# Sirui-Xu/InterDiff

Measured on AMD Instinct MI355X. Metric: denoising frame-steps/sec (denoising-steps/sec x B x T frames), higher is better.
Workload: dtype f32 (every contraction of the denoiser -- feed-forward block, QKV projection, self-attention, row-block contractions and the two token GEMMs: every fp32 operand as two f16 planes, 3 f16 MFMAs per product, fp32 accumulate; SMPL and everything else fp32 MFMA / VALU)

## Files before the change

include/interdiff_hip.h:

```cpp
#ifndef INTERDIFF_HIP_H
#define INTERDIFF_HIP_H

#include <stddef.h>
#include <stdint.h>

#ifdef __cplusplus
extern "C" {
#endif

#define IDF_OK            0
#define IDF_E_INVAL      -22
#define IDF_E_NOMEM      -12
#define IDF_E_LAUNCH     -5

int         interdiff_abi_version(void);
const char *interdiff_build_info(void);

int interdiff_rotation_6d_to_matrix   (const float *d6, float *m,  int64_t n, void *stream);
int interdiff_matrix_to_rotation_6d   (const float *m,  float *d6, int64_t n, void *stream);
int interdiff_matrix_to_axis_angle    (const float *m,  float *aa, int64_t n, void *stream);
int interdiff_axis_angle_to_matrix    (const float *aa, float *m,  int64_t n, void *stream);
int interdiff_axis_angle_to_quaternion(const float *aa, float *q,  int64_t n, void *stream);
int interdiff_rotation_6d_to_axis_angle(const float *d6, float *aa, int64_t n, void *stream);

typedef struct {
    int32_t V, J, n_betas, KB, S;
    const float   *blend;
    const float   *jt;
    const float   *js;
    const int32_t *parents;
    const int32_t *skin_idx;
    const float   *skin_w;
} idf_smpl_model;

size_t interdiff_smpl_workspace_bytes(const idf_smpl_model *m, int64_t N);
int interdiff_smpl_forward(const idf_smpl_model *m, const float *pose, const float *betas,
                           const float *trans, int64_t N, float *verts, float *jtr,
                           float *v_posed, void *ws, size_t ws_bytes, void *stream);

int interdiff_vertex_normals(const float *verts, int64_t N, int32_t V, const int32_t *faces,
                             const int32_t *adj_ptr, const int32_t *adj_face,
                             const int32_t *adj_corner, float *normals, void *stream);
int interdiff_nn_argmin(const float *q, int32_t Pq, const float *r, int32_t Pr, int64_t N,
                        int32_t *idx, void *stream);
int interdiff_point2point_signed(const float *x, int32_t P1, const float *y, int32_t P2, int64_t N,
                                 const float *x_normals, const float *y_normals,
                                 float *y2x_signed, float *x2y_signed, int32_t *yidx, int32_t *xidx,
                                 float *y2x, float *x2y, void *stream);

#define IDF_MDM_LAYERS 8
#define IDF_MDM_D      256
#define IDF_MDM_FF     1024
#define IDF_MDM_HEADS  4
#define IDF_MDM_NQ     10
#define IDF_MDM_MEM    10
#define IDF_MDM_MEM_MAX 16
#define IDF_FFN_SLICES 5

typedef struct {
    int64_t is_qan;
    int64_t sa_in_w, sa_in_b, sa_out_w, sa_out_b;
    int64_t qc, wk;
    int64_t ca_q_w, ca_q_b;
    int64_t ca_kv_w, ca_kv_b;
    int64_t ca_out_w, ca_out_b;
    int64_t ff1_w, ff1_b, ff2_w, ff2_b;
    int64_t ffn_pack;
    int64_t ffn_b1p;
    int64_t sa_in_pack;
    int64_t sa_out_frag;
    int64_t ln_w[3], ln_b[3];
    int64_t ffn_pack_h2;
    int64_t sa_in_pack_h2;
    int64_t qc_h2;
    int64_t rb_h2_ok;
    int64_t sa_out_frag_h2;
    int64_t qkv_bounds_ok;
} idf_mdm_layer;

typedef struct {
    int32_t C;
    int32_t n_steps;
    const float *arena;
    int64_t in_w, in_b;
    int64_t out_w, out_b;
    int64_t temb_table;
    int64_t pe;
    int32_t max_T, has_encoder;
    idf_mdm_layer layer[IDF_MDM_LAYERS];
    idf_mdm_layer enc_layer[IDF_MDM_LAYERS];
    int32_t tune[8];
    int64_t out_w_h2, in_w_h2;
    int64_t tail_h2_ok;
    int32_t mem_len;
    int32_t rb_tokens;
} idf_mdm_weights;

int interdiff_gemm_f32(const float *A, int32_t lda, const float *W, const float *bias, const float *resid, float *C,
                       int32_t ldc, int32_t M, int32_t N, int32_t K, int32_t epi, int32_t cfg, void *stream);

int interdiff_mdm_ffn(const idf_mdm_weights *w, int32_t layer, int32_t encoder, const float *x2, int32_t M, float *parts, void *stream);
size_t interdiff_mdm_memctx_floats_for(int32_t B, int32_t mem_len);

size_t interdiff_mdm_memctx_floats(int32_t B);
size_t interdiff_mdm_workspace_bytes(int32_t B, int32_t T);
int interdiff_mdm_prepare_memory(const idf_mdm_weights *w, const float *cond, int32_t B,
                                 float *memctx, void *ws, size_t ws_bytes, void *stream);
int interdiff_mdm_forward(const idf_mdm_weights *w, const float *memctx, const float *x,
                          const int64_t *ts, int32_t B, int32_t T, float *x0,
                          void *ws, size_t ws_bytes, void *stream);

typedef struct {
    int64_t w[3], b[3];
    int32_t c[4];
} idf_pn_mlp;

typedef struct {
    const float *arena;
    idf_pn_mlp sa1[2];
    idf_pn_mlp sa2[2];
    int64_t lin_w, lin_b;
} idf_pointnet2;

int interdiff_pointnet2_encode(const idf_pointnet2 *pn, const float *obj_points, int32_t B, int32_t P, float *out,
                               void *stream);
size_t interdiff_mdm_encode_workspace_bytes(int32_t B, int32_t Tp);
int interdiff_mdm_encode(const idf_mdm_weights *w, const float *pc, const float *x_past, int32_t B, int32_t Tp,
                         float *cond, void *ws, size_t ws_bytes, void *stream);

int interdiff_inpaint(float *x0, const float *gt, const uint8_t *mask, int64_t n, void *stream);
int interdiff_posterior_step(float *x, const float *x0, const float *noise, int64_t n,
                             float c1, float c2, float sigma, uint64_t seed, uint64_t step_index,
                             void *stream);
int interdiff_randn(float *out, int64_t n, uint64_t seed, uint64_t step_index, void *stream);
int interdiff_posterior_step_at(float *x, const float *x0, const float *noise, int64_t n,
                                float c1, float c2, float sigma, uint64_t seed, uint64_t step_index,
                                uint64_t elem0, void *stream);
int interdiff_randn_at(float *out, int64_t n, uint64_t seed, uint64_t step_index, uint64_t elem0, void *stream);
int interdiff_posterior_step_dev(float *x, const float *x0, const float *gt, const uint8_t *mask, int64_t n,
                                 const float *table, int64_t *state, int64_t *ts, int32_t B, void *stream);
int interdiff_sampler_advance(int64_t *state, int64_t *ts, int32_t B, void *stream);
int interdiff_posterior_step_dev_map(float *x, const float *x0, const float *gt, const uint8_t *mask, int64_t n,
                                     const float *table, const int64_t *tmap, int64_t *state, int64_t *ts, int32_t B, void *stream);
int interdiff_sampler_advance_map(int64_t *state, int64_t *ts, const int64_t *tmap, int32_t B, void *stream);
int interdiff_mdm_forward_step(const idf_mdm_weights *w, const float *memctx, float *x, int64_t *ts, int32_t B, int32_t T,
                               const float *gt, const uint8_t *mask, const float *table, int64_t *state,
                               void *ws, size_t ws_bytes, void *stream);
#define IDF_STEP_EMBED_READY 1
#define IDF_STEP_EMBED_NEXT 2
int interdiff_mdm_forward_step_ex(const idf_mdm_weights *w, const float *memctx, float *x, int64_t *ts, int32_t B, int32_t T,
                                  const float *gt, const uint8_t *mask, const float *table, int64_t *state, void *ws,
                                  size_t ws_bytes, int32_t flags, void *stream);
int interdiff_mdm_forward_step_map(const idf_mdm_weights *w, const float *memctx, float *x, int64_t *ts, int32_t B, int32_t T,
                                   const float *gt, const uint8_t *mask, const float *table, const int64_t *tmap, int64_t *state,
                                   void *ws, size_t ws_bytes, int32_t flags, void *stream);
int interdiff_mdm_step_chaining(const idf_mdm_weights *w);
int interdiff_exclusive_cu_report(char *buf, int32_t cap);
int interdiff_debug_deny_exclusive(const char *patterns);

typedef struct {
    int32_t T, past_len, P, n_pre;
    const float *arena;
    int64_t dct_pad;
    int64_t dct;
    int64_t idct;
    int64_t hand_bonus;
    int64_t layer[12];
    int32_t cin[12], cout[12];
} idf_objproj;

int interdiff_objprojector_sample(const idf_objproj *op, const float *obj_angles,
                                  const float *obj_trans, const float *markers,
                                  const int32_t *contact, int32_t B, float *out, void *stream);
size_t interdiff_objprojector_forward_workspace_bytes(int32_t B);
int interdiff_objprojector_forward(const idf_objproj *op, const float *obj_angles, const float *obj_trans, const float *markers,
                                   const int32_t *contact, int32_t B, int32_t initialize, float *out, void *ws, size_t ws_bytes, void *stream);

int interdiff_correction_finetune_param_table(const idf_objproj *op, int32_t *table, int32_t *n_param, int32_t *n_bn);
size_t interdiff_correction_finetune_workspace_bytes(const idf_objproj *op, int32_t B);
int interdiff_correction_finetune_grads(const idf_objproj *op, const float *params, const float *bn, const float *obj_angles,
                                        const float *obj_trans, const float *markers, const int32_t *contact, const float *d_obj_pred,
                                        int32_t B, int32_t T, int32_t initialize, const float *weights8, float *out9, float *grads, void *ws,
                                        size_t ws_bytes, void *stream);
int interdiff_correction_finetune_step(const idf_objproj *op, float *arena, float *params, const float *bn, const float *grads,
                                       float *exp_avg, float *exp_avg_sq, int32_t step, double lr, double beta1, double beta2, double eps,
                                       double weight_decay, void *stream);

size_t interdiff_correction_train_workspace_bytes(const idf_objproj *op, int32_t B);
int interdiff_correction_train_grads(const idf_objproj *op, const float *params, float *bn, const float *obj_angles, const float *obj_trans,
                                     const float *markers, const int32_t *contact, const int32_t *nodes, const float *d_obj_pred, int32_t B,
                                     int32_t T, int32_t initialize, const float *weights8, double p_drop, const uint8_t *masks, uint64_t seed,
                                     uint64_t step, double momentum, int32_t update_running, float *out9, float *grads, float *batch_stats,
                                     void *ws, size_t ws_bytes, void *stream);
int interdiff_correction_train_masks(const idf_objproj *op, int32_t B, double p_drop, uint64_t seed, uint64_t step, uint8_t *masks_out,
                                     void *stream);

int interdiff_correction_finetune_predict(const idf_objproj *op, const float *params, const float *bn, const float *obj_angles,
                                          const float *obj_trans, const float *markers, const int32_t *contact, int32_t B, int32_t T,
                                          int32_t initialize, float *obj_pred_out, void *ws, size_t ws_bytes, void *stream);
int interdiff_correction_train_predict(const idf_objproj *op, const float *params, const float *obj_angles, const float *obj_trans,
                                       const float *markers, const int32_t *contact, const int32_t *nodes, int32_t B, int32_t T,
                                       int32_t initialize, double p_drop, const uint8_t *masks, uint64_t seed, uint64_t step, float *obj_pred_out,
                                       void *ws, size_t ws_bytes, void *stream);

typedef struct {
    const idf_smpl_model *smpl;
    const idf_objproj    *objproj;
    const int32_t *faces;
    const int32_t *adj_ptr, *adj_face, *adj_corner;
    const int32_t *markers_idx;
    int32_t n_markers, n_points, past_len;
    int32_t tune;
    const int32_t *vorder, *faces_scan, *markers_scan, *adj_pair_scan;
    const int32_t *adj_pair;
    const int32_t *vrank;
} idf_correction_ctx;

size_t interdiff_correction_workspace_bytes(const idf_correction_ctx *c, int32_t B, int32_t T);
int interdiff_correction(const idf_correction_ctx *c, float *x0, const float *gt,
                         const float *hand_pose, const float *beta, const float *obj_points,
                         int32_t B, int32_t T, float blend_t ,
                         uint8_t *condition, int32_t *contact, float *distance, float *loss,
                         void *ws, size_t ws_bytes, void *stream);
int interdiff_correction_dev(const idf_correction_ctx *c, float *x0, const float *gt, const float *hand_pose,
                             const float *beta, const float *obj_points, int32_t B, int32_t T, const float *table,
                             const int64_t *state, void *ws, size_t ws_bytes, void *stream);

#define IDF_CONTACT_STATS 12
size_t interdiff_contact_nn_workspace_bytes(const idf_correction_ctx *c, int32_t B, int32_t T);
int interdiff_contact_nn(const idf_correction_ctx *c, const float *verts, const float *obj_points, const float *objR,
                         const float *objT, int32_t B, int32_t T, float *o2h, int32_t *idx, uint64_t *stats,
                         void *ws, size_t ws_bytes, void *stream);

size_t interdiff_metrics_workspace_bytes(const idf_correction_ctx *c, int32_t B, int32_t T);
int interdiff_metrics(const idf_correction_ctx *c, const float *obj_pred, const float *jtr,
                      const float *body_trans, const float *obj_gt, const float *jtr_gt,
                      const float *body_trans_gt, const float *verts, const float *obj_points,
                      int32_t B, int32_t T, int32_t J, float *out6 ,
                      void *ws, size_t ws_bytes, void *stream);

typedef struct {
    int32_t T, past_len, J, n_pre;
    const float *arena;
    int64_t dct_pad;
    int64_t dct;
    int64_t idct;
    int64_t layer[12];
    int32_t cin[12], cout[12];
} idf_skel_objproj;

int interdiff_skeleton_objprojector_sample(const idf_skel_objproj *op, const float *obj_angles,
                                           const float *obj_trans, const float *human_points, int32_t B,
                                           float *quat_out, float *trans_out, void *stream);
int interdiff_skeleton_correction(const idf_skel_objproj *op, const float *x, const float *gt,
                                  const float *zero_pose_obj, int32_t B, int32_t T, float blend_t,
                                  float *out, void *stream);
int interdiff_skeleton_metrics(const float *body_pred, const float *body_gt, const float *obj_pred,
                               const float *obj_gt, const float *pose_pred, const float *pose_gt,
                               int32_t T, int32_t B, int32_t from_frame, float *out4, void *stream);

int interdiff_skeleton_finetune_param_table(const idf_skel_objproj *op, int32_t *table, int32_t *n_param, int32_t *n_bn);
size_t interdiff_skeleton_finetune_workspace_bytes(const idf_skel_objproj *op, int32_t B);
int interdiff_skeleton_finetune_grads(const idf_skel_objproj *op, const float *params, const float *bn, const float *obj_angles,
                                      const float *obj_trans, const float *human_points, const float *pose_gt, int32_t B, int32_t T,
                                      const float *weights8, float *out9, float *grads, void *ws, size_t ws_bytes, void *stream);
int interdiff_skeleton_finetune_step(const idf_skel_objproj *op, float *arena, float *params, const float *bn, const float *grads,
                                     float *exp_avg, float *exp_avg_sq, int32_t step, double lr, double beta1, double beta2, double eps,
                                     double weight_decay, void *stream);

size_t interdiff_skeleton_train_workspace_bytes(const idf_skel_objproj *op, int32_t B);
int interdiff_skeleton_train_grads(const idf_skel_objproj *op, const float *params, float *bn, const float *obj_angles, const float *obj_trans,
                                   const float *human_points, const float *pose_gt, int32_t B, int32_t T, const float *weights8, double p_drop,
                                   const uint8_t *masks, uint64_t seed, uint64_t step, double momentum, int32_t update_running, float *out9,
                                   float *grads, float *batch_stats, void *ws, size_t ws_bytes, void *stream);
int interdiff_skeleton_train_masks(const idf_skel_objproj *op, int32_t B, double p_drop, uint64_t seed, uint64_t step, uint8_t *masks_out,
                                   void *stream);

typedef struct idf_skel_head {
    int32_t n_body, n_points;
    int32_t n_tiles, reserved;
    int64_t out_w, out_b;
    int64_t shape_w, shape_b;
} idf_skel_head;
int interdiff_skeleton_mdm_forward(const idf_mdm_weights *w, const idf_skel_head *head, const float *memctx, const float *x,
                                   const int64_t *ts, const float *zero_pose_obj, int32_t B, int32_t T, float *x0,
                                   void *ws, size_t ws_bytes, void *stream);
int interdiff_skeleton_mdm_forward_step(const idf_mdm_weights *w, const idf_skel_head *head, const float *memctx, float *x,
                                        int64_t *ts, const float *zero_pose_obj, int32_t B, int32_t T, const float *gt,
                                        const uint8_t *mask, const float *table, int64_t *state, void *ws, size_t ws_bytes,
                                        void *stream);
int interdiff_skeleton_mdm_forward_step_map(const idf_mdm_weights *w, const idf_skel_head *head, const float *memctx, float *x,
                                            int64_t *ts, const float *zero_pose_obj, int32_t B, int32_t T, const float *gt,
                                            const uint8_t *mask, const float *table, const int64_t *tmap, int64_t *state, void *ws,
                                            size_t ws_bytes, void *stream);
size_t interdiff_skeleton_mdm_encode_workspace_bytes(int32_t B, int32_t Tp);
int interdiff_skeleton_mdm_encode(const idf_mdm_weights *w, const idf_skel_head *head, const float *zero_pose_obj,
                                  const float *x_past, int32_t B, int32_t Tp, float *cond, void *ws, size_t ws_bytes,
                                  void *stream);

#define IDF_OPT_NP 483
#define IDF_OPT_NLOSS 6
typedef struct {
    const idf_correction_ctx *geo;
    const float   *blendT;
    const int32_t *jv_ptr;
    const int32_t *jv_vtx;
    const float   *jv_w;
    int32_t K3P, _pad;
} idf_opt_ctx;

typedef struct {
    int32_t B, T, P, max_iters;
    const float *betas;
    const float *obj_points;
    float *param, *init, *grad, *m, *v, *best;
    float *pose, *tr;
    float *verts, *vposed, *verts_gt, *gv;
    float *jtr;
    float *pts, *y2x;
    float *y2x_signed;
    int32_t *yidx;
    int32_t *near;
    float *dvposed;
    float *dA;
    float *dfeat;
    float *gtr;
    float *lossf;
    float *loss;
    float *loss_hist;
    float *best_loss;
    int32_t *flag;
    uint8_t *foot_static;
    int32_t *foot_cnt;
    int32_t *ctl;
    void *smpl_ws; size_t smpl_ws_bytes;
    int32_t *porder; float *psort, *pbox;
} idf_opt_state;

int interdiff_optimize_init(const idf_opt_ctx *c, const idf_opt_state *st, const float *pose, const float *trans,
                            const float *obj_angles, const float *obj_trans, int32_t first_iter, void *stream);
int interdiff_optimize_loss_grad(const idf_opt_ctx *c, const idf_opt_state *st, void *stream);
int interdiff_optimize_step(const idf_opt_ctx *c, const idf_opt_state *st, void *stream);
int interdiff_optimize_finish(const idf_opt_ctx *c, const idf_opt_state *st, float *pose, float *trans, float *obj_angles,
                              float *obj_trans, void *stream);
int interdiff_debug_joint_map_vjp(const float *R, const float *g_out, float *g_in, int32_t n);
int interdiff_debug_lds_sentinel(uint32_t *out, int32_t n_wg, int32_t spin, void *stream);
int interdiff_debug_f16_aggressor(const float *src, size_t n_floats, float *sink, int32_t iters, int32_t grid, int32_t with_loads, void *stream);

enum { IDF_LOSS_VAL = 0, IDF_LOSS_TEST = 1 };
int interdiff_q_sample(float *x_t, const float *x0, const float *noise, const int64_t *ts, const float *sqrt_ac, const float *sqrt_1mac,
                       int32_t n_steps, const float *gt, const uint8_t *mask, int32_t B, int64_t per_clip, uint64_t seed, uint64_t elem0,
                       void *stream);
int interdiff_denoising_losses(const float *pred, const float *target, int32_t B, int32_t T, int32_t past_len, float *out, void *stream);
size_t interdiff_sample_losses_workspace_bytes(int32_t K, int32_t B);
int interdiff_sample_losses(const float *samples, const float *gt, const float *hand_pose, int32_t K, int32_t B, int32_t T, int32_t past_len,
                            int32_t variant, float *out_terms, float *out_per_clip, void *ws, size_t ws_bytes, void *stream);

int interdiff_denoising_loss_grad(const float *pred, const float *target, int32_t B, int32_t T, int32_t past_len, const float *weights16,
                                  float *d_pred, void *stream);
int interdiff_mdm_train_param_table(int64_t *offsets, int64_t *sizes, int32_t *n_tensors, int64_t *n_param);
size_t interdiff_mdm_train_workspace_bytes(int32_t B, int32_t T, int32_t mem_len);
int interdiff_mdm_train_grads(const float *params, const float *pe, int32_t pe_rows, const float *x_t, const int64_t *ts, const float *cond,
                              const float *target, int32_t B, int32_t T, int32_t mem_len, int32_t past_len, const float *weights16,
                              const float *d_pred_in, float *grads, float *d_cond, float *pred, float *terms, void *ws, size_t ws_bytes,
                              void *stream);
int interdiff_mdm_train_step(float *params, const float *grads, float *exp_avg, float *exp_avg_sq, int64_t n, int32_t step, double lr,
                             double beta1, double beta2, double eps, double weight_decay, void *stream);

int interdiff_mdm_train_full_param_table(int64_t *offsets, int64_t *sizes, int32_t *n_tensors, int64_t *n_param);
size_t interdiff_mdm_train_full_workspace_bytes(int32_t B, int32_t T, int32_t past_len);
int interdiff_mdm_train_full_grads(const float *params, const float *pe, int32_t pe_rows, const float *x_t, const int64_t *ts, const float *pc,
                                   const float *target, int32_t B, int32_t T, int32_t past_len, const float *weights16, const float *d_pred_in,
                                   float *grads, float *cond, float *d_cond, float *d_pc, float *pred, float *terms, void *ws, size_t ws_bytes,
                                   void *stream);

size_t interdiff_pointnet2_saves_bytes(int32_t B);
int interdiff_pointnet2_encode_saved(const idf_pointnet2 *pn, const float *obj_points, int32_t B, int32_t P, float *out, void *saves, size_t saves_bytes,
                                     void *stream);
int interdiff_pointnet2_finetune_param_table(int64_t *offsets, int64_t *sizes, int32_t *n_tensors, int64_t *n_param);
size_t interdiff_pointnet2_finetune_workspace_bytes(int32_t B);
int interdiff_pointnet2_finetune_grads(const idf_pointnet2 *pn, const float *theta, const float *stats, const float *obj_points, int32_t B, int32_t P,
                                       const void *saves, const float *d_pc, float *grads, void *ws, size_t ws_bytes, void *stream);
int interdiff_pointnet2_refold(const idf_pointnet2 *pn, const float *theta, const float *stats, void *stream);

size_t interdiff_pointnet2_train_workspace_bytes(int32_t B);
int interdiff_pointnet2_train_forward(const float *theta, const float *obj_points, int32_t B, int32_t P, float *pc_out, void *ws, size_t ws_bytes, void *stream);
int interdiff_pointnet2_train_grads(const float *theta, const float *obj_points, int32_t B, int32_t P, const float *d_pc, float *grads, void *ws, size_t ws_bytes,
                                    void *stream);
int interdiff_pointnet2_train_stats(const void *ws, int32_t B, double momentum, float *stats, void *stream);

size_t interdiff_skeleton_sample_losses_workspace_bytes(int32_t K, int32_t B);
int interdiff_skeleton_sample_losses(const float *pred, const float *gt, int32_t K, int32_t B, int32_t C, int32_t T, int32_t past_len,
                                     int32_t n_body, int32_t n_points, float *out_terms, float *out_per_clip, void *ws, size_t ws_bytes,
                                     void *stream);
int interdiff_skeleton_denoising_losses(const float *pred, const float *target, int32_t B, int32_t T, int32_t past_len, int32_t n_body,
                                        int32_t n_points, float *out, void *stream);

int interdiff_skeleton_denoising_loss_grad(const float *pred, const float *target, int32_t B, int32_t T, int32_t past_len, const float *weights13,
                                           float *d_pred, void *stream);
int interdiff_skeleton_mdm_train_param_table(int64_t *offsets, int64_t *sizes, int32_t *n_tensors, int64_t *n_param);
size_t interdiff_skeleton_mdm_train_workspace_bytes(int32_t B, int32_t T, int32_t past_len);
int interdiff_skeleton_mdm_train_grads(const float *params, const float *pe, int32_t pe_rows, const float *x_t, const int64_t *ts, const float *target,
                                       const float *zero_pose_obj, int32_t B, int32_t T, int32_t past_len, const float *weights13,
                                       const float *d_pred_in, float *grads, float *cond, float *pred, float *terms, void *ws, size_t ws_bytes,
                                       void *stream);

size_t interdiff_correction_losses_workspace_bytes(int32_t T, int32_t B, int32_t V, int32_t P);
int interdiff_correction_losses(const float *obj_pred, const float *obj_gt, const float *obj_points, int32_t point_stride, const float *human_verts,
                                int32_t T, int32_t B, int32_t V, int32_t P, int32_t rot_width, int32_t past_len, float *out_terms, float *out_frames,
                                void *ws, size_t ws_bytes, void *stream);

size_t interdiff_correction_geometry_grads_workspace_bytes(int32_t T, int32_t B, int32_t V, int32_t P);
int interdiff_correction_geometry_grads(const float *obj_pred, const float *obj_points, int32_t point_stride, const float *human_verts, int32_t T,
                                        int32_t B, int32_t V, int32_t P, double w_penetration, double w_contact, float *d_obj_pred_out,
                                        float *terms2_out, float *frames_out, void *ws, size_t ws_bytes, void *stream);

size_t interdiff_contact_labels_workspace_bytes(int64_t N, int32_t V, int32_t F, int32_t P);
int interdiff_contact_labels(const float *verts, int64_t N, int32_t V, const int32_t *faces, int32_t F, const float *points, int32_t P,
                             int64_t point_frame_stride, const float *objR, const float *objT, float thres, uint8_t *obj_label ,
                             uint8_t *human_label , float *signed_dist , void *ws, size_t ws_bytes, void *stream);
int interdiff_debug_point_triangle(const float *tri, const float *p, float *out, int32_t n);

#define IDF_RENDER_SUBPIX 16
#define IDF_RENDER_GUARD 32768
#define IDF_RENDER_MAX_DIM 2048
#define IDF_RENDER_ZONE (1 << 28)
#define IDF_RENDER_REC_INTS 20
#define IDF_RENDER_TILE 16
#define IDF_RENDER_MAX_MESHES 8
enum { IDF_RMESH_SCENE_SPACE = 1, IDF_RMESH_VERTEX_RGB = 2 };
typedef struct {
    float off[3], cam_t[3];
    float cam_cos, cam_sin, znear, focal;
    float light[9];
    float light_gain, ambient;
    float bg[3];
    float reserved;
} idf_render_scene;
typedef struct {
    const float *verts, *normals;
    const int32_t *faces;
    const float *rgb, *R, *t;
    int32_t V, F, frames, flags;
} idf_render_mesh;
size_t interdiff_render_frames_workspace_bytes(int64_t n_images, int64_t n_triangles, int32_t H, int32_t W);
int interdiff_render_frames(const idf_render_scene *scene, const idf_render_mesh *meshes, int32_t n_meshes, int64_t N, int32_t views, int32_t H,
                            int32_t W, uint8_t *out_rgb, int32_t *out_id, int32_t *out_depth, int32_t *out_setup, int64_t *dropped, float *stage_ms,
                            void *ws, size_t ws_bytes, void *stream);
int interdiff_debug_render_setup_vertex(const idf_render_scene *scene, int32_t view, int32_t scene_space, int32_t H, int32_t W, const float *pos,
                                        const float *nrm, const float *rgb, float *out_f, int32_t *out_i, int32_t n);
int interdiff_debug_render_pixel(const int32_t *rec, const int32_t *ij, int32_t *out, int32_t n);

#define IDF_SKEL_REC_INTS 8
#define IDF_SKEL_MAX_REC 128
#define IDF_SKEL_MAX_WIRES 40
#define IDF_SKEL_WD_MAX 1024
#define IDF_SKEL_TILE 16
enum { IDF_SKEL_PLAIN = 0, IDF_SKEL_PREDGT = 1 };
typedef struct {
    float view[12];
    float aspect[3], margin[3];
    float dist, kx, cx, ky, cy;
    int32_t line_wd, disc_wd, style, pred_from;
    uint8_t colour[5][4];
} idf_skel_view;
size_t interdiff_skeleton_render_frames_workspace_bytes(int64_t n_frames);
int interdiff_skeleton_render_frames(const idf_skel_view *view, const float *body, const float *obj, const float *body_gt, const float *obj_gt,
                                     const int32_t *wires, int32_t n_wires, int64_t B, int32_t T, int32_t T_gt, int32_t H, int32_t W, uint8_t *out_rgb,
                                     int32_t *out_setup, int32_t *out_count, int64_t *dropped, float *stage_ms, void *ws, size_t ws_bytes, void *stream);
int interdiff_skeleton_raster_records(const int32_t *recs, int32_t count, int64_t n_frames, int32_t H, int32_t W, uint8_t *out_rgb, void *stream);
int interdiff_debug_skeleton_setup(const idf_skel_view *view, const float *body, const float *obj, const float *body_gt, const float *obj_gt,
                                   const int32_t *wires, int32_t n_wires, int32_t T, int32_t T_gt, int32_t t, int32_t *rec, int32_t *count,
                                   int32_t *dropped);
int interdiff_debug_skeleton_pixel(const int32_t *rec, int32_t n_rec, const int32_t *ij, int32_t *out, int32_t n);

typedef struct {
    int32_t n_seq, P, V, n_markers;
    const int64_t *seq_off;
    const float *pose, *betas;
    const double *fit64;
    const float *joints, *obj_points6;
    const int32_t *first_label, *body_ptr, *body_idx, *markers_idx;
} idf_clip_set;
typedef struct {
    float *body_pose, *hand_pose, *body_trans, *obj_angles, *obj_trans, *pelvis, *beta, *gt, *ground, *centroid, *rotation, *obj_points, *obj_points6;
    uint8_t *contact_label;
} idf_clip_batch;
int interdiff_clip_batch(const idf_clip_set *cs, const int32_t *clips, int32_t B, int32_t T, int32_t sample_rate, const idf_clip_batch *out, void *stream);
int interdiff_clip_body_records(const idf_clip_set *cs, const int32_t *clips, int32_t B, int32_t T, int32_t sample_rate, const float *verts,
                                const float *normals, const int32_t *frame_map, int64_t n_frames, float *human_verts, float *markers,
                                uint8_t *contact_label, void *stream);
int interdiff_debug_clip_canon(const double *fit, const float *pelvis, const float *pose, int32_t T, const float *rotation_override, float *root,
                               float *trans, float *obj_angle, float *obj_trans, float *pelvis_out, float *gt, float *centroid, float *rotation);

typedef struct {
    int32_t n_video, J, P, reserved;
    const int64_t *row_off;
    const float *table, *zero_pose_obj;
} idf_skel_clip_set;
typedef struct {
    float *body, *obj, *pose, *zero_pose_obj, *gt;
} idf_skel_window_batch;
int interdiff_skeleton_video_prepare(const double *skel, const double *obj, const double *pose, const double *contact, const int64_t *seq_off,
                                     const int64_t *row_off, int32_t n_video, int32_t J, int32_t P, int32_t stride, float *table, float *zero_pose_obj,
                                     double *report, double *row_contact, int8_t *signs, void *stream);
int interdiff_debug_skeleton_video_prepare(const double *skel, const double *obj, const double *pose, const double *contact, int64_t F, int32_t J, int32_t P,
                                           int32_t stride, float *table, float *zero_pose_obj, double *report, double *row_contact, int8_t *signs);
int interdiff_skeleton_window_batch(const idf_skel_clip_set *cs, const int32_t *clips, int32_t B, int32_t T, const idf_skel_window_batch *out, void *stream);

enum {
    IDF_K_EMBED = 0, IDF_K_GEMM_QKV, IDF_K_SELF_ATTN, IDF_K_GEMM_OUTPROJ, IDF_K_ROWBLOCK_QAN,
    IDF_K_ROWBLOCK_STD, IDF_K_FFN_FUSED, IDF_K_RESERVED7, IDF_K_GEMM_HEADS, IDF_K_MEM_PREP,
    IDF_K_INPAINT, IDF_K_POSTERIOR, IDF_K_CORR_PREPARE, IDF_K_SMPL_POSE, IDF_K_SMPL_BLEND_SKIN,
    IDF_K_CORR_CONTACT, IDF_K_CORR_REDUCE, IDF_K_OBJPROJ, IDF_K_CORR_BLEND, IDF_K_OTHER,
    IDF_K_COUNT
};
int interdiff_profile_begin(int32_t capacity);
int interdiff_profile_end(double *ms_per_kind, int64_t *count_per_kind);

enum {
    IDF_TUNE_FFN = 3, IDF_TUNE_FFN_MATH = 4, IDF_TUNE_COUNT = 8
};

#ifdef __cplusplus
}
#endif
#endif
```

interdiff_amd/_lib.py:

```python
import ctypes as C
import os
import torch

_HERE = os.path.dirname(os.path.abspath(__file__))
LIB_PATH = os.environ.get('INTERDIFF_HIP_LIB') or os.path.join(_HERE, 'csrc', 'libinterdiff_hip.so')
ABI_VERSION = 17

vp, i32, i64, f32, u64, sz = C.c_void_p, C.c_int32, C.c_int64, C.c_float, C.c_uint64, C.c_size_t

MDM_LAYERS = 8
FFN_SLICES = 5
STEP_EMBED_READY, STEP_EMBED_NEXT = 1, 2
LOSS_VAL, LOSS_TEST = 0, 1
TUNE = dict(ffn=3, ffn_math=4)


class SmplModel(C.Structure):
    _fields_ = [('V', i32), ('J', i32), ('n_betas', i32), ('KB', i32), ('S', i32),
                ('blend', vp), ('jt', vp), ('js', vp), ('parents', vp), ('skin_idx', vp), ('skin_w', vp)]


class MdmLayer(C.Structure):
    _fields_ = [('is_qan', i64),
                ('sa_in_w', i64), ('sa_in_b', i64), ('sa_out_w', i64), ('sa_out_b', i64),
                ('qc', i64), ('wk', i64),
                ('ca_q_w', i64), ('ca_q_b', i64), ('ca_kv_w', i64), ('ca_kv_b', i64),
                ('ca_out_w', i64), ('ca_out_b', i64),
                ('ff1_w', i64), ('ff1_b', i64), ('ff2_w', i64), ('ff2_b', i64), ('ffn_pack', i64), ('ffn_b1p', i64), ('sa_in_pack', i64), ('sa_out_frag', i64),
                ('ln_w', i64 * 3), ('ln_b', i64 * 3), ('ffn_pack_h2', i64), ('sa_in_pack_h2', i64), ('qc_h2', i64), ('rb_h2_ok', i64), ('sa_out_frag_h2', i64), ('qkv_bounds_ok', i64)]


class MdmWeights(C.Structure):
    _fields_ = [('C', i32), ('n_steps', i32), ('arena', vp),
                ('in_w', i64), ('in_b', i64), ('out_w', i64), ('out_b', i64),
                ('temb_table', i64), ('pe', i64), ('max_T', i32), ('has_encoder', i32),
                ('layer', MdmLayer * MDM_LAYERS), ('enc_layer', MdmLayer * MDM_LAYERS), ('tune', i32 * 8), ('out_w_h2', i64), ('in_w_h2', i64), ('tail_h2_ok', i64), ('mem_len', i32), ('rb_tokens', i32)]


class PnMlp(C.Structure):
    _fields_ = [('w', i64 * 3), ('b', i64 * 3), ('c', i32 * 4)]


class PointNet2(C.Structure):
    _fields_ = [('arena', vp), ('sa1', PnMlp * 2), ('sa2', PnMlp * 2), ('lin_w', i64), ('lin_b', i64)]


class ObjProj(C.Structure):
    _fields_ = [('T', i32), ('past_len', i32), ('P', i32), ('n_pre', i32), ('arena', vp),
                ('dct_pad', i64), ('dct', i64), ('idct', i64), ('hand_bonus', i64),
                ('layer', i64 * 12), ('cin', i32 * 12), ('cout', i32 * 12)]


class SkelObjProj(C.Structure):
    _fields_ = [('T', i32), ('past_len', i32), ('J', i32), ('n_pre', i32), ('arena', vp),
                ('dct_pad', i64), ('dct', i64), ('idct', i64),
                ('layer', i64 * 12), ('cin', i32 * 12), ('cout', i32 * 12)]


class SkelHead(C.Structure):
    _fields_ = [('n_body', i32), ('n_points', i32), ('n_tiles', i32), ('reserved', i32),
                ('out_w', i64), ('out_b', i64), ('shape_w', i64), ('shape_b', i64)]


class CorrectionCtx(C.Structure):
    _fields_ = [('smpl', C.POINTER(SmplModel)), ('objproj', C.POINTER(ObjProj)),
                ('faces', vp), ('adj_ptr', vp), ('adj_face', vp), ('adj_corner', vp), ('markers_idx', vp),
                ('n_markers', i32), ('n_points', i32), ('past_len', i32), ('tune', i32),
                ('vorder', vp), ('faces_scan', vp), ('markers_scan', vp), ('adj_pair_scan', vp), ('adj_pair', vp), ('vrank', vp)]


class OptCtx(C.Structure):
    _fields_ = [('geo', C.POINTER(CorrectionCtx)), ('blendT', vp), ('jv_ptr', vp), ('jv_vtx', vp), ('jv_w', vp), ('K3P', i32), ('_pad', i32)]


OPT_NP, OPT_NLOSS = 483, 6
_OPT_PTRS = ('betas', 'obj_points', 'param', 'init', 'grad', 'm', 'v', 'best', 'pose', 'tr', 'verts', 'vposed', 'verts_gt', 'gv',
             'jtr', 'pts', 'y2x', 'y2x_signed', 'yidx', 'near', 'dvposed', 'dA', 'dfeat', 'gtr', 'lossf', 'loss', 'loss_hist',
             'best_loss', 'flag', 'foot_static', 'foot_cnt', 'ctl', 'smpl_ws')


class OptState(C.Structure):
    _fields_ = [('B', i32), ('T', i32), ('P', i32), ('max_iters', i32)] + [(k, vp) for k in _OPT_PTRS] + [('smpl_ws_bytes', sz), ('porder', vp), ('psort', vp), ('pbox', vp)]


class RenderScene(C.Structure):
    _fields_ = [('off', f32 * 3), ('cam_t', f32 * 3), ('cam_cos', f32), ('cam_sin', f32), ('znear', f32), ('focal', f32),
                ('light', f32 * 9), ('light_gain', f32), ('ambient', f32), ('bg', f32 * 3), ('reserved', f32)]


class RenderMesh(C.Structure):
    _fields_ = [('verts', vp), ('normals', vp), ('faces', vp), ('rgb', vp), ('R', vp), ('t', vp),
                ('V', i32), ('F', i32), ('frames', i32), ('flags', i32)]


class SkelView(C.Structure):
    _fields_ = [('view', f32 * 12), ('aspect', f32 * 3), ('margin', f32 * 3), ('dist', f32), ('kx', f32), ('cx', f32), ('ky', f32), ('cy', f32),
                ('line_wd', i32), ('disc_wd', i32), ('style', i32), ('pred_from', i32), ('colour', (C.c_uint8 * 4) * 5)]


class ClipSet(C.Structure):
    _fields_ = [('n_seq', i32), ('P', i32), ('V', i32), ('n_markers', i32), ('seq_off', vp), ('pose', vp), ('betas', vp), ('fit64', vp), ('joints', vp),
                ('obj_points6', vp), ('first_label', vp), ('body_ptr', vp), ('body_idx', vp), ('markers_idx', vp)]


CLIP_BATCH_FIELDS = ('body_pose', 'hand_pose', 'body_trans', 'obj_angles', 'obj_trans', 'pelvis', 'beta', 'gt', 'ground', 'centroid', 'rotation', 'obj_points',
                     'obj_points6', 'contact_label')


class ClipBatch(C.Structure):
    _fields_ = [(k, vp) for k in CLIP_BATCH_FIELDS]


class SkelClipSet(C.Structure):
    _fields_ = [('n_video', i32), ('J', i32), ('P', i32), ('reserved', i32), ('row_off', vp), ('table', vp), ('zero_pose_obj', vp)]


SKEL_WINDOW_FIELDS = ('body', 'obj', 'pose', 'zero_pose_obj', 'gt')


class SkelWindowBatch(C.Structure):
    _fields_ = [(k, vp) for k in SKEL_WINDOW_FIELDS]


CLIP_MAX_T = 128
SKEL_SET_MAX_P, SKEL_WINDOW_LDS = 64, 64 * 1024
SKEL_PLAIN, SKEL_PREDGT = 0, 1
SKEL_REC_INTS, SKEL_MAX_REC, SKEL_MAX_WIRES, SKEL_WD_MAX, SKEL_TILE = 8, 128, 40, 1024, 16
RMESH_SCENE_SPACE, RMESH_VERTEX_RGB = 1, 2
RENDER_SUBPIX, RENDER_GUARD, RENDER_MAX_DIM, RENDER_ZONE, RENDER_REC_INTS, RENDER_TILE = 16, 32768, 2048, 1 << 28, 20, 16

_SIGS = {
    'interdiff_abi_version': (C.c_int, []),
    'interdiff_build_info': (C.c_char_p, []),
    'interdiff_rotation_6d_to_matrix': (C.c_int, [vp, vp, i64, vp]),
    'interdiff_matrix_to_rotation_6d': (C.c_int, [vp, vp, i64, vp]),
    'interdiff_matrix_to_axis_angle': (C.c_int, [vp, vp, i64, vp]),
    'interdiff_axis_angle_to_matrix': (C.c_int, [vp, vp, i64, vp]),
    'interdiff_axis_angle_to_quaternion': (C.c_int, [vp, vp, i64, vp]),
    'interdiff_rotation_6d_to_axis_angle': (C.c_int, [vp, vp, i64, vp]),
    'interdiff_smpl_workspace_bytes': (sz, [C.POINTER(SmplModel), i64]),
    'interdiff_smpl_forward': (C.c_int, [C.POINTER(SmplModel), vp, vp, vp, i64, vp, vp, vp, vp, sz, vp]),
    'interdiff_vertex_normals': (C.c_int, [vp, i64, i32, vp, vp, vp, vp, vp, vp]),
    'interdiff_nn_argmin': (C.c_int, [vp, i32, vp, i32, i64, vp, vp]),
    'interdiff_point2point_signed': (C.c_int, [vp, i32, vp, i32, i64, vp, vp, vp, vp, vp, vp, vp, vp, vp]),
    'interdiff_gemm_f32': (C.c_int, [vp, i32, vp, vp, vp, vp, i32, i32, i32, i32, i32, i32, vp]),
    'interdiff_pointnet2_encode': (C.c_int, [C.POINTER(PointNet2), vp, i32, i32, vp, vp]),
    'interdiff_mdm_encode_workspace_bytes': (sz, [i32, i32]),
    'interdiff_mdm_encode': (C.c_int, [C.POINTER(MdmWeights), vp, vp, i32, i32, vp, vp, sz, vp]),
    'interdiff_mdm_ffn': (C.c_int, [C.POINTER(MdmWeights), i32, i32, vp, i32, vp, vp]),
    'interdiff_mdm_memctx_floats': (sz, [i32]),
    'interdiff_mdm_memctx_floats_for': (sz, [i32, i32]),
    'interdiff_mdm_workspace_bytes': (sz, [i32, i32]),
    'interdiff_mdm_prepare_memory': (C.c_int, [C.POINTER(MdmWeights), vp, i32, vp, vp, sz, vp]),
    'interdiff_mdm_forward': (C.c_int, [C.POINTER(MdmWeights), vp, vp, vp, i32, i32, vp, vp, sz, vp]),
    'interdiff_mdm_forward_step': (C.c_int, [C.POINTER(MdmWeights), vp, vp, vp, i32, i32, vp, vp, vp, vp, vp, sz, vp]),
    'interdiff_mdm_forward_step_ex': (C.c_int, [C.POINTER(MdmWeights), vp, vp, vp, i32, i32, vp, vp, vp, vp, vp, sz, i32, vp]),
    'interdiff_mdm_forward_step_map': (C.c_int, [C.POINTER(MdmWeights), vp, vp, vp, i32, i32, vp, vp, vp, vp, vp, vp, sz, i32, vp]),
    'interdiff_mdm_step_chaining': (C.c_int, [C.POINTER(MdmWeights)]),
    'interdiff_inpaint': (C.c_int, [vp, vp, vp, i64, vp]),
    'interdiff_posterior_step': (C.c_int, [vp, vp, vp, i64, f32, f32, f32, u64, u64, vp]),
    'interdiff_randn': (C.c_int, [vp, i64, u64, u64, vp]),
    'interdiff_posterior_step_at': (C.c_int, [vp, vp, vp, i64, f32, f32, f32, u64, u64, u64, vp]),
    'interdiff_randn_at': (C.c_int, [vp, i64, u64, u64, u64, vp]),
    'interdiff_posterior_step_dev': (C.c_int, [vp, vp, vp, vp, i64, vp, vp, vp, i32, vp]),
    'interdiff_sampler_advance': (C.c_int, [vp, vp, i32, vp]),
    'interdiff_posterior_step_dev_map': (C.c_int, [vp, vp, vp, vp, i64, vp, vp, vp, vp, i32, vp]),
    'interdiff_sampler_advance_map': (C.c_int, [vp, vp, vp, i32, vp]),
    'interdiff_objprojector_sample': (C.c_int, [C.POINTER(ObjProj), vp, vp, vp, vp, i32, vp, vp]),
    'interdiff_objprojector_forward_workspace_bytes': (sz, [i32]),
    'interdiff_objprojector_forward': (C.c_int, [C.POINTER(ObjProj), vp, vp, vp, vp, i32, i32, vp, vp, sz, vp]),
    'interdiff_correction_finetune_param_table': (C.c_int, [C.POINTER(ObjProj), vp, C.POINTER(i32), C.POINTER(i32)]),
    'interdiff_correction_finetune_workspace_bytes': (sz, [C.POINTER(ObjProj), i32]),
    'interdiff_correction_finetune_grads': (C.c_int, [C.POINTER(ObjProj), vp, vp, vp, vp, vp, vp, vp, i32, i32, i32, C.POINTER(f32), vp, vp, vp, sz, vp]),
    'interdiff_correction_finetune_step': (C.c_int, [C.POINTER(ObjProj), vp, vp, vp, vp, vp, vp, i32, C.c_double, C.c_double, C.c_double, C.c_double,
                                                     C.c_double, vp]),
    'interdiff_correction_finetune_predict': (C.c_int, [C.POINTER(ObjProj), vp, vp, vp, vp, vp, vp, i32, i32, i32, vp, vp, sz, vp]),
    'interdiff_correction_train_predict': (C.c_int, [C.POINTER(ObjProj), vp, vp, vp, vp, vp, vp, i32, i32, i32, C.c_double, vp, u64, u64, vp, vp, sz, vp]),
    'interdiff_correction_geometry_grads_workspace_bytes': (sz, [i32, i32, i32, i32]),
    'interdiff_correction_geometry_grads': (C.c_int, [vp, vp, i32, vp, i32, i32, i32, i32, C.c_double, C.c_double, vp, vp, vp, vp, sz, vp]),
    'interdiff_correction_train_workspace_bytes': (sz, [C.POINTER(ObjProj), i32]),
    'interdiff_correction_train_grads': (C.c_int, [C.POINTER(ObjProj), vp, vp, vp, vp, vp, vp, vp, vp, i32, i32, i32, C.POINTER(f32), C.c_double, vp, u64, u64,
                                                   C.c_double, i32, vp, vp, vp, vp, sz, vp]),
    'interdiff_correction_train_masks': (C.c_int, [C.POINTER(ObjProj), i32, C.c_double, u64, u64, vp, vp]),
    'interdiff_correction_workspace_bytes': (sz, [C.POINTER(CorrectionCtx), i32, i32]),
    'interdiff_correction': (C.c_int, [C.POINTER(CorrectionCtx), vp, vp, vp, vp, vp, i32, i32, f32,
                                       vp, vp, vp, vp, vp, sz, vp]),
    'interdiff_correction_dev': (C.c_int, [C.POINTER(CorrectionCtx), vp, vp, vp, vp, vp, i32, i32, vp, vp, vp, sz, vp]),
    'interdiff_metrics_workspace_bytes': (sz, [C.POINTER(CorrectionCtx), i32, i32]),
    'interdiff_metrics': (C.c_int, [C.POINTER(CorrectionCtx), vp, vp, vp, vp, vp, vp, vp, vp, i32, i32, i32,
                                    vp, vp, sz, vp]),
    'interdiff_contact_nn_workspace_bytes': (sz, [C.POINTER(CorrectionCtx), i32, i32]),
    'interdiff_contact_nn': (C.c_int, [C.POINTER(CorrectionCtx), vp, vp, vp, vp, i32, i32, vp, vp, vp, vp, sz, vp]),
    'interdiff_skeleton_objprojector_sample': (C.c_int, [C.POINTER(SkelObjProj), vp, vp, vp, i32, vp, vp, vp]),
    'interdiff_skeleton_correction': (C.c_int, [C.POINTER(SkelObjProj), vp, vp, vp, i32, i32, f32, vp, vp]),
    'interdiff_skeleton_metrics': (C.c_int, [vp, vp, vp, vp, vp, vp, i32, i32, i32, vp, vp]),
    'interdiff_skeleton_finetune_param_table': (C.c_int, [C.POINTER(SkelObjProj), vp, C.POINTER(i32), C.POINTER(i32)]),
    'interdiff_skeleton_finetune_workspace_bytes': (sz, [C.POINTER(SkelObjProj), i32]),
    'interdiff_skeleton_finetune_grads': (C.c_int, [C.POINTER(SkelObjProj), vp, vp, vp, vp, vp, vp, i32, i32, C.POINTER(f32), vp, vp, vp, sz, vp]),
    'interdiff_skeleton_finetune_step': (C.c_int, [C.POINTER(SkelObjProj), vp, vp, vp, vp, vp, vp, i32, C.c_double, C.c_double, C.c_double, C.c_double,
                                                   C.c_double, vp]),
    'interdiff_skeleton_train_workspace_bytes': (sz, [C.POINTER(SkelObjProj), i32]),
    'interdiff_skeleton_train_grads': (C.c_int, [C.POINTER(SkelObjProj), vp, vp, vp, vp, vp, vp, i32, i32, C.POINTER(f32), C.c_double, vp, u64, u64,
                                                 C.c_double, i32, vp, vp, vp, vp, sz, vp]),
    'interdiff_skeleton_train_masks': (C.c_int, [C.POINTER(SkelObjProj), i32, C.c_double, u64, u64, vp, vp]),
    'interdiff_skeleton_mdm_forward': (C.c_int, [C.POINTER(MdmWeights), C.POINTER(SkelHead), vp, vp, vp, vp, i32, i32, vp, vp, sz, vp]),
    'interdiff_skeleton_mdm_forward_step': (C.c_int, [C.POINTER(MdmWeights), C.POINTER(SkelHead), vp, vp, vp, vp, i32, i32, vp, vp, vp, vp, vp, sz, vp]),
    'interdiff_skeleton_mdm_forward_step_map': (C.c_int, [C.POINTER(MdmWeights), C.POINTER(SkelHead), vp, vp, vp, vp, i32, i32, vp, vp, vp, vp, vp, vp, sz, vp]),
    'interdiff_skeleton_mdm_encode_workspace_bytes': (sz, [i32, i32]),
    'interdiff_skeleton_mdm_encode': (C.c_int, [C.POINTER(MdmWeights), C.POINTER(SkelHead), vp, vp, i32, i32, vp, vp, sz, vp]),
    'interdiff_q_sample': (C.c_int, [vp, vp, vp, vp, vp, vp, i32, vp, vp, i32, i64, u64, u64, vp]),
    'interdiff_denoising_losses': (C.c_int, [vp, vp, i32, i32, i32, vp, vp]),
    'interdiff_sample_losses_workspace_bytes': (sz, [i32, i32]),
    'interdiff_sample_losses': (C.c_int, [vp, vp, vp, i32, i32, i32, i32, i32, vp, vp, vp, sz, vp]),
    'interdiff_denoising_loss_grad': (C.c_int, [vp, vp, i32, i32, i32, C.POINTER(f32), vp, vp]),
    'interdiff_mdm_train_param_table': (C.c_int, [C.POINTER(i64), C.POINTER(i64), C.POINTER(i32), C.POINTER(i64)]),
    'interdiff_mdm_train_workspace_bytes': (sz, [i32, i32, i32]),
    'interdiff_mdm_train_grads': (C.c_int, [vp, vp, i32, vp, vp, vp, vp, i32, i32, i32, i32, C.POINTER(f32), vp, vp, vp, vp, vp, vp, sz, vp]),
    'interdiff_mdm_train_step': (C.c_int, [vp, vp, vp, vp, i64, i32, C.c_double, C.c_double, C.c_double, C.c_double, C.c_double, vp]),
    'interdiff_mdm_train_full_param_table': (C.c_int, [C.POINTER(i64), C.POINTER(i64), C.POINTER(i32), C.POINTER(i64)]),
    'interdiff_mdm_train_full_workspace_bytes': (sz, [i32, i32, i32]),
    'interdiff_mdm_train_full_grads': (C.c_int, [vp, vp, i32, vp, vp, vp, vp, i32, i32, i32, C.POINTER(f32), vp, vp, vp, vp, vp, vp, vp, vp, sz, vp]),
    'interdiff_pointnet2_saves_bytes': (sz, [i32]),
    'interdiff_pointnet2_encode_saved': (C.c_int, [C.POINTER(PointNet2), vp, i32, i32, vp, vp, sz, vp]),
    'interdiff_pointnet2_finetune_param_table': (C.c_int, [C.POINTER(i64), C.POINTER(i64), C.POINTER(i32), C.POINTER(i64)]),
    'interdiff_pointnet2_finetune_workspace_bytes': (sz, [i32]),
    'interdiff_pointnet2_finetune_grads': (C.c_int, [C.POINTER(PointNet2), vp, vp, vp, i32, i32, vp, vp, vp, vp, sz, vp]),
    'interdiff_pointnet2_refold': (C.c_int, [C.POINTER(PointNet2), vp, vp, vp]),
    'interdiff_pointnet2_train_workspace_bytes': (sz, [i32]),
    'interdiff_pointnet2_train_forward': (C.c_int, [vp, vp, i32, i32, vp, vp, sz, vp]),
    'interdiff_pointnet2_train_grads': (C.c_int, [vp, vp, i32, i32, vp, vp, vp, sz, vp]),
    'interdiff_pointnet2_train_stats': (C.c_int, [vp, i32, C.c_double, vp, vp]),
    'interdiff_skeleton_sample_losses_workspace_bytes': (sz, [i32, i32]),
    'interdiff_skeleton_sample_losses': (C.c_int, [vp, vp, i32, i32, i32, i32, i32, i32, i32, vp, vp, vp, sz, vp]),
    'interdiff_skeleton_denoising_losses': (C.c_int, [vp, vp, i32, i32, i32, i32, i32, vp, vp]),
    'interdiff_skeleton_denoising_loss_grad': (C.c_int, [vp, vp, i32, i32, i32, C.POINTER(f32), vp, vp]),
    'interdiff_skeleton_mdm_train_param_table': (C.c_int, [C.POINTER(i64), C.POINTER(i64), C.POINTER(i32), C.POINTER(i64)]),
    'interdiff_skeleton_mdm_train_workspace_bytes': (sz, [i32, i32, i32]),
    'interdiff_skeleton_mdm_train_grads': (C.c_int, [vp, vp, i32, vp, vp, vp, vp, i32, i32, i32, C.POINTER(f32), vp, vp, vp, vp, vp, vp, sz, vp]),
    'interdiff_correction_losses_workspace_bytes': (sz, [i32, i32, i32, i32]),
    'interdiff_correction_losses': (C.c_int, [vp, vp, vp, i32, vp, i32, i32, i32, i32, i32, i32, vp, vp, vp, sz, vp]),
    'interdiff_contact_labels_workspace_bytes': (sz, [i64, i32, i32, i32]),
    'interdiff_contact_labels': (C.c_int, [vp, i64, i32, vp, i32, vp, i32, i64, vp, vp, f32, vp, vp, vp, vp, sz, vp]),
    'interdiff_debug_point_triangle': (C.c_int, [vp, vp, vp, i32]),
    'interdiff_render_frames_workspace_bytes': (sz, [i64, i64, i32, i32]),
    'interdiff_render_frames': (C.c_int, [C.POINTER(RenderScene), C.POINTER(RenderMesh), i32, i64, i32, i32, i32, vp, vp, vp, vp, C.POINTER(i64), C.POINTER(f32),
                                          vp, sz, vp]),
    'interdiff_debug_render_setup_vertex': (C.c_int, [C.POINTER(RenderScene), i32, i32, i32, i32, vp, vp, vp, vp, vp, i32]),
    'interdiff_debug_render_pixel': (C.c_int, [vp, vp, vp, i32]),
    'interdiff_skeleton_render_frames_workspace_bytes': (sz, [i64]),
    'interdiff_skeleton_render_frames': (C.c_int, [C.POINTER(SkelView), vp, vp, vp, vp, vp, i32, i64, i32, i32, i32, i32, vp, vp, vp, C.POINTER(i64),
                                                   C.POINTER(f32), vp, sz, vp]),
    'interdiff_skeleton_raster_records': (C.c_int, [vp, i32, i64, i32, i32, vp, vp]),
    'interdiff_debug_skeleton_setup': (C.c_int, [C.POINTER(SkelView), vp, vp, vp, vp, vp, i32, i32, i32, i32, vp, C.POINTER(i32), C.POINTER(i32)]),
    'interdiff_debug_skeleton_pixel': (C.c_int, [vp, i32, vp, vp, i32]),
    'interdiff_optimize_init': (C.c_int, [C.POINTER(OptCtx), C.POINTER(OptState), vp, vp, vp, vp, i32, vp]),
    'interdiff_optimize_loss_grad': (C.c_int, [C.POINTER(OptCtx), C.POINTER(OptState), vp]),
    'interdiff_optimize_step': (C.c_int, [C.POINTER(OptCtx), C.POINTER(OptState), vp]),
    'interdiff_optimize_finish': (C.c_int, [C.POINTER(OptCtx), C.POINTER(OptState), vp, vp, vp, vp, vp]),
    'interdiff_debug_joint_map_vjp': (C.c_int, [vp, vp, vp, i32]),
    'interdiff_clip_batch': (C.c_int, [C.POINTER(ClipSet), vp, i32, i32, i32, C.POINTER(ClipBatch), vp]),
    'interdiff_clip_body_records': (C.c_int, [C.POINTER(ClipSet), vp, i32, i32, i32, vp, vp, vp, i64, vp, vp, vp, vp]),
    'interdiff_debug_clip_canon': (C.c_int, [vp, vp, vp, i32, vp, vp, vp, vp, vp, vp, vp, vp, vp]),
    'interdiff_skeleton_video_prepare': (C.c_int, [vp, vp, vp, vp, vp, vp, i32, i32, i32, i32, vp, vp, vp, vp, vp, vp]),
    'interdiff_debug_skeleton_video_prepare': (C.c_int, [vp, vp, vp, vp, i64, i32, i32, i32, vp, vp, vp, vp, vp]),
    'interdiff_skeleton_window_batch': (C.c_int, [C.POINTER(SkelClipSet), vp, i32, i32, C.POINTER(SkelWindowBatch), vp]),
    'interdiff_debug_lds_sentinel':(C.c_int, [vp, i32, i32, vp]),
    'interdiff_exclusive_cu_report': (C.c_int, [C.c_char_p, i32]),
    'interdiff_debug_deny_exclusive': (C.c_int, [C.c_char_p]),
    'interdiff_debug_f16_aggressor': (C.c_int, [vp, sz, vp, i32, i32, i32, vp]),
    'interdiff_profile_begin': (C.c_int, [i32]),
    'interdiff_profile_end': (C.c_int, [C.POINTER(C.c_double), C.POINTER(C.c_int64)]),
}

KERNEL_KINDS = ('embed', 'gemm_qkv', 'self_attn', 'gemm_outproj', 'rowblock_qan', 'rowblock_std', 'ffn_fused', 'reserved7',
                'gemm_heads', 'mem_prep', 'inpaint', 'posterior', 'corr_prepare', 'smpl_pose', 'smpl_blend_skin',
                'corr_contact', 'corr_reduce', 'objproj', 'corr_blend', 'other')

_lib = None


class HipLibraryMissing(RuntimeError):
    pass


def load():
    global _lib
    if _lib is not None:
        return _lib
    if not os.path.exists(LIB_PATH):
        raise HipLibraryMissing('%s not found: build it with `python -m interdiff_amd.csrc.build` '
                                '(there is no CPU/torch fallback for the hot path)' % LIB_PATH)
    lib = C.CDLL(LIB_PATH)
    for name, (res, args) in _SIGS.items():
        fn = getattr(lib, name)
        fn.restype, fn.argtypes = res, args
    if lib.interdiff_abi_version() != ABI_VERSION:
        raise HipLibraryMissing('stale %s: abi %d != %d, rebuild' % (LIB_PATH, lib.interdiff_abi_version(), ABI_VERSION))
    _lib = lib
    return lib


def exclusive_cu_report():
    buf = C.create_string_buffer(8192)
    bad = load().interdiff_exclusive_cu_report(buf, len(buf))
    if bad < 0:
        check(bad, 'exclusive_cu_report')
    return buf.value.decode(), bad


def debug_deny_exclusive(patterns=''):
    check(load().interdiff_debug_deny_exclusive(patterns.encode() if patterns else None), 'debug_deny_exclusive')


def exported_symbols():
    return sorted(_SIGS)


_ERR = {-22: 'IDF_E_INVAL (bad shape / pointer / unsupported size)', -12: 'IDF_E_NOMEM (workspace too small)',
        -5: 'IDF_E_LAUNCH (kernel launch failed)'}


def check(rc, what=''):
    if rc != 0:
        raise RuntimeError('interdiff_hip %s failed: %s' % (what, _ERR.get(rc, rc)))


def dptr(t, dtype=None, allow_none=False):
    if t is None:
        if allow_none:
            return vp(None)
        raise ValueError('null tensor')
    if not t.is_cuda:
        raise ValueError('interdiff_amd ops need device tensors (got %s); the HIP path has no CPU fallback' % t.device)
    if not t.is_contiguous():
        raise ValueError('tensor must be contiguous')
    if dtype is not None and t.dtype != dtype:
        raise ValueError('expected %s, got %s' % (dtype, t.dtype))
    return vp(t.data_ptr())


def stream():
    return vp(torch.cuda.current_stream().cuda_stream)
```

interdiff_amd/correction.py:

```python
import ctypes as C
import os
import itertools
import numpy as np
import torch
from . import _lib
from .geometry import MeshTopology

MARKERS67 = [3470, 3171, 3327, 857, 1812, 628, 182, 3116, 3040, 239,
             1666, 1725, 0, 2174, 1568, 1368, 3387, 2112, 1053, 1058,
             3336, 3346, 1323, 2108, 3122, 3314, 1252, 1082, 1861, 1454,
             850, 2224, 3233, 1769, 6728, 4343, 5273, 4116, 3694, 6399,
             6540, 6488, 3749, 5135, 5194, 3512, 5635, 5210, 4360, 4841,
             6786, 5573, 4538, 4544, 6736, 6747, 4804, 5568, 6544, 6682,
             5322, 4927, 5686, 4598, 6633, 3506, 3508]


_UID = itertools.count(1)


def correction_gate(t0):
    return not (t0 > 500 or t0 % 50 != 0)


class HipCorrection:
    def __init__(self, smpl_layer, objprojector, n_points=2048, past_len=10, markers=MARKERS67, device='cuda', scan_order=True):
        self.lib = _lib.load()
        self.device = torch.device(device)
        self.smpl, self.objproj, self.past_len = smpl_layer, objprojector, past_len
        self.topo = MeshTopology(smpl_layer.th_faces, smpl_layer.cmodel.V, self.device, rest_vertices=getattr(smpl_layer, 'v_template', None) if scan_order else None)
        self.markers_idx = torch.tensor(list(markers), dtype=torch.int32, device=self.device)
        ctx = _lib.CorrectionCtx()
        ctx.smpl = C.pointer(smpl_layer.cmodel)
        ctx.objproj = C.pointer(objprojector.cop)
        self.topo.fill_ctx(ctx)
        ctx.markers_idx = self.markers_idx.data_ptr()
        ctx.n_markers, ctx.n_points, ctx.past_len = len(markers), n_points, past_len
        if self.topo.vorder is not None:
            self.markers_scan = self.topo.scan_positions(markers, self.device)
            ctx.markers_scan = self.markers_scan.data_ptr()
        ctx.tune = 0
        self.ctx = ctx
        self._ws = {}
        self.debug = None
        self._uid = next(_UID)

    graph_capturable = True

    def workspace_for(self, B, T):
        return torch.empty(self.lib.interdiff_correction_workspace_bytes(C.byref(self.ctx), B, T), dtype=torch.uint8, device=self.device)

    def apply_dev(self, x, table, state, y, ws):
        B, _, Cc, T = x.shape
        if y['obj_points'].shape[1] != self.ctx.n_points:
            raise ValueError('obj_points must have %d points' % self.ctx.n_points)
        _lib.check(self.lib.interdiff_correction_dev(C.byref(self.ctx), _lib.dptr(x, torch.float32), _lib.dptr(y['inpainted_motion'], torch.float32),
                                                     _lib.dptr(y['hand_pose'], torch.float32), _lib.dptr(y['beta'], torch.float32),
                                                     _lib.dptr(y['obj_points'], torch.float32), B, T, _lib.dptr(table), _lib.dptr(state),
                                                     _lib.dptr(ws), ws.numel(), _lib.stream()), 'correction_dev')
        return x

    def _workspace(self, B, T):
        need = self.lib.interdiff_correction_workspace_bytes(C.byref(self.ctx), B, T)
        key = torch.cuda.current_stream(self.device).cuda_stream
        ws = self._ws.pop(key, None)
        if ws is None or ws.numel() < need:
            ws = torch.empty(need, dtype=torch.uint8, device=self.device)
        self._ws[key] = ws
        if len(self._ws) > self.MAX_STREAM_WORKSPACES:
            torch.cuda.synchronize(self.device)
            self._ws.pop(next(iter(self._ws)))
        return ws

    MAX_STREAM_WORKSPACES = 4

    def apply(self, x, t0, y):
        B, _, Cc, T = x.shape
        if not x.is_contiguous():
            raise ValueError('x must be contiguous (it is updated in place)')
        if y['obj_points'].shape[1] != self.ctx.n_points:
            raise ValueError('obj_points must have %d points' % self.ctx.n_points)
        gt = y['inpainted_motion'].contiguous()
        hp, beta, pts = y['hand_pose'].contiguous().float(), y['beta'].contiguous().float(), y['obj_points'].contiguous().float()
        ws = self._workspace(B, T)
        dbg = [None] * 4
        if self.debug is not None:
            dbg = [torch.empty(B, dtype=torch.uint8, device=self.device), torch.empty(B, len(MARKERS67), dtype=torch.int32, device=self.device),
                   torch.empty(B, device=self.device), torch.empty(B, device=self.device)]
        blend_t = float(np.float32(t0) / np.float32(1000))
        _lib.check(self.lib.interdiff_correction(C.byref(self.ctx), _lib.dptr(x, torch.float32), _lib.dptr(gt, torch.float32),
                                                 _lib.dptr(hp), _lib.dptr(beta), _lib.dptr(pts), B, T, blend_t,
                                                 *[_lib.dptr(d, allow_none=True) for d in dbg], _lib.dptr(ws), ws.numel(),
                                                 _lib.stream()), 'correction')
        if self.debug is not None:
            self.debug.update(condition=dbg[0], contact=dbg[1], distance=dbg[2], loss=dbg[3])
        return x

    def contact_nn(self, verts, obj_points, objR, objT, want_stats=False):
        T, B = verts.shape[:2]
        P = self.ctx.n_points
        o2h = torch.empty(T, B, P, device=self.device)
        idx = torch.empty(T, B, P, dtype=torch.int32, device=self.device)
        stats = torch.zeros(12, dtype=torch.int64, device=self.device) if want_stats else None
        need = self.lib.interdiff_contact_nn_workspace_bytes(C.byref(self.ctx), B, T)
        ws = getattr(self, '_nn_ws', None)
        if ws is None or ws.numel() < need:
            ws = self._nn_ws = torch.empty(need, dtype=torch.uint8, device=self.device)
        v, pts, R_, t_ = (a.contiguous().float() for a in (verts, obj_points, objR, objT))
        _lib.check(self.lib.interdiff_contact_nn(C.byref(self.ctx), _lib.dptr(v), _lib.dptr(pts), _lib.dptr(R_), _lib.dptr(t_), B, T, _lib.dptr(o2h),
                                                 _lib.dptr(idx), _lib.dptr(stats, allow_none=True), _lib.dptr(ws), ws.numel(), _lib.stream()), 'contact_nn')
        return (o2h, idx, tuple(int(x) for x in stats.cpu())) if want_stats else (o2h, idx)

    def is_active(self, t0):
        return correction_gate(int(t0))

    def __call__(self, x, t, model_kwargs):
        t0 = getattr(t, 'host_value', None)
        if t0 is None:
            t0 = int(t[0])
        if not correction_gate(t0):
            return x
        return self.apply(x, t0, model_kwargs['y'])
```

interdiff_amd/csrc/contact_scan.h:

```cpp
#pragma once
#include <float.h>
#include "common.h"
#include "objproj.h"
#include "vec3.h"

namespace {

constexpr int MAXP = 2048;
__global__ __launch_bounds__(1024) void corr_point_order_kernel(const float *__restrict__ obj_points, int P, int32_t *__restrict__ porder) {
    __shared__ unsigned long long keys[MAXP];
    __shared__ float red[6][1024];
    const int b = blockIdx.x, tid = threadIdx.x;
    const float *op = obj_points + (size_t)b * P * 3;
    float p[2][3];
    float lo[3] = {FLT_MAX, FLT_MAX, FLT_MAX}, hi[3] = {-FLT_MAX, -FLT_MAX, -FLT_MAX};
#pragma unroll
    for (int k = 0; k < 2; ++k) {
        const int i = tid + 1024 * k;
#pragma unroll
        for (int a = 0; a < 3; ++a) {
            p[k][a] = i < P ? op[3 * i + a] : 0.f;
            if (i < P) { lo[a] = fminf(lo[a], p[k][a]); hi[a] = fmaxf(hi[a], p[k][a]); }
        }
    }
#pragma unroll
    for (int a = 0; a < 3; ++a) { red[a][tid] = lo[a]; red[3 + a][tid] = hi[a]; }
    __syncthreads();
    for (int s = 512; s > 0; s >>= 1) {
        if (tid < s) {
#pragma unroll
            for (int a = 0; a < 3; ++a) {
                red[a][tid] = fminf(red[a][tid], red[a][tid + s]);
                red[3 + a][tid] = fmaxf(red[3 + a][tid], red[3 + a][tid + s]);
            }
        }
        __syncthreads();
    }
#pragma unroll
    for (int k = 0; k < 2; ++k) {
        const int i = tid + 1024 * k;
        unsigned long long key = ~0ull;
        if (i < P) {
            unsigned code = 0;
            unsigned q[3];
#pragma unroll
            for (int a = 0; a < 3; ++a) {
                const float ext = red[3 + a][0] - red[a][0];
                const float u = ext > 0.f ? (p[k][a] - red[a][0]) / ext : 0.f;
                q[a] = (unsigned)fminf(fmaxf(u * 1023.0f, 0.f), 1023.0f);
            }
#pragma unroll
            for (int bit = 0; bit < 10; ++bit)
#pragma unroll
                for (int a = 0; a < 3; ++a) code |= ((q[a] >> bit) & 1u) << (3 * bit + a);
            key = ((unsigned long long)code << 11) | (unsigned)i;
        }
        keys[i] = key;
    }
    __syncthreads();
    for (int k = 2; k <= MAXP; k <<= 1) {
        for (int j = k >> 1; j > 0; j >>= 1) {
            const int l = 2 * j * (tid / j) + (tid % j), r = l + j;
            const unsigned long long x = keys[l], y = keys[r];
            const bool up = (l & k) == 0;
            if ((x > y) == up) { keys[l] = y; keys[r] = x; }
            __syncthreads();
        }
    }
#pragma unroll
    for (int k = 0; k < 2; ++k) {
        const int i = tid + 1024 * k;
        if (i < P) porder[(size_t)b * P + i] = (int32_t)(keys[i] & 2047u);
    }
}

constexpr int MAXM = 128;
constexpr float MARK_D2 = 0.00039999996079131961f;
constexpr int CB = 16;
constexpr int SB = 8;
constexpr int SEED_STRIDE = 4;
constexpr int CT = 1024;
constexpr int TASK = 64;
typedef float v2f __attribute__((ext_vector_type(2)));

struct ContactLds {
    int V4, nCB, nSB, nSeed;
    int rec, mark, box, sbox, seed, flags, red, pl, total;
    __host__ __device__ explicit ContactLds(int V) {
        V4 = (V + CB - 1) / CB * CB; nCB = V4 / CB; nSB = (nCB + SB - 1) / SB; nSeed = (nCB + SEED_STRIDE - 1) / SEED_STRIDE;
        rec = 0;
        mark = rec + V4;
        box = mark + MAXM;
        sbox = box + 3 * (nSB * SB / 2);
        seed = sbox + 3 * ((nSB + 2) / 2);
        flags = seed + 2 * ((nSeed + 1) / 2);
        red = flags + MAXM / 4;
        pl = red + CT / 4;
        total = pl + MAXP / 4;
    }
};

__device__ __forceinline__ float3 lds_rec(const float4 *vs, int pos) {
    const float *f = reinterpret_cast<const float *>(vs + 2 * (pos >> 1));
    const int h = pos & 1;
    return make_float3(f[h], f[2 + h], f[4 + h]);
}
__device__ __forceinline__ void lds_rec_store(float4 *vs, int pos, float x, float y, float z) {
    float *f = reinterpret_cast<float *>(vs + 2 * (pos >> 1));
    const int h = pos & 1;
    f[h] = x; f[2 + h] = y; f[4 + h] = z;
}
__device__ __forceinline__ void lds_box_store(float4 *bx, int k, float3 lo, float3 hi) {
    float *f = reinterpret_cast<float *>(bx + 3 * (k >> 1));
    const int h = k & 1;
    f[h] = lo.x; f[2 + h] = lo.y; f[4 + h] = lo.z; f[6 + h] = hi.x; f[8 + h] = hi.y; f[10 + h] = hi.z;
}
__device__ __forceinline__ void lds_box_load(const float4 *bx, int k, float3 &lo, float3 &hi) {
    const float *f = reinterpret_cast<const float *>(bx + 3 * (k >> 1));
    const int h = k & 1;
    lo = make_float3(f[h], f[2 + h], f[4 + h]);
    hi = make_float3(f[6 + h], f[8 + h], f[10 + h]);
}

struct PredArgs {
    idf_objproj op;
    const float *obj_angles, *obj_trans;
    const int32_t *markers_idx;
    float *markers, *keep;
    int nclips;
};
template <bool OPT, bool WITH_PRED = false>
__global__ __launch_bounds__(CT) void corr_contact_kernel(const float *__restrict__ verts, int V,
                                                          const float *__restrict__ obj_points, int P,
                                                          const int32_t *__restrict__ porder ,
                                                          const float *__restrict__ objR, const float *__restrict__ objT,
                                                          const int32_t *__restrict__ faces ,
                                                          const int32_t *__restrict__ adj_ptr,
                                                          const int32_t *__restrict__ adj_face,
                                                          const int32_t *__restrict__ adj_corner,
                                                          const int32_t *__restrict__ adj_pair ,
                                                          const int32_t *__restrict__ vorder ,
                                                          const int32_t *__restrict__ vrank ,
                                                          const int32_t *__restrict__ markers_pos , int M, int B,
                                                          float *__restrict__ markers_out, float *__restrict__ loss_sum,
                                                          float *__restrict__ min_dist, int32_t *__restrict__ label,
                                                          float *__restrict__ o2h_out ,
                                                          int32_t *__restrict__ idx_out ,
                                                          unsigned long long *__restrict__ stats ,
                                                          int64_t nn_from ,
                                                          const float *__restrict__ pts_frame , int frames_per_clip ,
                                                          const PredArgs pred) {
    extern __shared__ __attribute__((aligned(16))) float4 vs[];
    if constexpr (WITH_PRED) {
        if ((int)blockIdx.x < pred.nclips) {
            const int b = blockIdx.x, Tn = pred.op.T;
            for (int i = threadIdx.x; i < Tn * M; i += CT) {
                const int t = i / M, m = i - t * M;
                const size_t nfr = (size_t)t * B + b;
                const float *v = verts + (nfr * V + pred.markers_idx[m]) * 3;
                float *o = pred.markers + (nfr * M + m) * 3;
                o[0] = v[0]; o[1] = v[1]; o[2] = v[2];
            }
            __threadfence();
            __syncthreads();
            idf_objproj_dev::objproj_body<1>(reinterpret_cast<float *>(vs), pred.op, pred.obj_angles, pred.obj_trans, pred.markers, nullptr, B, b, pred.keep, nullptr);
            return;
        }
    }
    const ContactLds L(V);
    const int nCB = L.nCB, nSB = L.nSB;
    float4 *ms = vs + L.mark, *bb = vs + L.box, *sbb = vs + L.sbox, *sd = vs + L.seed;
    int *flags = reinterpret_cast<int *>(vs + L.flags);
    float *red = reinterpret_cast<float *>(vs + L.red);
    float *pl = reinterpret_cast<float *>(vs + L.pl);
    __shared__ int next_task;
    const int64_t n = WITH_PRED ? (int64_t)blockIdx.x - pred.nclips : (int64_t)blockIdx.x;
    const int b = OPT ? (int)(n / frames_per_clip) : (int)(n % B), tid = threadIdx.x;
    const float *vf = verts + (size_t)n * V * 3;
    const bool do_nn = n >= nn_from;
    long long t_prev = 0;
    int n_phase = 0;
    auto phase_done = [&]() {
        if (stats && tid == 0 && do_nn) {
            const long long now = (long long)__builtin_readcyclecounter();
            if (n_phase > 0) atomicAdd(stats + 3 + n_phase, (unsigned long long)(now - t_prev));
            t_prev = now;
        }
        ++n_phase;
    };
    phase_done();
    float R[9] = {1.f, 0.f, 0.f, 0.f, 1.f, 0.f, 0.f, 0.f, 1.f}, tr[3] = {0.f, 0.f, 0.f};
    if constexpr (!OPT) {
#pragma unroll
        for (int k = 0; k < 9; ++k) R[k] = objR[n * 9 + k];
#pragma unroll
        for (int k = 0; k < 3; ++k) tr[k] = objT[n * 3 + k];
    }
    const int my_marker_pos = (!OPT && tid < M) ? markers_pos[tid] : 0;
    if (vorder && vrank) {
        for (int i0 = tid; i0 < V; i0 += 4 * CT) {
            typedef float f3v __attribute__((ext_vector_type(3), aligned(4)));
            int pos[4];
            f3v pv[4];
#pragma unroll
            for (int k = 0; k < 4; ++k) {
                const int i = min(i0 + k * CT, V - 1);
                pos[k] = vrank[i];
                pv[k] = *reinterpret_cast<const f3v *>(vf + 3 * i);
            }
#pragma unroll
            for (int k = 0; k < 4; ++k) {
                if (i0 + k * CT < V) {
                    lds_rec_store(vs, pos[k], pv[k].x, pv[k].y, pv[k].z);
                    reinterpret_cast<int *>(vs + 2 * (pos[k] >> 1) + 1)[2 + (pos[k] & 1)] = i0 + k * CT;
                }
            }
        }
        for (int v = V + tid; v < L.V4; v += CT) {
            lds_rec_store(vs, v, 3e18f, 3e18f, 3e18f);
            reinterpret_cast<int *>(vs + 2 * (v >> 1) + 1)[2 + (v & 1)] = 0x7fffffff;
        }
    } else
    for (int v0 = tid; v0 < L.V4; v0 += 4 * CT) {
        int o[4];
        float x[4], y[4], z[4];
#pragma unroll
        for (int k = 0; k < 4; ++k) {
            const int v = v0 + k * CT;
            o[k] = v < V ? (vorder ? vorder[v] : v) : -1;
        }
#pragma unroll
        for (int k = 0; k < 4; ++k) {
            x[k] = y[k] = z[k] = 3e18f;
            if (o[k] >= 0) {
                typedef float f3v __attribute__((ext_vector_type(3), aligned(4)));
                const f3v pv = *reinterpret_cast<const f3v *>(vf + 3 * o[k]);
                x[k] = pv.x; y[k] = pv.y; z[k] = pv.z;
            }
        }
#pragma unroll
        for (int k = 0; k < 4; ++k) {
            const int v = v0 + k * CT;
            if (v < L.V4) {
                lds_rec_store(vs, v, x[k], y[k], z[k]);
                reinterpret_cast<int *>(vs + 2 * (v >> 1) + 1)[2 + (v & 1)] = o[k] >= 0 ? o[k] : 0x7fffffff;
            }
        }
    }
    if (tid < MAXM) flags[tid] = 0;
    const int ntask_all = (P + TASK - 1) / TASK;
    const int task0 = (int)((long long)blockIdx.y * ntask_all / gridDim.y), task1 = (int)((long long)(blockIdx.y + 1) * ntask_all / gridDim.y);
    if (tid == 0) next_task = task0;
    for (int i = tid; i < MAXP; i += CT) pl[i] = 0.f;
    __syncthreads();
    phase_done();
    if (!OPT && tid < ((M + 1) & ~1)) {
        float3 mk = make_float3(3e18f, 3e18f, 3e18f);
        if (tid < M) {
            mk = lds_rec(vs, my_marker_pos);
            if (markers_out) {
                float *mo = markers_out + ((size_t)n * M + tid) * 3;
                mo[0] = mk.x; mo[1] = mk.y; mo[2] = mk.z;
            }
        }
        lds_rec_store(ms, tid, mk.x, mk.y, mk.z);
    }
    if (do_nn) {
#define IDF_DPP8(v, op, ctrl) v = op(v, __builtin_bit_cast(float, __builtin_amdgcn_update_dpp(__builtin_bit_cast(int, v), __builtin_bit_cast(int, v), ctrl, 0xf, 0xf, false)))
        const int lane_ = tid & 63, wave_ = tid >> 6, nsw = 2 * ((nSB + 2) / 2);
        for (int sb = wave_; sb < nsw; sb += CT / 64) {
            const int pr = sb * 64 + lane_;
            float lx = FLT_MAX, ly = FLT_MAX, lz = FLT_MAX, hx = -FLT_MAX, hy = -FLT_MAX, hz = -FLT_MAX;
            if (2 * pr < V) {
                const float4 xy = vs[2 * pr], zz = vs[2 * pr + 1];
                const bool two = 2 * pr + 1 < V;
                lx = two ? fminf(xy.x, xy.y) : xy.x; hx = two ? fmaxf(xy.x, xy.y) : xy.x;
                ly = two ? fminf(xy.z, xy.w) : xy.z; hy = two ? fmaxf(xy.z, xy.w) : xy.z;
                lz = two ? fminf(zz.x, zz.y) : zz.x; hz = two ? fmaxf(zz.x, zz.y) : zz.x;
            }
            IDF_DPP8(lx, fminf, 0xB1); IDF_DPP8(lx, fminf, 0x4E); IDF_DPP8(lx, fminf, 0x141);
            IDF_DPP8(ly, fminf, 0xB1); IDF_DPP8(ly, fminf, 0x4E); IDF_DPP8(ly, fminf, 0x141);
            IDF_DPP8(lz, fminf, 0xB1); IDF_DPP8(lz, fminf, 0x4E); IDF_DPP8(lz, fminf, 0x141);
            IDF_DPP8(hx, fmaxf, 0xB1); IDF_DPP8(hx, fmaxf, 0x4E); IDF_DPP8(hx, fmaxf, 0x141);
            IDF_DPP8(hy, fmaxf, 0xB1); IDF_DPP8(hy, fmaxf, 0x4E); IDF_DPP8(hy, fmaxf, 0x141);
            IDF_DPP8(hz, fmaxf, 0xB1); IDF_DPP8(hz, fmaxf, 0x4E); IDF_DPP8(hz, fmaxf, 0x141);
            const int cb = sb * SB + (lane_ >> 3);
            if ((lane_ & 7) == 0 && cb < nSB * SB) lds_box_store(bb, cb, make_float3(lx, ly, lz), make_float3(hx, hy, hz));
            const float slx = -wave_max(-lx), sly = -wave_max(-ly), slz = -wave_max(-lz), shx = wave_max(hx), shy = wave_max(hy), shz = wave_max(hz);
            if (lane_ == 0) lds_box_store(sbb, sb, make_float3(slx, sly, slz), make_float3(shx, shy, shz));
        }
#undef IDF_DPP8
        for (int k = tid; k < 2 * ((L.nSeed + 1) / 2); k += CT) {
            const float3 p = lds_rec(vs, min(k * SEED_STRIDE, nCB - 1) * CB);
            lds_rec_store(sd, k, p.x, p.y, p.z);
        }
    }
    const float *op = OPT ? pts_frame + (size_t)n * P * 3 : obj_points + (size_t)b * P * 3;
    const int ln = tid & 63, ntask = task1;
    __syncthreads();
    phase_done();
    float mind2 = FLT_MAX;
    unsigned n_exec = 0, n_test = 0, n_tasks = 0;
    for (;;) {
        int task = 0;
        if (ln == 0) task = atomicAdd(&next_task, 1);
        task = __builtin_amdgcn_readfirstlane(task);
        if (task >= ntask) break;
        ++n_tasks;
        const int sp = task * TASK + ln;
        const int i = sp < P ? (porder ? porder[(size_t)b * P + sp] : sp) : -1;
        const bool valid = i >= 0;
        float px = 0.f, py = 0.f, pz = 0.f;
        if (valid) { px = op[3 * i]; py = op[3 * i + 1]; pz = op[3 * i + 2]; }
        const float qx = OPT ? px : (px * R[0] + py * R[1] + pz * R[2]) + tr[0];
        const float qy = OPT ? py : (px * R[3] + py * R[4] + pz * R[5]) + tr[1];
        const float qz = OPT ? pz : (px * R[6] + py * R[7] + pz * R[8]) + tr[2];
        if (do_nn) {
#pragma clang fp contract(off)
            const v2f QX = v2f{qx, qx}, QY = v2f{qy, qy}, QZ = v2f{qz, qz};
            auto pair_d2 = [&](const float4 xy, const float4 zz) {
#pragma clang fp contract(off)
                const v2f dx = QX - v2f{xy.x, xy.y}, dy = QY - v2f{xy.z, xy.w}, dz = QZ - v2f{zz.x, zz.y};
                return (dx * dx + dy * dy) + dz * dz;
            };
            auto pair_a2 = [&](const float4 xy, const float2 zz) {
                const v2f dx = QX - v2f{xy.x, xy.y}, dy = QY - v2f{xy.z, xy.w}, dz = QZ - v2f{zz.x, zz.y};
                return __builtin_elementwise_fma(dz, dz, __builtin_elementwise_fma(dy, dy, dx * dx));
            };
            constexpr float SCAN_M = 1.000003814697265625f, SCAN_ABS = 1e-37f;
            float seed = FLT_MAX;
            for (int k = 0; k < (L.nSeed + 1) / 2; k += 4) {
                float4 xy[4]; float2 zz[4];
#pragma unroll
                for (int u = 0; u < 4; ++u) { xy[u] = sd[2 * min(k + u, (L.nSeed + 1) / 2 - 1)]; zz[u] = *reinterpret_cast<const float2 *>(&sd[2 * min(k + u, (L.nSeed + 1) / 2 - 1) + 1]); }
#pragma unroll
                for (int u = 0; u < 4; ++u) {
                    const v2f a2 = pair_a2(xy[u], zz[u]);
                    seed = fminf(fminf(seed, a2.x), a2.y);
                }
            }
            float thr = __builtin_fmaf(seed, SCAN_M, SCAN_ABS);
            float best = FLT_MAX, bthr = FLT_MAX;
            int tie = 0;
            int bblk = 0, bblk2 = 0;
            auto pair_lb = [&](const float4 a, const float4 bq, const float4 c) {
#pragma clang fp contract(off)
                const v2f ax = v2f{a.x, a.y} - QX, bx = QX - v2f{bq.z, bq.w};
                const v2f ay = v2f{a.z, a.w} - QY, by = QY - v2f{c.x, c.y};
                const v2f az = v2f{bq.x, bq.y} - QZ, bz = QZ - v2f{c.z, c.w};
                const v2f ex = v2f{fmaxf(fmaxf(ax.x, bx.x), 0.f), fmaxf(fmaxf(ax.y, bx.y), 0.f)};
                const v2f ey = v2f{fmaxf(fmaxf(ay.x, by.x), 0.f), fmaxf(fmaxf(ay.y, by.y), 0.f)};
                const v2f ez = v2f{fmaxf(fmaxf(az.x, bz.x), 0.f), fmaxf(fmaxf(az.y, bz.y), 0.f)};
                return __builtin_elementwise_fma(ez, ez, __builtin_elementwise_fma(ey, ey, ex * ex));
            };
            auto score_block = [&](int cb) {
                ++n_exec;
                const int v0 = cb * CB;
                float4 xy[CB / 2]; float2 zz[CB / 2];
#pragma unroll
                for (int u = 0; u < CB / 2; ++u) { xy[u] = vs[v0 + 2 * u]; zz[u] = *reinterpret_cast<const float2 *>(&vs[v0 + 2 * u + 1]); }
                float bm = FLT_MAX;
#pragma unroll
                for (int u = 0; u < CB / 2; ++u) {
                    const v2f a2 = pair_a2(xy[u], zz[u]);
                    bm = fminf(fminf(bm, a2.x), a2.y);
                }
                if (bm < best) {
                    const float w = __builtin_fmaf(bm, SCAN_M, SCAN_ABS);
                    if (best <= w) { tie = tie ? 2 : 1; bblk2 = bblk; } else tie = 0;
                    best = bm; bblk = v0; bthr = w; thr = fminf(thr, w);
                } else if (bm <= bthr) { tie = tie ? 2 : 1; bblk2 = v0; }
            };
            auto scan_super = [&](int sb) {
                const int cb0 = sb * SB;
#pragma unroll
                for (int j = 0; j < SB / 2; ++j) {
                    const int cb = cb0 + 2 * j;
                    const float4 *bx = bb + 3 * (cb >> 1);
                    const v2f lb = pair_lb(bx[0], bx[1], bx[2]);
                    n_test += 2;
                    if (__builtin_amdgcn_ballot_w64(valid && lb.x <= thr) != 0ull) score_block(cb);
                    if (__builtin_amdgcn_ballot_w64(valid && lb.y <= thr) != 0ull) score_block(cb + 1);
                }
            };
            if (!vorder) {
                for (int cb = 0; cb < nCB; ++cb) score_block(cb);
            } else
            for (int sb = 0; sb < nSB; sb += 2) {
                const float4 *bx = sbb + 3 * (sb >> 1);
                const v2f lb = pair_lb(bx[0], bx[1], bx[2]);
                n_test += 2;
                if (__builtin_amdgcn_ballot_w64(valid && lb.x <= thr) != 0ull) scan_super(sb);
                if (__builtin_amdgcn_ballot_w64(valid && lb.y <= thr) != 0ull) scan_super(sb + 1);
            }
            int pos = bblk, org = 0x7fffffff;
            float ebest = FLT_MAX;
            auto resolve_pair = [&](int pr) {
                const float4 xy = vs[2 * pr], zz = vs[2 * pr + 1];
                const v2f d2 = pair_d2(xy, zz);
                const int o0 = __builtin_bit_cast(int, zz.z), o1 = __builtin_bit_cast(int, zz.w);
                if (d2.x < ebest || (d2.x == ebest && o0 < org)) { ebest = d2.x; org = o0; pos = 2 * pr; }
                if (d2.y < ebest || (d2.y == ebest && o1 < org)) { ebest = d2.y; org = o1; pos = 2 * pr + 1; }
            };
            if (tie < 2) {
#pragma unroll
                for (int u = 0; u < CB / 2; ++u) resolve_pair((bblk >> 1) + u);
                if (tie) {
#pragma unroll
                    for (int u = 0; u < CB / 2; ++u) resolve_pair((bblk2 >> 1) + u);
                }
            } else {
                for (int pr = 0; pr < (V + 1) / 2; ++pr) resolve_pair(pr);
            }
            pos = min(pos, V - 1);
            if (org == 0x7fffffff) org = vorder ? vorder[pos] : pos;
            if constexpr (OPT) {
                if (valid) idx_out[(size_t)n * P + i] = org;
            } else if (valid) {
                const float3 v3 = lds_rec(vs, pos);
                float3 acc = make_float3(0.f, 0.f, 0.f);
                const int e0 = adj_ptr[org], e1 = adj_ptr[org + 1];
                if (adj_pair) {
                    for (int e = e0; e < e1; e += 4) {
                        int2 ab[4];
#pragma unroll
                        for (int u = 0; u < 4; ++u) ab[u] = *reinterpret_cast<const int2 *>(adj_pair + 2 * (size_t)min(e + u, e1 - 1));
#pragma unroll
                        for (int u = 0; u < 4; ++u) {
                            if (e + u < e1) {
                                const float3 nn = cross3(sub3(lds_rec(vs, ab[u].x), v3), sub3(lds_rec(vs, ab[u].y), v3));
                                acc.x += nn.x; acc.y += nn.y; acc.z += nn.z;
                            }
                        }
                    }
                } else {
                    for (int e = e0; e < e1; ++e) {
                        const int f = adj_face[e], c = adj_corner[e];
                        const float3 p0 = lds_rec(vs, faces[3 * f]), p1 = lds_rec(vs, faces[3 * f + 1]), p2 = lds_rec(vs, faces[3 * f + 2]);
                        float3 nn;
                        if (c == 1) nn = cross3(sub3(p2, p1), sub3(p0, p1));
                        else if (c == 2) nn = cross3(sub3(p0, p2), sub3(p1, p2));
                        else nn = cross3(sub3(p1, p0), sub3(p2, p0));
                        acc.x += nn.x; acc.y += nn.y; acc.z += nn.z;
                    }
                }
                const float nl = fmaxf(sqrtf(acc.x * acc.x + acc.y * acc.y + acc.z * acc.z), 1e-6f);
                const float vx = qx - v3.x, vy = qy - v3.y, vz = qz - v3.z;
                const float dt = (acc.x / nl) * vx + (acc.y / nl) * vy + (acc.z / nl) * vz;
                const float d = sqrtf(vx * vx + vy * vy + vz * vz);
                const float o2h = d * (dt > 0.f ? 1.f : (dt < 0.f ? -1.f : 0.f));
                if (o2h_out) o2h_out[(size_t)n * P + i] = o2h;
                if (idx_out) idx_out[(size_t)n * P + i] = org;
                pl[sp] = o2h < 0.f ? fabsf(o2h) * 20.0f : 0.f;
            }
        }
        if (!OPT && valid) {
#pragma clang fp contract(off)
            const v2f QX = v2f{qx, qx}, QY = v2f{qy, qy}, QZ = v2f{qz, qz};
            for (int p2 = 0; p2 < (M + 1) / 2; ++p2) {
                const float4 xy = ms[2 * p2], zz = ms[2 * p2 + 1];
                const v2f dx = v2f{xy.x, xy.y} - QX, dy = v2f{xy.z, xy.w} - QY, dz = v2f{zz.x, zz.y} - QZ;
                const v2f d2 = __builtin_elementwise_fma(dy, dy, dx * dx) + dz * dz;
                mind2 = fminf(fminf(mind2, d2.x), d2.y);
                if (__builtin_amdgcn_ballot_w64(fminf(d2.x, d2.y) < MARK_D2) != 0ull) {
                    if (d2.x < MARK_D2) flags[2 * p2] = 1;
                    if (d2.y < MARK_D2) flags[2 * p2 + 1] = 1;
                }
            }
        }
    }
    if (stats && ln == 0 && do_nn) {
        atomicAdd(stats, (unsigned long long)n_exec);
        atomicAdd(stats + 1, (unsigned long long)nCB * n_tasks);
        atomicAdd(stats + 2, (unsigned long long)n_test);
    }
    phase_done();
    if constexpr (OPT) return;
    __syncthreads();
    phase_done();
    float loss = 0.f;
#pragma unroll
    for (int k = 0; k < MAXP / CT; ++k) loss += pl[tid + CT * k];
    red[tid] = loss;
    __syncthreads();
    for (int s = CT / 2; s > 0; s >>= 1) {
        if (tid < s) red[tid] += red[tid + s];
        __syncthreads();
    }
    const float loss_total = red[0];
    __syncthreads();
    red[tid] = mind2;
    __syncthreads();
    for (int s = CT / 2; s > 0; s >>= 1) {
        if (tid < s) red[tid] = fminf(red[tid], red[tid + s]);
        __syncthreads();
    }
    if (tid == 0) { loss_sum[n] = loss_total; min_dist[n] = red[0] == FLT_MAX ? FLT_MAX : sqrtf(red[0]); }
    if (tid < M) label[(size_t)n * M + tid] = flags[tid];
    phase_done();
    if (stats && tid == 0 && do_nn) atomicAdd(stats + 3, 1ull);
}

size_t contact_lds_bytes(int V) { return (size_t)ContactLds(V).total * sizeof(float4); }

struct ContactArgs {
    const float *verts; int V;
    const float *obj_points; int P;
    int32_t *porder;
    const float *objR, *objT;
    const idf_correction_ctx *ctx;
    int B;
    float *markers, *loss_sum, *min_dist;
    int32_t *label;
    float *o2h;
    int32_t *idx;
    unsigned long long *stats;
    int64_t nn_from;
    const float *pts_frame; int frames_per_clip;
    PredArgs pred;
};

template <bool OPT, bool WITH_PRED>
int launch_contact(hipStream_t s, int64_t N, const ContactArgs &a) {
    static_assert(!(OPT && WITH_PRED), "the predictor rides with the hook's scan only");
    constexpr int SCAN_LDS_MAX = 160 * 1024 - 16384, LDS_LIMIT = WITH_PRED ? 160 * 1024 - 2048 : SCAN_LDS_MAX;
    const idf_correction_ctx *c = a.ctx;
    const size_t lds = contact_lds_bytes(a.V);
    if (lds > (size_t)SCAN_LDS_MAX || a.P > MAXP) return IDF_E_INVAL;
    const bool ordered = c->vorder != nullptr;
    if (OPT ? !ordered : (ordered != (c->faces_scan != nullptr) || ordered != (c->markers_scan != nullptr) || ordered != (c->adj_pair_scan != nullptr))) return IDF_E_INVAL;
    const int32_t *faces = OPT ? nullptr : ordered ? c->faces_scan : c->faces, *mpos = OPT ? nullptr : ordered ? c->markers_scan : c->markers_idx;
    const int32_t *adj_ptr = OPT ? nullptr : c->adj_ptr, *adj_face = OPT ? nullptr : c->adj_face, *adj_corner = OPT ? nullptr : c->adj_corner;
    const int32_t *adj_pair = OPT ? nullptr : c->adj_pair_scan;
    const int M = OPT ? 0 : c->n_markers;
    if (!OPT && a.porder) hipLaunchKernelGGL(corr_point_order_kernel, dim3((unsigned)a.B), dim3(1024), 0, s, a.obj_points, a.P, a.porder);
    const int nclips = WITH_PRED ? a.pred.nclips : 0;
    const size_t lds_launch = (nclips > 0 && lds < idf_objproj_dev::OBJPROJ_LDS) ? idf_objproj_dev::OBJPROJ_LDS : lds;
    if (lds_launch > (size_t)LDS_LIMIT) return IDF_E_INVAL;
    static std::atomic<uint64_t> lds_ok{0};
    if (idf_opt_in_lds(reinterpret_cast<const void *>(corr_contact_kernel<OPT, WITH_PRED>), LDS_LIMIT, lds_ok) != IDF_OK) return IDF_E_LAUNCH;
    hipLaunchKernelGGL((corr_contact_kernel<OPT, WITH_PRED>), OPT ? dim3((unsigned)N, 2) : dim3((unsigned)(N + nclips)), dim3(CT), lds_launch, s, a.verts, a.V,
                       a.obj_points, a.P, a.porder, a.objR, a.objT, faces, adj_ptr, adj_face, adj_corner, adj_pair, c->vorder, c->vrank, mpos, M, a.B,
                       a.markers, a.loss_sum, a.min_dist, a.label, a.o2h, a.idx, a.stats, a.nn_from, a.pts_frame, a.frames_per_clip, a.pred);
    return IDF_OK;
}

}
```

interdiff_amd/csrc/correction.hip:

```cpp
#include "common.h"
#include "objproj.h"
#include "rot_math.h"
#include <float.h>

namespace {

constexpr int NBODY = 22;
constexpr int CTOK = 144;

__global__ __launch_bounds__(256) void corr_prepare_kernel(const float *__restrict__ x0, const float *__restrict__ gt,
                                                           const float *__restrict__ hand_pose, int B, int T,
                                                           float *__restrict__ pose, float *__restrict__ trans,
                                                           float *__restrict__ objR, float *__restrict__ objT,
                                                           float *__restrict__ gt_angles, float *__restrict__ gt_trans) {
    const int64_t i = (int64_t)blockIdx.x * 256 + threadIdx.x;
    const int64_t N = (int64_t)B * T;
    if (i >= N * 24) return;
    const int64_t n = i / 24;
    const int slot = (int)(i - n * 24), t = (int)(n / B), b = (int)(n - (int64_t)t * B);
    const float *xb = x0 + (size_t)b * CTOK * T + t;
    if (slot < NBODY) {
        float d[6], m[9], a[3];
#pragma unroll
        for (int k = 0; k < 6; ++k) d[k] = xb[(size_t)(slot * 6 + k) * T];
        rot::rot6d_to_matrix(d, m);
        rot::matrix_to_axis_angle(m, a);
        float *p = pose + n * 156 + slot * 3;
        p[0] = a[0]; p[1] = a[1]; p[2] = a[2];
    } else if (slot == 22) {
        for (int k = 0; k < 90; ++k) pose[n * 156 + 66 + k] = hand_pose[n * 90 + k];
#pragma unroll
        for (int k = 0; k < 3; ++k) trans[n * 3 + k] = xb[(size_t)(132 + k) * T];
    } else {
        float d[6], m[9];
#pragma unroll
        for (int k = 0; k < 6; ++k) d[k] = xb[(size_t)(135 + k) * T];
        rot::rot6d_to_matrix(d, m);
#pragma unroll
        for (int k = 0; k < 9; ++k) objR[n * 9 + k] = m[k];
        const float *gb = gt + (size_t)b * CTOK * T + t;
#pragma unroll
        for (int k = 0; k < 3; ++k) {
            objT[n * 3 + k] = xb[(size_t)(141 + k) * T];
            gt_trans[n * 3 + k] = gb[(size_t)(141 + k) * T];
        }
#pragma unroll
        for (int k = 0; k < 6; ++k) gt_angles[n * 6 + k] = gb[(size_t)(135 + k) * T];
    }
}

}

#include "contact_scan.h"

namespace {

__global__ __launch_bounds__(128) void corr_reduce_kernel(const float *__restrict__ loss_sum, const float *__restrict__ min_dist,
                                                          const int32_t *__restrict__ label, int B, int T, int past, int P, int M,
                                                          uint8_t *__restrict__ condition, int32_t *__restrict__ contact,
                                                          float *__restrict__ distance_out, float *__restrict__ loss_out) {
    extern __shared__ float fr[];
    const int b = blockIdx.x, tid = threadIdx.x;
    for (int t = tid; t < T; t += 128) {
        fr[t] = loss_sum[(size_t)t * B + b];
        fr[T + t] = min_dist[(size_t)t * B + b];
    }
    if (tid < M) {
        int c = 0;
#pragma unroll 16
        for (int t = past; t < T; ++t) c += label[((size_t)t * B + b) * M + tid];
        contact[(size_t)b * M + tid] = c;
    }
    __syncthreads();
    if (tid == 0) {
        float ls = 0.f, ds = 0.f;
        for (int t = past; t < T; ++t) ls += fr[t] / (float)P;
        for (int t = 0; t < T; ++t) ds += fr[T + t];
        const float loss = ls / (float)(T - past), dist = ds / (float)T;
        condition[b] = !((loss < 0.002f) && (dist < 0.02f));
        if (distance_out) distance_out[b] = dist;
        if (loss_out) loss_out[b] = loss;
    }
}

__global__ __launch_bounds__(256) void corr_blend_kernel(float *__restrict__ x0, const float *__restrict__ proj,
                                                         const uint8_t *__restrict__ condition, int B, int T, float a,
                                                         const float *__restrict__ a_table, const int64_t *__restrict__ a_state) {
    if (a_table) a = a_table[a_state[0] * 4 + 3];
    const int64_t i = (int64_t)blockIdx.x * 256 + threadIdx.x;
    if (i >= (int64_t)B * CTOK * T) return;
    const int b = (int)(i / (CTOK * T)), r = (int)(i - (int64_t)b * CTOK * T), c = r / T, t = r - c * T;
    if (!condition[b]) return;
    const float x = x0[i];
    const float other = c < 135 ? x : proj[((size_t)t * B + b) * 9 + (c - 135)];
    x0[i] = a * x + (1.0f - a) * other;
}

struct CorrWs {
    float *pose, *trans, *objR, *objT, *gt_angles, *gt_trans, *verts, *jtr, *markers, *loss_sum, *min_dist, *proj, *proj_keep;
    int32_t *label, *contact, *porder;
    uint8_t *condition;
    void *smpl_ws;
    size_t smpl_ws_bytes, total;
};

CorrWs carve(const idf_correction_ctx *c, int B, int T, void *ws) {
    const int64_t N = (int64_t)B * T;
    const int V = c->smpl->V, J = c->smpl->J, M = c->n_markers;
    char *p = reinterpret_cast<char *>(ws);
    size_t off = 0;
    auto take = [&](size_t bytes) { char *r = p ? p + off : nullptr; off += idf_align(bytes); return r; };
    CorrWs w;
    w.pose = (float *)take(N * 156 * 4);
    w.trans = (float *)take(N * 3 * 4);
    w.objR = (float *)take(N * 9 * 4);
    w.objT = (float *)take(N * 3 * 4);
    w.gt_angles = (float *)take(N * 6 * 4);
    w.gt_trans = (float *)take(N * 3 * 4);
    w.verts = (float *)take((size_t)N * V * 3 * 4);
    w.jtr = (float *)take((size_t)N * J * 3 * 4);
    w.markers = (float *)take((size_t)N * M * 3 * 4);
    w.loss_sum = (float *)take(N * 4);
    w.min_dist = (float *)take(N * 4);
    w.proj = (float *)take(N * 9 * 4);
    w.label = (int32_t *)take((size_t)N * M * 4);
    w.contact = (int32_t *)take((size_t)B * M * 4);
    w.condition = (uint8_t *)take(B);
    w.porder = (int32_t *)take((size_t)B * c->n_points * 4);
    w.proj_keep = (float *)take((size_t)B * idf_objproj_keep_floats() * 4);
    w.smpl_ws_bytes = interdiff_smpl_workspace_bytes(c->smpl, N);
    w.smpl_ws = take(w.smpl_ws_bytes);
    w.total = off;
    return w;
}

}

#include "near_mask.h"

extern "C" size_t interdiff_correction_workspace_bytes(const idf_correction_ctx *c, int32_t B, int32_t T) {
    if (!c || !c->smpl || B <= 0 || T <= 0) return 0;
    return carve(c, B, T, nullptr).total;
}

static int correction_impl(const idf_correction_ctx *c, float *x0, const float *gt, const float *hand_pose,
                           const float *beta, const float *obj_points, int32_t B, int32_t T, float blend_t, const float *blend_table,
                           const int64_t *blend_state, uint8_t *condition, int32_t *contact, float *distance, float *loss, void *ws,
                           size_t ws_bytes, void *stream) {
    if (!c || !c->smpl || !c->objproj || !x0 || !gt || !hand_pose || !beta || !obj_points || !ws || B <= 0 || T <= 0) return IDF_E_INVAL;
    const int V = c->smpl->V, M = c->n_markers, P = c->n_points;
    if (c->smpl->J != 52 || c->smpl->n_betas != 10 || M > MAXM || M != c->objproj->P || P > MAXP || T != c->objproj->T ||
        c->past_len != c->objproj->past_len || c->past_len >= T)
        return IDF_E_INVAL;
    CorrWs w = carve(c, B, T, ws);
    if (ws_bytes < w.total) return IDF_E_NOMEM;
    hipStream_t s = idf_stream(stream);
    const int64_t N = (int64_t)B * T;
    const bool fused = (c->tune & 2) == 0 && idf_objproj_check(c->objproj) == IDF_OK;
    idf_prof_mark(IDF_K_CORR_PREPARE, s);
    hipLaunchKernelGGL(corr_prepare_kernel, dim3((unsigned)idf_cdiv(N * 24, 256)), dim3(256), 0, s, x0, gt, hand_pose, B, T, w.pose,
                       w.trans, w.objR, w.objT, w.gt_angles, w.gt_trans);
    int rc = interdiff_smpl_forward(c->smpl, w.pose, beta, w.trans, N, w.verts, w.jtr, nullptr, w.smpl_ws, w.smpl_ws_bytes, stream);
    if (rc) return rc;
    idf_prof_mark(IDF_K_CORR_CONTACT, s);
    ContactArgs a{};
    a.verts = w.verts; a.V = V;
    a.obj_points = obj_points; a.P = P;
    a.porder = w.porder;
    a.objR = w.objR; a.objT = w.objT;
    a.ctx = c;
    a.B = B;
    a.markers = fused ? nullptr : w.markers;
    a.loss_sum = w.loss_sum; a.min_dist = w.min_dist; a.label = w.label;
    a.nn_from = (int64_t)c->past_len * B;
    if (fused) {
        PredArgs &pred = a.pred;
        pred.op = *c->objproj;
        pred.obj_angles = w.gt_angles; pred.obj_trans = w.gt_trans;
        pred.markers_idx = c->markers_idx; pred.markers = w.markers; pred.keep = w.proj_keep;
        pred.nclips = B;
    }
    rc = launch_contact<false, true>(s, N, a);
    if (rc) return rc;
    uint8_t *cond = condition ? condition : w.condition;
    int32_t *cont = contact ? contact : w.contact;
    idf_prof_mark(IDF_K_CORR_REDUCE, s);
    hipLaunchKernelGGL(corr_reduce_kernel, dim3(B), dim3(128), 2 * (size_t)T * sizeof(float), s, w.loss_sum, w.min_dist, w.label, B, T, c->past_len, P, M, cond,
                       cont, distance, loss);
    if (fused) {
        idf_prof_mark(IDF_K_OBJPROJ, s);
        rc = idf_objproj_pick(c->objproj, w.proj_keep, cont, B, w.proj, s);
    } else {
        rc = interdiff_objprojector_sample(c->objproj, w.gt_angles, w.gt_trans, w.markers, cont, B, w.proj, stream);
    }
    if (rc) return rc;
    idf_prof_mark(IDF_K_CORR_BLEND, s);
    hipLaunchKernelGGL(corr_blend_kernel, dim3((unsigned)idf_cdiv((int64_t)B * CTOK * T, 256)), dim3(256), 0, s, x0, w.proj, cond, B, T,
                       blend_t, blend_table, blend_state);
    idf_prof_mark(-1, s);
    IDF_CHECK_LAUNCH();
    return IDF_OK;
}

extern "C" int interdiff_correction(const idf_correction_ctx *c, float *x0, const float *gt, const float *hand_pose,
                                    const float *beta, const float *obj_points, int32_t B, int32_t T, float blend_t,
                                    uint8_t *condition, int32_t *contact, float *distance, float *loss, void *ws,
                                    size_t ws_bytes, void *stream) {
    return correction_impl(c, x0, gt, hand_pose, beta, obj_points, B, T, blend_t, nullptr, nullptr, condition, contact, distance, loss, ws, ws_bytes, stream);
}

extern "C" int interdiff_correction_dev(const idf_correction_ctx *c, float *x0, const float *gt, const float *hand_pose,
                                        const float *beta, const float *obj_points, int32_t B, int32_t T, const float *table,
                                        const int64_t *state, void *ws, size_t ws_bytes, void *stream) {
    if (!table || !state) return IDF_E_INVAL;
    return correction_impl(c, x0, gt, hand_pose, beta, obj_points, B, T, 0.f, table, state, nullptr, nullptr, nullptr, nullptr, ws, ws_bytes, stream);
}

#include "corr_metrics.h"

static ContactArgs metrics_scan_args(const idf_correction_ctx *c, const MetWs &w, const float *verts, const float *obj_points, const float *objR, const float *objT, int B) {
    ContactArgs a{};
    a.verts = verts; a.V = c->smpl->V;
    a.obj_points = obj_points; a.P = c->n_points;
    a.porder = w.porder;
    a.objR = objR; a.objT = objT;
    a.ctx = c;
    a.B = B;
    a.markers = w.markers; a.loss_sum = w.loss_sum; a.min_dist = w.min_dist; a.label = w.label;
    return a;
}

extern "C" size_t interdiff_contact_nn_workspace_bytes(const idf_correction_ctx *c, int32_t B, int32_t T) {
    if (!c || B <= 0 || T <= 0) return 0;
    return carve_metrics(c, B, T, nullptr).total;
}

extern "C" int interdiff_contact_nn(const idf_correction_ctx *c, const float *verts, const float *obj_points, const float *objR,
                                    const float *objT, int32_t B, int32_t T, float *o2h, int32_t *idx, uint64_t *stats, void *ws,
                                    size_t ws_bytes, void *stream) {
    if (!c || !c->smpl || !verts || !obj_points || !objR || !objT || !ws || B <= 0 || T <= 0 || (!o2h && !idx)) return IDF_E_INVAL;
    if (c->n_markers > MAXM || c->n_points > MAXP) return IDF_E_INVAL;
    MetWs w = carve_metrics(c, B, T, ws);
    if (ws_bytes < w.total) return IDF_E_NOMEM;
    hipStream_t s = idf_stream(stream);
    if (stats && hipMemsetAsync(stats, 0, IDF_CONTACT_STATS * sizeof(uint64_t), s) != hipSuccess) return IDF_E_LAUNCH;
    ContactArgs a = metrics_scan_args(c, w, verts, obj_points, objR, objT, B);
    a.o2h = o2h ? o2h : w.o2h; a.idx = idx;
    a.stats = reinterpret_cast<unsigned long long *>(stats);
    const int rc = launch_contact<false, false>(s, (int64_t)B * T, a);
    if (rc) return rc;
    IDF_CHECK_LAUNCH();
    return IDF_OK;
}

extern "C" size_t interdiff_metrics_workspace_bytes(const idf_correction_ctx *c, int32_t B, int32_t T) {
    if (!c || B <= 0 || T <= 0) return 0;
    return carve_metrics(c, B, T, nullptr).total;
}

extern "C" int interdiff_metrics(const idf_correction_ctx *c, const float *obj_pred, const float *jtr, const float *body_trans,
                                 const float *obj_gt, const float *jtr_gt, const float *body_trans_gt, const float *verts,
                                 const float *obj_points, int32_t B, int32_t T, int32_t J, float *out6, void *ws, size_t ws_bytes,
                                 void *stream) {
    if (!c || !c->smpl || !obj_pred || !jtr || !body_trans || !obj_gt || !jtr_gt || !body_trans_gt || !verts || !obj_points || !out6 ||
        !ws || B <= 0 || T <= 0 || J <= 0)
        return IDF_E_INVAL;
    const int M = c->n_markers, P = c->n_points;
    if (M > MAXM || P > MAXP) return IDF_E_INVAL;
    MetWs w = carve_metrics(c, B, T, ws);
    if (ws_bytes < w.total) return IDF_E_NOMEM;
    hipStream_t s = idf_stream(stream);
    const int64_t N = (int64_t)B * T;
    idf_prof_mark(IDF_K_OTHER, s);
    hipLaunchKernelGGL(metrics_prepare_kernel, dim3((unsigned)idf_cdiv(N, 256)), dim3(256), 0, s, obj_pred, N, w.objR, w.objT);
    ContactArgs a = metrics_scan_args(c, w, verts, obj_points, w.objR, w.objT, B);
    a.o2h = w.o2h;
    const int rc = launch_contact<false, false>(s, N, a);
    if (rc) return rc;
    hipLaunchKernelGGL(metrics_reduce_kernel, dim3(B), dim3(256), 0, s, obj_pred, jtr, body_trans, obj_gt, jtr_gt, body_trans_gt, w.o2h, B,
                       T, J, P, out6);
    idf_prof_mark(-1, s);
    IDF_CHECK_LAUNCH();
    return IDF_OK;
}

int idf_point_order(hipStream_t s, const float *obj_points, int B, int P, int32_t *porder) {
    if (P > MAXP) return IDF_E_INVAL;
    hipLaunchKernelGGL(corr_point_order_kernel, dim3((unsigned)B), dim3(1024), 0, s, obj_points, P, porder);
    return IDF_OK;
}

int idf_nn_scan_opt(hipStream_t s, int64_t N, int frames_per_clip, const float *verts, int V, const float *pts_frame, const float *obj_points, int P,
                    const int32_t *porder, const idf_correction_ctx *c, int32_t *yidx) {
    ContactArgs a{};
    a.verts = verts; a.V = V;
    a.obj_points = obj_points; a.P = P;
    a.porder = const_cast<int32_t *>(porder);
    a.ctx = c;
    a.B = (int)(N / frames_per_clip);
    a.idx = yidx;
    a.pts_frame = pts_frame; a.frames_per_clip = frames_per_clip;
    return launch_contact<true, false>(s, N, a);
}

int idf_near_mask_opt(hipStream_t s, int64_t N, int frames_per_clip, const float *verts, int V, const float *pts_frame, int P, const int32_t *porder,
                      const int32_t *vorder, float *psort, float *pbox, int32_t *near) {
    return launch_near_mask(s, N, frames_per_clip, verts, V, pts_frame, P, porder, vorder, psort, pbox, near);
}
```

interdiff_amd/csrc/smpl.hip:

```cpp
#include "common.h"
#include "rot_math.h"
#include <algorithm>

#ifndef IDF_SMPL_STAMP
#define IDF_SMPL_STAMP(i) do { } while (0)
#endif

namespace {

constexpr int MAXJ = 64;

__global__ __launch_bounds__(64) void smpl_pose_kernel(const idf_smpl_model m, const float *__restrict__ pose,
                                                       const float *__restrict__ betas, const float *__restrict__ trans,
                                                       float *__restrict__ feat, float *__restrict__ A,
                                                       float *__restrict__ jtr) {
    __shared__ float Rs[MAXJ * 9], Js[MAXJ * 3], Gs[MAXJ * 12];
    const int64_t n = blockIdx.x;
    const int j = threadIdx.x, J = m.J, nb = m.n_betas, KB = m.KB;
    const float *beta = betas + n * nb;
    if (j < J) {
        rot::rodrigues_smpl(pose + n * 3 * J + 3 * j, Rs + j * 9);
#pragma unroll
        for (int c = 0; c < 3; ++c) {
            float s = m.jt[j * 3 + c];
            const float *jsr = m.js + (size_t)(j * 3 + c) * nb;
            for (int k = 0; k < nb; ++k) s += jsr[k] * beta[k];
            Js[j * 3 + c] = s;
        }
    }
    float *f = feat + n * KB;
    if (j >= 1 && j < J) {
#pragma unroll
        for (int e = 0; e < 9; ++e) f[(j - 1) * 9 + e] = Rs[j * 9 + e] - ((e == 0 || e == 4 || e == 8) ? 1.0f : 0.0f);
    }
    const int base = 9 * (J - 1);
    for (int k = j; k < KB - base; k += 64) f[base + k] = k < nb ? beta[k] : (k == nb ? 1.0f : 0.0f);
    __syncthreads();
    if (j < 12) {
        const int r = j >> 2, c = j & 3;
        Gs[j] = c < 3 ? Rs[r * 3 + c] : Js[r];
    }
    __syncthreads();
    for (int i = 1; i < J; ++i) {
        const int p = m.parents[i];
        if (j < 12) {
            const int r = j >> 2, c = j & 3;
            const float *gp = Gs + p * 12 + r * 4;
            float v;
            if (c < 3)
                v = gp[0] * Rs[i * 9 + c] + gp[1] * Rs[i * 9 + 3 + c] + gp[2] * Rs[i * 9 + 6 + c];
            else
                v = gp[0] * (Js[i * 3] - Js[p * 3]) + gp[1] * (Js[i * 3 + 1] - Js[p * 3 + 1]) +
                    gp[2] * (Js[i * 3 + 2] - Js[p * 3 + 2]) + gp[3];
            Gs[i * 12 + j] = v;
        }
        __syncthreads();
    }
    if (j < J) {
        const float *g = Gs + j * 12;
        const float jx = Js[j * 3], jy = Js[j * 3 + 1], jz = Js[j * 3 + 2];
        float *a = A + ((size_t)n * J + j) * 12;
#pragma unroll
        for (int r = 0; r < 3; ++r) {
            a[r * 4 + 0] = g[r * 4 + 0];
            a[r * 4 + 1] = g[r * 4 + 1];
            a[r * 4 + 2] = g[r * 4 + 2];
            a[r * 4 + 3] = g[r * 4 + 3] - (g[r * 4] * jx + g[r * 4 + 1] * jy + g[r * 4 + 2] * jz);
            jtr[((size_t)n * J + j) * 3 + r] = g[r * 4 + 3] + trans[n * 3 + r];
        }
    }
}

constexpr int FT = 32, VT = 64, NTC = 3 * VT;
constexpr int BT = 256;
constexpr int FM = FT / 16;
constexpr int STS = NTC + 1;
constexpr int SF = 16;
constexpr int TBF = 10, TBV = 4;

template <int NG>
__global__ __launch_bounds__(BT) void smpl_blend_skin_kernel(const idf_smpl_model m, const float *__restrict__ feat,
                                                              const float *__restrict__ A, const float *__restrict__ trans,
                                                              int64_t N, float *__restrict__ verts,
                                                              float *__restrict__ v_posed) {
    extern __shared__ __attribute__((aligned(16))) float sm[];
    idf_args_now(m.V, m.J, m.S, m.blend, m.skin_idx, m.skin_w, feat, A, trans, N, verts, v_posed, gridDim.x);
    constexpr int KB = 16 * NG, nq = KB / 4;
    const int V = m.V, J = m.J, S = m.S;
    float *As = sm, *stage = sm;
    const int tid = threadIdx.x, lane = tid & 63, wave = (tid >> 6) & 3, fh = tid >> 8, li = lane & 15, kq = lane >> 4;
    const int nft = (int)((N + FT - 1) / FT), nvt = (V + VT - 1) / VT;
    const int nwg = gridDim.x, id = blockIdx.x;
    const int xq = nwg >> 3, xr = nwg & 7, xcd = id & 7;
    const int lid = (xcd < xr ? xcd * (xq + 1) : xr * (xq + 1) + (xcd - xr) * xq) + (id >> 3);
    const int blk = lid / (TBF * TBV), wi = lid - blk * (TBF * TBV);
    const int nvb = (nvt + TBV - 1) / TBV;
    const int ftile = blk / nvb * TBF + wi % TBF, vtile = blk % nvb * TBV + wi / TBF;
    if (ftile >= nft || vtile >= nvt) return;
    const int64_t f0 = (int64_t)ftile * FT;
    const int v0 = vtile * VT;
    IDF_SMPL_STAMP(0);

    {
        const uint32_t as_lds = idf_lds_addr(As);
        const int ncell = FT * nq;
        for (int i = wave; i * 64 < ncell; i += BT / 64) {
            const int p = min(i * 64 + lane, ncell - 1), row = p / nq, pos = p - row * nq;
            idf_dma16_v(feat + (size_t)min(f0 + row, N - 1) * KB + ((pos ^ ((row >> 1) & 7)) << 2), as_lds + (uint32_t)(i * 1024));
        }
    }
    const int vl = tid & 63, vme = v0 + vl;
    float sw[4];
    int so[4];
#pragma unroll
    for (int k = 0; k < 4; ++k) {
        const size_t e = (size_t)min(vme, V - 1) * S + min(k, S - 1);
        sw[k] = m.skin_w[e];
        so[k] = m.skin_idx[e] * 12;
    }
#pragma unroll
    for (int k = 0; k < 4; ++k) {
        const bool ok = k < S && vme < V;
        sw[k] = ok ? sw[k] : 0.f;
        so[k] = ok ? so[k] : 0;
    }
    asm volatile("s_waitcnt vmcnt(0)" ::: "memory");
    __syncthreads();
    IDF_SMPL_STAMP(1);

    const float *brow[3];
#pragma unroll
    for (int t = 0; t < 3; ++t) brow[t] = m.blend + ((size_t)((vtile * 4 + wave) * 3 + t) * NG * 64 + lane) * 4;
    f32x4 acc[FM][3];
#pragma unroll
    for (int i = 0; i < FM; ++i)
#pragma unroll
        for (int t = 0; t < 3; ++t) acc[i][t] = f32x4{0.f, 0.f, 0.f, 0.f};
    constexpr int PD = 3;
    float4 bq[PD + 1][3];
    auto ldg = [&](float4 (&dst)[3], int gi) {
#pragma unroll
        for (int t = 0; t < 3; ++t) dst[t] = *reinterpret_cast<const float4 *>(brow[t] + gi * 256);
    };
    auto mac = [&](const float4 (&bc)[3], int gi) {
#pragma unroll
        for (int i = 0; i < FM; ++i) {
            const int row = (fh * FM + i) * 16 + li;
            const float4 a = *reinterpret_cast<const float4 *>(As + row * KB + (((gi * 4 + kq) ^ ((row >> 1) & 7)) << 2));
#pragma unroll
            for (int t = 0; t < 3; ++t) acc[i][t] = __builtin_amdgcn_mfma_f32_16x16x4f32(a.x, bc[t].x, acc[i][t], 0, 0, 0);
#pragma unroll
            for (int t = 0; t < 3; ++t) acc[i][t] = __builtin_amdgcn_mfma_f32_16x16x4f32(a.y, bc[t].y, acc[i][t], 0, 0, 0);
#pragma unroll
            for (int t = 0; t < 3; ++t) acc[i][t] = __builtin_amdgcn_mfma_f32_16x16x4f32(a.z, bc[t].z, acc[i][t], 0, 0, 0);
#pragma unroll
            for (int t = 0; t < 3; ++t) acc[i][t] = __builtin_amdgcn_mfma_f32_16x16x4f32(a.w, bc[t].w, acc[i][t], 0, 0, 0);
        }
    };
#pragma unroll
    for (int g = 0; g < PD && g < NG; ++g) ldg(bq[g], g);
#pragma unroll
    for (int g = 0; g < NG; ++g) {
        if (g + PD < NG) ldg(bq[(g + PD) % (PD + 1)], g + PD);
        __builtin_amdgcn_sched_barrier(0);
        mac(bq[g % (PD + 1)], g);
        __builtin_amdgcn_sched_barrier(0);
    }
    __syncthreads();
    IDF_SMPL_STAMP(2);
#pragma unroll
    for (int i = 0; i < FM; ++i)
#pragma unroll
        for (int t = 0; t < 3; ++t)
#pragma unroll
            for (int r = 0; r < 4; ++r) stage[((fh * FM + i) * 16 + kq * 4 + r) * STS + (wave * 3 + t) * 16 + li] = acc[i][t][r];

    float *Asub = sm + ((FT * STS + 255) & ~255);
    float *ost = Asub + ((SF * J * 12 + 255) & ~255);
    float *trs = ost + SF * NTC;
    const int arow = J * 12;
    if (tid < FT * 3) trs[tid] = trans[min(f0 + tid / 3, N - 1) * 3 + tid % 3];
    for (int sub = 0; sub < FT / SF; ++sub) {
        const int64_t fs = f0 + sub * SF;
        if (fs >= N) break;
        __syncthreads();
        {
            const uint32_t asub_lds = idf_lds_addr(Asub);
            const float *src = idf_uniform_ptr(A + (size_t)fs * arow);
            for (int i = wave; i * 256 < SF * arow; i += BT / 64) idf_dma16_s(src + (size_t)i * 256, (uint32_t)(lane << 4), asub_lds + (uint32_t)(i * 1024));
            asm volatile("s_waitcnt vmcnt(0)" ::: "memory");
        }
        __syncthreads();
        IDF_SMPL_STAMP(3 + 3 * sub);
#pragma unroll
        for (int k = 0; k < SF * VT / BT; ++k) {
            const int f = (tid >> 6) + (BT / 64) * k, fr = sub * SF + f;
            const float px = stage[fr * STS + 3 * vl], py = stage[fr * STS + 3 * vl + 1], pz = stage[fr * STS + 3 * vl + 2];
            float4 t0 = make_float4(0.f, 0.f, 0.f, 0.f), t1 = t0, t2 = t0;
            const float *Af = Asub + f * arow;
#pragma unroll
            for (int b = 0; b < 4; ++b) {
                if (b < S) {
                    const float w = sw[b];
                    const float4 *a = reinterpret_cast<const float4 *>(Af + so[b]);
                    const float4 a0 = a[0], a1 = a[1], a2 = a[2];
                    t0.x = fmaf(w, a0.x, t0.x); t0.y = fmaf(w, a0.y, t0.y); t0.z = fmaf(w, a0.z, t0.z); t0.w = fmaf(w, a0.w, t0.w);
                    t1.x = fmaf(w, a1.x, t1.x); t1.y = fmaf(w, a1.y, t1.y); t1.z = fmaf(w, a1.z, t1.z); t1.w = fmaf(w, a1.w, t1.w);
                    t2.x = fmaf(w, a2.x, t2.x); t2.y = fmaf(w, a2.y, t2.y); t2.z = fmaf(w, a2.z, t2.z); t2.w = fmaf(w, a2.w, t2.w);
                }
            }
            float *o = ost + f * NTC + 3 * vl;
            o[0] = fmaf(t0.x, px, fmaf(t0.y, py, fmaf(t0.z, pz, t0.w))) + trs[fr * 3 + 0];
            o[1] = fmaf(t1.x, px, fmaf(t1.y, py, fmaf(t1.z, pz, t1.w))) + trs[fr * 3 + 1];
            o[2] = fmaf(t2.x, px, fmaf(t2.y, py, fmaf(t2.z, pz, t2.w))) + trs[fr * 3 + 2];
        }
        __syncthreads();
        IDF_SMPL_STAMP(4 + 3 * sub);
        const int nvalid = min(VT, V - v0) * 3;
        for (int idx = tid; idx < SF * (NTC / 2); idx += BT) {
            const int f = idx / (NTC / 2), c2 = (idx - f * (NTC / 2)) * 2;
            if (fs + f >= N || c2 >= nvalid) continue;
            const size_t go = ((size_t)(fs + f) * V + v0) * 3 + c2;
            *reinterpret_cast<float2 *>(verts + go) = *reinterpret_cast<const float2 *>(ost + f * NTC + c2);
            if (v_posed) *reinterpret_cast<float2 *>(v_posed + go) = make_float2(stage[(sub * SF + f) * STS + c2], stage[(sub * SF + f) * STS + c2 + 1]);
        }
        IDF_SMPL_STAMP(5 + 3 * sub);
    }
}

}

extern "C" size_t interdiff_smpl_workspace_bytes(const idf_smpl_model *m, int64_t N) {
    if (!m || N < 0) return 0;
    return idf_align((size_t)N * m->KB * sizeof(float)) + idf_align(((size_t)N + SF) * m->J * 12 * sizeof(float));
}

extern "C" int interdiff_smpl_forward(const idf_smpl_model *m, const float *pose, const float *betas, const float *trans,
                                      int64_t N, float *verts, float *jtr, float *v_posed, void *ws, size_t ws_bytes,
                                      void *stream) {
    if (!m || !pose || !betas || !trans || !verts || !jtr || !ws || N < 0) return IDF_E_INVAL;
    if (m->J < 1 || m->J > MAXJ || m->KB % 16 != 0 || m->KB < 9 * (m->J - 1) + m->n_betas + 1 || m->S < 1) return IDF_E_INVAL;
    if (ws_bytes < interdiff_smpl_workspace_bytes(m, N)) return IDF_E_NOMEM;
    if (N == 0) return IDF_OK;
    hipStream_t s = idf_stream(stream);
    float *feat = reinterpret_cast<float *>(ws);
    float *A = reinterpret_cast<float *>(reinterpret_cast<char *>(ws) + idf_align((size_t)N * m->KB * sizeof(float)));
    idf_prof_mark(IDF_K_SMPL_POSE, s);
    hipLaunchKernelGGL(smpl_pose_kernel, dim3((unsigned)N), dim3(64), 0, s, *m, pose, betas, trans, feat, A, jtr);
    const size_t lds = std::max((size_t)FT * m->KB, (size_t)((FT * STS + 255) & ~255) + ((SF * m->J * 12 + 255) & ~255) + (size_t)SF * NTC + FT * 3) * sizeof(float);
    if (lds > 150 * 1024 || m->KB % 32 != 0 || (m->V * 3) % 2 != 0 || m->S > 4) return IDF_E_INVAL;
    if (m->KB != 480) return IDF_E_INVAL;
    static std::atomic<uint64_t> lds_ok{0};
    if (lds > 64 * 1024 && idf_opt_in_lds(reinterpret_cast<const void *>(smpl_blend_skin_kernel<30>), 150 * 1024, lds_ok) != IDF_OK) return IDF_E_LAUNCH;
    idf_prof_mark(IDF_K_SMPL_BLEND_SKIN, s);
    const unsigned nwg_launch = (unsigned)(idf_cdiv(idf_cdiv(N, FT), TBF) * idf_cdiv(idf_cdiv(m->V, VT), TBV) * TBF * TBV);
    hipLaunchKernelGGL(smpl_blend_skin_kernel<30>, dim3(nwg_launch), dim3(BT), lds, s, *m,
                       feat, A, trans, N, verts, v_posed);
    idf_prof_mark(-1, s);
    IDF_CHECK_LAUNCH();
    return IDF_OK;
}
```

interdiff_amd/diffusion.py:

```python
import itertools
import math
import os
import numpy as np
import torch
from . import _lib
from . import graph_sampler


def get_named_beta_schedule(schedule_name, num_diffusion_timesteps, scale_betas=1.):
    n = num_diffusion_timesteps
    if schedule_name == 'linear':
        scale = scale_betas * 1000 / n
        return np.linspace(scale * 0.0001, scale * 0.02, n, dtype=np.float64)
    if schedule_name == 'cosine':
        abar = lambda t: math.cos((t + 0.008) / 1.008 * math.pi / 2) ** 2
        return np.array([min(1 - abar((i + 1) / n) / abar(i / n), 0.999) for i in range(n)], dtype=np.float64)
    raise NotImplementedError('unknown beta schedule: %s' % schedule_name)


GRAPH_BLOCKS = (49, 7, 1)
SPLIT_MAX_BATCH = int(os.environ.get('INTERDIFF_SPLIT_MAX_BATCH', 128))
N_CHAINS = int(os.environ.get('INTERDIFF_CHAINS', 2))
MAX_GRAPH_SHAPES = 8
_UID = itertools.count(1)


def fresh_seed():
    return int(torch.randint(0, 2 ** 62, (1,), dtype=torch.int64).item())


def mask_operands(mask, gt, like):
    if mask is None or gt is None:
        return None, None
    assert like.shape == mask.shape == gt.shape
    return (mask if mask.dtype == torch.uint8 else mask.view(torch.uint8)).contiguous(), gt.contiguous()


def inpaint(x, gt, mask_u8):
    _lib.check(_lib.load().interdiff_inpaint(_lib.dptr(x, torch.float32), _lib.dptr(gt, torch.float32), _lib.dptr(mask_u8), x.numel(), _lib.stream()), 'inpaint')


def seeded_state(t_start, seed, elem0):
    return torch.tensor([t_start, 0, int(seed) & 0x7FFFFFFFFFFFFFFF, 0, 0, 0, elem0, 0], dtype=torch.int64)


def space_timesteps(num_timesteps, section_counts):
    if isinstance(section_counts, str):
        if section_counts.startswith('ddim'):
            want = int(section_counts[len('ddim'):])
            for stride in range(1, num_timesteps):
                if len(range(0, num_timesteps, stride)) == want:
                    return set(range(0, num_timesteps, stride))
            raise ValueError('cannot create exactly %d steps with an integer stride' % num_timesteps)
        section_counts = [int(c) for c in section_counts.split(',')]
    size_per, extra = divmod(num_timesteps, len(section_counts))
    start, kept = 0, []
    for k, count in enumerate(section_counts):
        size = size_per + (1 if k < extra else 0)
        if size < count:
            raise ValueError('cannot divide section of %d steps into %d' % (size, count))
        stride = 1 if count <= 1 else (size - 1) / (count - 1)
        kept += [start + round(cur) for cur in _strided(stride, count)]
        start += size
    return set(kept)


def _strided(stride, count):
    cur = 0.0
    for _ in range(count):
        yield cur
        cur += stride


def ddim_coefficients(alphas_cumprod, alphas_cumprod_prev, eta):
    ab, abp = np.asarray(alphas_cumprod, np.float64), np.asarray(alphas_cumprod_prev, np.float64)
    sigma = float(eta) * np.sqrt((1.0 - abp) / (1.0 - ab)) * np.sqrt(1.0 - ab / abp)
    k = np.sqrt(np.maximum(1.0 - abp - sigma ** 2, 0.0)) / np.sqrt(1.0 / ab - 1.0)
    return np.sqrt(abp) - k, k * np.sqrt(1.0 / ab), sigma


class GaussianDiffusion:

    def __init__(self, betas):
        betas = np.array(betas, dtype=np.float64)
        assert betas.ndim == 1 and (betas > 0).all() and (betas <= 1).all()
        self.betas = betas
        self.num_timesteps = int(betas.shape[0])
        alphas = 1.0 - betas
        self.alphas_cumprod = np.cumprod(alphas, axis=0)
        self.alphas_cumprod_prev = np.append(1.0, self.alphas_cumprod[:-1])
        self.posterior_variance = betas * (1.0 - self.alphas_cumprod_prev) / (1.0 - self.alphas_cumprod)
        self.posterior_log_variance_clipped = np.log(np.append(self.posterior_variance[1], self.posterior_variance[1:]))
        self.posterior_mean_coef1 = betas * np.sqrt(self.alphas_cumprod_prev) / (1.0 - self.alphas_cumprod)
        self.posterior_mean_coef2 = (1.0 - self.alphas_cumprod_prev) * np.sqrt(alphas) / (1.0 - self.alphas_cumprod)
        self._c1 = self.posterior_mean_coef1.astype(np.float32)
        self._c2 = self.posterior_mean_coef2.astype(np.float32)
        self._sigma = np.exp(np.float32(0.5) * self.posterior_log_variance_clipped.astype(np.float32)).astype(np.float32)
        self.sqrt_alphas_cumprod = np.sqrt(self.alphas_cumprod)
        self.sqrt_one_minus_alphas_cumprod = np.sqrt(1.0 - self.alphas_cumprod)
        self.timestep_map = list(range(self.num_timesteps))
        self.original_num_steps = self.num_timesteps
        self.identity_tmap_is_null = True
        self._t_cache = {}
        self._tables = {}
        self._rows_cache = {}
        self._tmaps = {}
        self._q_tables = {}
        self.fuse_plain_step = True
        self.chain_plain_steps = os.environ.get('INTERDIFF_CHAIN_STEPS', '1') != '0'
        self.split_chains = True
        self.split_min_rows = None
        self._uid = next(_UID)

    @property
    def is_respaced(self):
        return self.timestep_map != list(range(self.num_timesteps))

    def _timesteps(self, B, device, loop_side=False):
        key = (B, str(device), bool(loop_side) and self.is_respaced)
        if key not in self._t_cache:
            vals = torch.tensor(self.timestep_map, dtype=torch.int64) if not key[2] and self.is_respaced else torch.arange(self.num_timesteps, dtype=torch.int64)
            self._t_cache[key] = vals.to(device)[:, None].repeat(1, B).contiguous()
        return self._t_cache[key]

    def _tmap(self, device):
        if not self.is_respaced and self.identity_tmap_is_null:
            return None
        key = str(device)
        if key not in self._tmaps:
            self._tmaps[key] = torch.tensor(self.timestep_map, dtype=torch.int64).to(device)
        return self._tmaps[key]

    def _rows(self, sampler=('ddpm',)):
        if sampler not in self._rows_cache:
            if sampler[0] == 'ddpm':
                c1, c2, sig = self._c1, self._c2, self._sigma.copy()
            else:
                c1, c2, sig = (v.astype(np.float32) for v in ddim_coefficients(self.alphas_cumprod, self.alphas_cumprod_prev, sampler[1]))
            sig[0] = 0.0
            blend = (np.arange(self.num_timesteps, dtype=np.float32) / np.float32(1000)).astype(np.float32)
            self._rows_cache[sampler] = np.ascontiguousarray(np.stack([c1, c2, sig, blend], axis=1).astype(np.float32))
        return self._rows_cache[sampler]

    def _table(self, device, sampler=('ddpm',)):
        key = (str(device), sampler)
        if key not in self._tables:
            self._tables[key] = torch.from_numpy(self._rows(sampler)).to(device)
        return self._tables[key]

    def _step(self, model, img, x0_buf, i, it, t, model_kwargs, denoised_fn, noise_i, seed, elem0=0, rows_kw={}, t_hook=None, rows=None):
        lib = _lib.load()
        y = model_kwargs.get('y', {})
        x0 = model(img, t, **model_kwargs, **rows_kw)
        mu8, gc = mask_operands(y.get('inpainting_mask'), y.get('inpainted_motion'), x0)
        if mu8 is not None:
            inpaint(x0, gc, mu8)
        if denoised_fn is not None:
            x0 = denoised_fn(x0, t if t_hook is None else t_hook, model_kwargs)
        c1, c2, sigma = (float(v) for v in (self._rows() if rows is None else rows)[i, :3])
        _lib.check(lib.interdiff_posterior_step_at(_lib.dptr(img, torch.float32), _lib.dptr(x0, torch.float32),
                                                   _lib.dptr(noise_i, torch.float32, allow_none=True), img.numel(),
                                                   c1, c2, sigma, seed, it, elem0, _lib.stream()),
                   'posterior_step')
        return x0

    def p_sample_loop(self, model, shape, noise=None, clip_denoised=True, denoised_fn=None, cond_fn=None, model_kwargs=None,
                      device=None, progress=False, skip_timesteps=0, init_image=None, randomize_class=False,
                      cond_fn_with_grad=False, dump_steps=None, const_noise=False, step_noise=None, seed=None, n_steps=None,
                      use_graph=True, first_t=None, shard=None):
        return self._sample_loop(('ddpm',), model, shape, noise, clip_denoised, denoised_fn, cond_fn, model_kwargs, device, skip_timesteps,
                                 init_image, randomize_class, cond_fn_with_grad, dump_steps, const_noise, step_noise, seed, n_steps, use_graph,
                                 first_t, shard)

    def ddim_sample_loop(self, model, shape, noise=None, clip_denoised=True, denoised_fn=None, cond_fn=None, model_kwargs=None,
                         device=None, progress=False, eta=0.0, skip_timesteps=0, init_image=None, randomize_class=False,
                         cond_fn_with_grad=False, dump_steps=None, const_noise=False, step_noise=None, seed=None, n_steps=None,
                         use_graph=True, first_t=None, shard=None):
        return self._sample_loop(('ddim', float(eta)), model, shape, noise, clip_denoised, denoised_fn, cond_fn, model_kwargs, device,
                                 skip_timesteps, init_image, randomize_class, cond_fn_with_grad, dump_steps, const_noise, step_noise, seed,
                                 n_steps, use_graph, first_t, shard)

    def _sample_loop(self, sampler, model, shape, noise, clip_denoised, denoised_fn, cond_fn, model_kwargs, device, skip_timesteps, init_image,
                     randomize_class, cond_fn_with_grad, dump_steps, const_noise, step_noise, seed, n_steps, use_graph, first_t, shard):
        if clip_denoised:
            raise NotImplementedError('clip_denoised=True is not used on the eval path (eval_smpl_short.py:153)')
        if cond_fn is not None or skip_timesteps or init_image is not None or randomize_class or cond_fn_with_grad or const_noise:
            raise NotImplementedError('only noise=, denoised_fn=, model_kwargs=, dump_steps= are live (SURVEY.md §8(b))')
        if model_kwargs is None:
            model_kwargs = {}
        if seed is None:
            seed = fresh_seed()
        if device is None:
            device = next(model.parameters()).device
        assert isinstance(shape, (tuple, list))
        if shard is not None:
            shard = (int(shard[0]), int(shard[1]))
            if not 0 <= shard[0] <= shard[0] + shape[0] <= shard[1]:
                raise ValueError('shard=(first_clip, total_clips) must contain this batch of %d clips' % shape[0])
        first, total = (0, shape[0]) if shard is None else shard
        per_clip = int(np.prod(shape[1:]))
        elem0 = first * per_clip
        if shard is not None and elem0 % 4:
            raise ValueError('a shard must start at a multiple of 4 elements (C * T = %d per clip)' % per_clip)
        if noise is not None:
            img = noise.clone().contiguous().float()
        else:
            img = torch.empty(*shape, dtype=torch.float32, device=device)
            _lib.check(_lib.load().interdiff_randn_at(_lib.dptr(img), img.numel(), seed, 0xFFFFFFFF, elem0, _lib.stream()), 'randn')
            y = model_kwargs.get('y', {})
            mu8, gc = mask_operands(y.get('inpainting_mask'), y.get('inpainted_motion'), img) if sampler[0] == 'ddpm' else (None, None)
            if mu8 is not None:
                inpaint(img, gc, mu8)
        t_first = self.num_timesteps - 1 if first_t is None else int(first_t)
        if not 0 <= t_first < self.num_timesteps:
            raise ValueError('first_t outside the schedule')
        todo = t_first + 1 if n_steps is None else min(int(n_steps), t_first + 1)
        if (step_noise is None and use_graph and getattr(model, 'graph_safe', False) and img.is_cuda
                and 'cond' in model_kwargs.get('y', {}) and os.environ.get('INTERDIFF_NO_GRAPH') != '1'):
            return graph_sampler.sample(self, model, img, model_kwargs, denoised_fn, seed, todo, dump_steps, t_first, shard, sampler)
        rows_kw = {'batch_rows': total * shape[-1]} if shard is not None and getattr(model, 'accepts_batch_rows', False) else {}
        ts, ts_hook, rows = self._timesteps(shape[0], device), self._timesteps(shape[0], device, loop_side=True), self._rows(sampler)
        dump = []
        cond = model_kwargs.get('y', {}).get('cond') if isinstance(model_kwargs.get('y', None), dict) else None
        if cond is not None and hasattr(model, 'prepare_memory'):
            model.prepare_memory(cond)
        for it, i in enumerate(range(t_first, t_first - todo, -1)):
            t, th = ts[i], ts_hook[i]
            t.host_value = th.host_value = i
            if step_noise is None:
                nz = None
            elif callable(step_noise):
                nz = step_noise(it, img).contiguous()
            else:
                nz = step_noise[it]
            self._step(model, img, None, i, it, t, model_kwargs, denoised_fn, nz, seed, elem0, rows_kw, th, rows)
            if dump_steps is not None and it in dump_steps:
                dump.append(img.clone())
        return dump if dump_steps is not None else img

    def sample_timesteps(self, B, device, generator=None):
        gdev = generator.device if generator is not None else device
        t = torch.randint(0, self.num_timesteps, (B,), dtype=torch.int64, device=gdev, generator=generator).to(device)
        return t, torch.ones(B, dtype=torch.float32, device=device)

    def q_sample(self, x_start, t, noise=None, seed=None, inpainted_motion=None, inpainting_mask=None, elem0=0):
        lib = _lib.load()
        x0 = x_start.contiguous()
        if x0.dtype != torch.float32:
            raise ValueError('x_start must be float32')
        B = x0.shape[0]
        if tuple(t.shape) != (B,):
            raise ValueError('t must be [B]')
        if not t.is_cuda:
            if int(t.min()) < 0 or int(t.max()) >= self.num_timesteps:
                raise ValueError('t outside the schedule')
            t = t.to(x0.device)
        key = str(x0.device)
        if key not in self._q_tables:
            self._q_tables[key] = tuple(torch.from_numpy(v.astype(np.float32)).to(x0.device) for v in (self.sqrt_alphas_cumprod, self.sqrt_one_minus_alphas_cumprod))
        sa, s1 = self._q_tables[key]
        if (inpainted_motion is None) != (inpainting_mask is None):
            raise ValueError('inpainted_motion and inpainting_mask go together')
        mu8, gc = mask_operands(inpainting_mask, inpainted_motion, x0)
        if noise is not None:
            assert noise.shape == x0.shape
            noise = noise.contiguous()
        elif seed is None:
            seed = fresh_seed()
        x_t = torch.empty_like(x0)
        _lib.check(lib.interdiff_q_sample(_lib.dptr(x_t), _lib.dptr(x0), _lib.dptr(noise, torch.float32, allow_none=True),
                                          _lib.dptr(t.contiguous(), torch.int64), _lib.dptr(sa), _lib.dptr(s1), self.num_timesteps,
                                          _lib.dptr(gc, torch.float32, allow_none=True), _lib.dptr(mu8, allow_none=True), B, x0.numel() // B,
                                          int(seed or 0) & 0xFFFFFFFFFFFFFFFF, int(elem0), _lib.stream()), 'q_sample')
        return x_t

    def training_losses(self, model, x_start, t, model_kwargs=None, noise=None, seed=None):
        if model_kwargs is None:
            model_kwargs = {}
        y = model_kwargs.get('y', {})
        both = 'inpainting_mask' in y and 'inpainted_motion' in y
        x_t = self.q_sample(x_start, t, noise=noise, seed=seed, inpainted_motion=y['inpainted_motion'] if both else None,
                            inpainting_mask=y['inpainting_mask'] if both else None)
        t = t.to(x_t.device)
        if self.is_respaced:
            t = torch.tensor(self.timestep_map, dtype=torch.int64, device=x_t.device)[t]
        model_output = model(x_t, t, **model_kwargs)
        assert model_output.shape == x_start.shape
        return model_output, x_start


def sample_loop(diffusion, model, shape, sampler='ddpm', eta=0.0, **kw):
    if sampler == 'ddpm':
        return diffusion.p_sample_loop(model, shape, **kw)
    if sampler == 'ddim':
        return diffusion.ddim_sample_loop(model, shape, eta=eta, **kw)
    raise ValueError("sampler must be 'ddpm' or 'ddim'")


class SpacedDiffusion(GaussianDiffusion):

    def __init__(self, use_timesteps, betas, rescale_timesteps=False):
        if rescale_timesteps:
            raise NotImplementedError('rescale_timesteps=True is not built (the reference configuration is False: model/diffusion_smpl.py:258)')
        base = GaussianDiffusion(betas)
        self.use_timesteps = set(use_timesteps)
        last, new_betas, tmap = 1.0, [], []
        for i, ac in enumerate(base.alphas_cumprod):
            if i in self.use_timesteps:
                new_betas.append(1 - ac / last)
                last = ac
                tmap.append(i)
        super().__init__(np.array(new_betas))
        self.timestep_map, self.original_num_steps, self.rescale_timesteps = tmap, len(base.betas), False


def create_gaussian_diffusion(noise_schedule='cosine', diffusion_steps=1000, timestep_respacing=''):
    betas = get_named_beta_schedule(noise_schedule, diffusion_steps, 1.)
    if not timestep_respacing:
        timestep_respacing = [diffusion_steps]
    return SpacedDiffusion(space_timesteps(diffusion_steps, timestep_respacing), betas)
```

interdiff_amd/graph_sampler.py:

```python
import os
import torch
from . import _lib, diffusion

HOOK_KEYS = ('hand_pose', 'beta', 'obj_points')


def plan_steps(t_start, todo, active, dump_steps, fuse_hook):
    blocks = diffusion.GRAPH_BLOCKS
    dumps = () if dump_steps is None else dump_steps
    ops, i, it, end = [], t_start, 0, t_start - todo
    while i > end:
        if active(i):
            ops.append(('hook', 0) if fuse_hook else ('eager_hook',))
            k = 1
        else:
            run = 1
            while i - run > end and not active(i - run) and (it + run - 1) not in dumps:
                run += 1
            k = next(b for b in blocks if b <= run)
            if fuse_hook and k == run and i - run > end and active(i - run) and (it + k - 1) not in dumps:
                ops.append(('hook', k))
                k += 1
            else:
                ops.append(('plain', k))
        i -= k
        it += k
        if (it - 1) in dumps:
            ops.append(('dump', it - 1))
    return ops


def capture(enqueue, *args):
    g = torch.cuda.CUDAGraph()
    with torch.cuda.graph(g):
        enqueue(*args)
    return g


def posterior_update(x, x0, gt, mask, table, state, ts, tmap=None):
    _lib.check(_lib.load().interdiff_posterior_step_dev_map(_lib.dptr(x), _lib.dptr(x0), _lib.dptr(gt, allow_none=True), _lib.dptr(mask, allow_none=True),
                                                            x.numel(), _lib.dptr(table), _lib.dptr(tmap, torch.int64, allow_none=True), _lib.dptr(state),
                                                            _lib.dptr(ts), ts.numel(), _lib.stream()),
               'posterior_step_dev')


class Chain:

    def __init__(self, model, entry, sl, own_state):
        dev, h, mem_len = entry.x.device, sl.stop - sl.start, entry.cond.shape[0]
        self.sl = sl
        self.x, self.ts = entry.x[sl], entry.ts[sl]
        self.gt = None if entry.gt is None else entry.gt[sl]
        self.mask = None if entry.mask is None else entry.mask[sl]
        self.kwargs = {} if entry.zpo is None else {'zero_pose_obj': entry.zpo[sl]}
        self.state = torch.zeros(8, dtype=torch.int64, device=dev) if own_state else entry.state
        self.cond = torch.empty(mem_len, h, entry.cond.shape[2], device=dev)
        self.memctx = torch.empty(model.memctx_floats(h, mem_len), dtype=torch.float32, device=dev)
        self.ws = torch.empty(model.workspace_bytes(h, entry.x.shape[-1]), dtype=torch.uint8, device=dev)
        self.stream = torch.cuda.Stream(dev)


class HookBuffers:

    def __init__(self, hook, entry, y, shapes):
        B, T = entry.x.shape[0], entry.x.shape[-1]
        self.shapes = shapes
        self.ws = hook.workspace_for(B, T)
        self.y = {k: torch.empty(y[k].shape, dtype=torch.float32, device=entry.x.device) for k in HOOK_KEYS}
        self.y['inpainted_motion'] = entry.gt if entry.gt is not None else torch.empty_like(entry.x)
        self.fresh = True


class Entry:

    def __init__(self, img, cond, has_mask, zpo):
        dev = img.device
        self.x, self.x0 = torch.zeros_like(img), torch.empty_like(img)
        self.ts = torch.zeros(img.shape[0], dtype=torch.int64, device=dev)
        self.state = torch.zeros(8, dtype=torch.int64, device=dev)
        self.cond = torch.empty_like(cond, memory_format=torch.contiguous_format)
        self.gt = torch.empty_like(img) if has_mask else None
        self.mask = torch.empty(img.shape, dtype=torch.uint8, device=dev) if has_mask else None
        self.zpo = None if zpo is None else torch.empty(zpo.shape, dtype=torch.float32, device=dev)
        self.kwargs = {'y': {'cond': self.cond}}
        if zpo is not None:
            self.kwargs['zero_pose_obj'] = self.zpo
        self.graphs = {}
        self.chains = []
        self.hooks = {}
        self.chain_steps = None
        self.pool_keys = ()

    @staticmethod
    def of(model, key, img, cond, has_mask, zpo):
        cache = model.__dict__.setdefault('_graph_cache', {})
        entry = cache.get(key)
        if entry is not None:
            return entry, False
        entry = Entry(img, cond, has_mask, zpo)
        if len(cache) >= diffusion.MAX_GRAPH_SHAPES:
            evicted = list(cache.values())
            cache.clear()
            for old in evicted:
                model.forget_shape_buffers(old.pool_keys)
        cache[key] = entry
        return entry, True

    def load(self, cond, zpo, gt, mask):
        self.cond.copy_(cond)
        if zpo is not None:
            self.zpo.copy_(zpo)
        if mask is not None:
            self.gt.copy_(gt)
            self.mask.copy_(mask)

    def warm_up(self, model, table, rows, tmap=None):
        model(self.x, self.ts, out=self.x0, **self.kwargs, batch_rows=rows)
        if model.supports_forward_step:
            t0 = min(2, table.shape[0] - 1)
            x, ts, state = self.x.clone(), self.ts.clone(), diffusion.seeded_state(t0, 1, 0).to(self.x.device)
            model.forward_step(x, ts, table, state, gt=self.gt, mask=self.mask, tmap=tmap, **self.kwargs, batch_rows=rows)
            if model.step_chaining:
                state.copy_(diffusion.seeded_state(t0, 1, 0))
                ts.copy_(self.ts)
                model.forward_step(x, ts, table, state, gt=self.gt, mask=self.mask, tmap=tmap, embed_next=True, **self.kwargs, batch_rows=rows)
                model.forward_step(x, ts, table, state, gt=self.gt, mask=self.mask, tmap=tmap, embed_ready=True, **self.kwargs, batch_rows=rows)
        torch.cuda.synchronize(self.x.device)

    def split_into_chains(self, model, n):
        B = self.x.shape[0]
        for c in range(n):
            start = c * (B // n) + min(c, B % n)
            self.chains.append(Chain(model, self, slice(start, start + B // n + (1 if c < B % n else 0)), own_state=c > 0))

    def hook_buffers(self, hook, y, table):
        shapes = tuple(tuple(y[k].shape) for k in HOOK_KEYS)
        hk = self.hooks.get(hook._uid)
        if hk is None or hk.shapes != shapes:
            hk = self.hooks[hook._uid] = HookBuffers(hook, self, y, shapes)
            for stale in [gk for gk in self.graphs if isinstance(gk, tuple) and gk[0] == 'hook' and gk[1] == hook._uid]:
                del self.graphs[stale]
        for k in HOOK_KEYS + (() if self.gt is not None else ('inpainted_motion',)):
            hk.y[k].copy_(y[k])
        if hk.fresh:
            hook.apply_dev(hk.y['inpainted_motion'].clone(), table, torch.zeros(8, dtype=torch.int64, device=self.x.device), hk.y, hk.ws)
            torch.cuda.synchronize(self.x.device)
            hk.fresh = False
        return hk


def hook_capturable(hook, y):
    return (hook is not None and getattr(hook, 'graph_capturable', False) and getattr(hook, 'debug', None) is None
            and getattr(hook, 'is_active', None) is not None and all(k in y for k in ('inpainted_motion',) + HOOK_KEYS)
            and os.environ.get('INTERDIFF_EAGER_HOOK') != '1')


def hook_gate(hook):
    if hook is None:
        return lambda t: False
    return getattr(hook, 'is_active', None) or (lambda t: True)


class Run:

    def __init__(self, model, entry, table, rows, fused, split, hook, hk, tmap=None):
        self.model, self.entry, self.table, self.rows, self.tmap = model, entry, table, rows, tmap
        self.fused, self.split, self.hook, self.hk = fused, split, hook, hk

    def enqueue_forward(self):
        st = self.entry
        self.model(st.x, st.ts, out=st.x0, **st.kwargs, batch_rows=self.rows)

    def enqueue_plain(self, k):
        st, model = self.entry, self.model
        links = [dict(embed_ready=i > 0, embed_next=i + 1 < k) if st.chain_steps else {} for i in range(k)]
        if self.split:
            cur = torch.cuda.current_stream()
            for ch in st.chains:
                ch.stream.wait_stream(cur)
                with torch.cuda.stream(ch.stream):
                    for link in links:
                        model.forward_step(ch.x, ch.ts, self.table, ch.state, gt=ch.gt, mask=ch.mask, tmap=self.tmap, memctx=ch.memctx, ws=ch.ws, batch_rows=self.rows, **link, **ch.kwargs)
            for ch in st.chains:
                cur.wait_stream(ch.stream)
        elif self.fused:
            for link in links:
                model.forward_step(st.x, st.ts, self.table, st.state, gt=st.gt, mask=st.mask, tmap=self.tmap, **link, **st.kwargs, batch_rows=self.rows)
        else:
            for _ in links:
                self.enqueue_forward()
                posterior_update(st.x, st.x0, st.gt, st.mask, self.table, st.state, st.ts, self.tmap)

    def finish_hook_step(self, x0):
        st = self.entry
        posterior_update(st.x, x0, None, None, self.table, st.state, st.ts, self.tmap)
        if self.split:
            for ch in st.chains[1:]:
                ch.state[:6].copy_(st.state[:6])

    def enqueue_hook_block(self, k):
        st = self.entry
        if k:
            self.enqueue_plain(k)
        self.enqueue_forward()
        if st.mask is not None:
            diffusion.inpaint(st.x0, st.gt, st.mask)
        self.hook.apply_dev(st.x0, self.table, st.state, self.hk.y, self.hk.ws)
        self.finish_hook_step(st.x0)

    def graph(self, key, enqueue, *args):
        graphs = self.entry.graphs
        if key not in graphs:
            graphs[key] = capture(enqueue, *args)
        return graphs[key]

    def plain_block(self, k):
        return self.graph((k, self.fused, self.split), self.enqueue_plain, k)

    def hook_block(self, k):
        return self.graph(('hook', self.hook._uid, k, self.fused, self.split), self.enqueue_hook_block, k)

    def eager_hook_step(self, t, model_kwargs):
        st = self.entry
        self.graph('fwd', self.enqueue_forward).replay()
        if st.mask is not None:
            diffusion.inpaint(st.x0, st.gt, st.mask)
        self.finish_hook_step(self.hook(st.x0, t, model_kwargs).contiguous())

    def play(self, plan, t_start, ts_all, model_kwargs):
        st, dump, i = self.entry, [], t_start
        for op in plan:
            if op[0] == 'plain':
                self.plain_block(op[1]).replay()
                i -= op[1]
            elif op[0] == 'hook':
                self.hook_block(op[1]).replay()
                i -= op[1] + 1
            elif op[0] == 'eager_hook':
                t = ts_all[i]
                t.host_value = i
                self.eager_hook_step(t, model_kwargs)
                i -= 1
            else:
                dump.append(st.x.clone())
        return dump


def sample(diff, model, img, model_kwargs, hook, seed, todo, dump_steps, t_start, shard=None, sampler=('ddpm',)):
    y = model_kwargs.get('y', {})
    B, T, dev = img.shape[0], img.shape[-1], img.device
    first, total = (0, B) if shard is None else shard
    per_clip = img.numel() // B
    elem0 = first * per_clip
    rows = total * T
    table, tmap = diff._table(dev, sampler), diff._tmap(dev)
    mask, gt = diffusion.mask_operands(y.get('inpainting_mask'), y.get('inpainted_motion'), img)
    cond, zpo = y['cond'], model_kwargs.get('zero_pose_obj')
    key = (diff._uid, tuple(img.shape), mask is not None, tuple(cond.shape), model.ffn_graph_key(rows)) + (() if sampler == ('ddpm',) and tmap is None else (sampler, tmap is not None))
    if zpo is not None:
        key += (tuple(zpo.shape),)
    st, fresh = Entry.of(model, key, img, cond, mask is not None, zpo)
    st.load(cond, zpo, gt, mask)
    pools_before = model.shape_buffer_keys() if fresh else None
    model.prepare_memory(st.cond)
    if fresh:
        st.warm_up(model, table, rows, tmap)
        st.pool_keys = model.shape_buffer_keys() - pools_before

    fused = diff.fuse_plain_step and model.supports_forward_step
    nch = diffusion.N_CHAINS
    split = (fused and diff.split_chains and nch > 1 and 2 * nch <= B <= diffusion.SPLIT_MAX_BATCH
             and B * T > (model.one_chain_max_rows() if diff.split_min_rows is None else diff.split_min_rows))
    if split:
        if not st.chains:
            st.split_into_chains(model, nch)
        for ch in st.chains:
            ch.cond.copy_(st.cond[:, ch.sl])
            model.prepare_memory(ch.cond, into=ch.memctx)
    chain_steps = diff.chain_plain_steps and fused and model.step_chaining
    if st.chain_steps != chain_steps:
        st.graphs.clear()
        st.chain_steps = chain_steps
    fuse_hook = hook_capturable(hook, y)
    run = Run(model, st, table, rows, fused, split, hook, st.hook_buffers(hook, y, table) if fuse_hook else None, tmap)

    st.x.copy_(img)
    st.state.copy_(diffusion.seeded_state(t_start, seed, elem0))
    if split:
        for ch in st.chains[1:]:
            ch.state.copy_(diffusion.seeded_state(t_start, seed, elem0 + ch.sl.start * per_clip))
    st.ts.fill_(diff.timestep_map[t_start])
    dump = run.play(plan_steps(t_start, todo, hook_gate(hook), dump_steps, fuse_hook), t_start, diff._timesteps(B, dev, loop_side=True), model_kwargs)
    return dump if dump_steps is not None else st.x.clone()
```

interdiff_amd/smpl.py:

```python
import ctypes as C
import numpy as np
import torch
from . import _lib


def _np(a):
    return a.detach().cpu().numpy() if isinstance(a, torch.Tensor) else np.asarray(a)


def pack_smpl_model(model, device):
    vt = _np(model['v_template']).astype(np.float64).reshape(-1, 3)
    sdirs = _np(model['shapedirs']).astype(np.float64)
    pdirs = _np(model['posedirs']).astype(np.float64)
    jreg = _np(model['J_regressor']).astype(np.float64)
    wts = _np(model['weights']).astype(np.float32)
    parents = _np(model['parents']).astype(np.int64).copy()
    V, J, nb = vt.shape[0], wts.shape[1], sdirs.shape[2]
    kp = 9 * (J - 1)
    if pdirs.shape != (V, 3, kp) or jreg.shape != (J, V):
        raise ValueError('inconsistent SMPL buffers')
    KB = (kp + nb + 1 + 15) // 16 * 16
    blend = np.zeros((3 * V, KB), np.float32)
    blend[:, :kp] = pdirs.reshape(3 * V, kp)
    blend[:, kp:kp + nb] = sdirs.reshape(3 * V, nb)
    blend[:, kp + nb] = vt.reshape(3 * V)
    jt = (jreg @ vt).astype(np.float32)
    js = np.einsum('jv,vck->jck', jreg, sdirs).astype(np.float32)
    nnz = (wts != 0)
    S = max(1, int(nnz.sum(1).max()))
    skin_idx = np.zeros((V, S), np.int32)
    skin_w = np.zeros((V, S), np.float32)
    for v in range(V):
        js_ = np.nonzero(nnz[v])[0]
        skin_idx[v, :len(js_)] = js_
        skin_w[v, :len(js_)] = wts[v, js_]
    parents[0] = 0
    t = lambda a: torch.from_numpy(np.ascontiguousarray(a)).to(device)
    nvt = -(-V // 64)
    rows = np.zeros((nvt * 192, KB), np.float32)
    rows[:3 * V] = blend
    frag = rows.reshape(nvt, 4, 3, 16, KB // 16, 4, 4).transpose(0, 1, 2, 4, 5, 3, 6)
    bufs = dict(blend=t(frag), blend_rows=t(blend), jt=t(jt), js=t(js), parents=t(parents.astype(np.int32)), skin_idx=t(skin_idx), skin_w=t(skin_w))
    m = _lib.SmplModel()
    m.V, m.J, m.n_betas, m.KB, m.S = V, J, nb, KB, S
    for k, v in bufs.items():
        if k != 'blend_rows':
            setattr(m, k, v.data_ptr())
    return m, bufs


class SMPL_Layer:
    def __init__(self, model, device='cuda'):
        self.lib = _lib.load()
        self.device = torch.device(device)
        self.cmodel, self._bufs = pack_smpl_model(model, self.device)
        self.th_faces = torch.from_numpy(_np(model['faces']).astype(np.int64)).to(self.device)
        self.v_template = _np(model['v_template']).astype(np.float32).reshape(-1, 3)
        self.num_joints = self.cmodel.J
        self.kintree_parents = [int(p) for p in _np(model['parents'])]
        self._ws = None

    def _workspace(self, N):
        need = self.lib.interdiff_smpl_workspace_bytes(C.byref(self.cmodel), N)
        if self._ws is None or self._ws.numel() < need:
            self._ws = torch.empty(max(need, 256), dtype=torch.uint8, device=self.device)
        return self._ws

    def forward(self, th_pose_axisang, th_betas=None, th_trans=None, th_offsets=None, scale=1., want_v_posed=True):
        if th_offsets is not None or scale != 1.:
            raise NotImplementedError('th_offsets / scale are not used on the eval_smpl_short path')
        N = th_pose_axisang.shape[0]
        J, V, nb = self.cmodel.J, self.cmodel.V, self.cmodel.n_betas
        if th_pose_axisang.shape[1] != 3 * J:
            raise ValueError('pose must be [N,%d]' % (3 * J))
        if th_betas is None:
            th_betas = torch.zeros(N, nb, device=self.device)
        if th_trans is None:
            th_trans = torch.zeros(N, 3, device=self.device)
        pose, betas, trans = (a.contiguous().float() for a in (th_pose_axisang, th_betas, th_trans))
        verts = torch.empty(N, V, 3, dtype=torch.float32, device=self.device)
        jtr = torch.empty(N, J, 3, dtype=torch.float32, device=self.device)
        v_posed = torch.empty(N, V, 3, dtype=torch.float32, device=self.device) if want_v_posed else None
        ws = self._workspace(N)
        _lib.check(self.lib.interdiff_smpl_forward(C.byref(self.cmodel), _lib.dptr(pose, torch.float32), _lib.dptr(betas, torch.float32),
                                                   _lib.dptr(trans, torch.float32), N, _lib.dptr(verts), _lib.dptr(jtr),
                                                   _lib.dptr(v_posed, allow_none=True), _lib.dptr(ws), ws.numel(), _lib.stream()),
                   'smpl_forward')
        return verts, jtr, v_posed, v_posed

    __call__ = forward
```

Before: 7.156 million.

## Precompute deduplicated SMPL blend base per sample and reuse it across denoising steps

Adds a per-sample prepare stage that finds frames with bit-identical hand pose and betas. It gathers the unique rows, computes their SMPL blend-shape base once, and records a per-frame base index and the object point order. During each correction step the SMPL forward then runs only the suffix from that cached base, and the point-order kernel is skipped. This cuts repeated blend GEMM work across steps. In exchange it adds a host sync in prepare, a host-side header map keyed by workspace pointer, and a path that only engages when duplication is high (unique rows at most N/4).

```diff
diff --git a/include/interdiff_hip.h b/include/interdiff_hip.h
--- a/include/interdiff_hip.h
+++ b/include/interdiff_hip.h
@@ -37,6 +37,12 @@
 int interdiff_smpl_forward(const idf_smpl_model *m, const float *pose, const float *betas,
                            const float *trans, int64_t N, float *verts, float *jtr,
                            float *v_posed, void *ws, size_t ws_bytes, void *stream);
+size_t interdiff_smpl_base_floats(const idf_smpl_model *m);
+int interdiff_smpl_blend_base(const idf_smpl_model *m, const float *pose, const float *betas, const float *trans, int64_t U, float *base,
+                              float *jtr, void *ws, size_t ws_bytes, void *stream);
+int interdiff_smpl_forward_from_base(const idf_smpl_model *m, const float *pose, const float *betas, const float *trans, int64_t N,
+                                     const float *base, const int32_t *base_id, float *verts, float *jtr, float *v_posed, void *ws,
+                                     size_t ws_bytes, void *stream);
 
 int interdiff_vertex_normals(const float *verts, int64_t N, int32_t V, const int32_t *faces,
                              const int32_t *adj_ptr, const int32_t *adj_face,
@@ -225,6 +231,9 @@
 int interdiff_correction_dev(const idf_correction_ctx *c, float *x0, const float *gt, const float *hand_pose,
                              const float *beta, const float *obj_points, int32_t B, int32_t T, const float *table,
                              const int64_t *state, void *ws, size_t ws_bytes, void *stream);
+int interdiff_correction_prepare(const idf_correction_ctx *c, const float *hand_pose, const float *beta, const float *obj_points, int32_t B,
+                                 int32_t T, void *ws, size_t ws_bytes, void *stream);
+int interdiff_correction_prepare_info(const idf_correction_ctx *c, int32_t B, int32_t T, const void *ws, int64_t *info4);
 
 #define IDF_CONTACT_STATS 12
 size_t interdiff_contact_nn_workspace_bytes(const idf_correction_ctx *c, int32_t B, int32_t T);
diff --git a/interdiff_amd/_lib.py b/interdiff_amd/_lib.py
--- a/interdiff_amd/_lib.py
+++ b/interdiff_amd/_lib.py
@@ -140,6 +140,9 @@
     'interdiff_rotation_6d_to_axis_angle': (C.c_int, [vp, vp, i64, vp]),
     'interdiff_smpl_workspace_bytes': (sz, [C.POINTER(SmplModel), i64]),
     'interdiff_smpl_forward': (C.c_int, [C.POINTER(SmplModel), vp, vp, vp, i64, vp, vp, vp, vp, sz, vp]),
+    'interdiff_smpl_base_floats': (sz, [C.POINTER(SmplModel)]),
+    'interdiff_smpl_blend_base': (C.c_int, [C.POINTER(SmplModel), vp, vp, vp, i64, vp, vp, vp, sz, vp]),
+    'interdiff_smpl_forward_from_base': (C.c_int, [C.POINTER(SmplModel), vp, vp, vp, i64, vp, vp, vp, vp, vp, vp, sz, vp]),
     'interdiff_vertex_normals': (C.c_int, [vp, i64, i32, vp, vp, vp, vp, vp, vp]),
     'interdiff_nn_argmin': (C.c_int, [vp, i32, vp, i32, i64, vp, vp]),
     'interdiff_point2point_signed': (C.c_int, [vp, i32, vp, i32, i64, vp, vp, vp, vp, vp, vp, vp, vp, vp]),
@@ -186,6 +189,8 @@
     'interdiff_correction': (C.c_int, [C.POINTER(CorrectionCtx), vp, vp, vp, vp, vp, i32, i32, f32,
                                        vp, vp, vp, vp, vp, sz, vp]),
     'interdiff_correction_dev': (C.c_int, [C.POINTER(CorrectionCtx), vp, vp, vp, vp, vp, i32, i32, vp, vp, vp, sz, vp]),
+    'interdiff_correction_prepare': (C.c_int, [C.POINTER(CorrectionCtx), vp, vp, vp, i32, i32, vp, sz, vp]),
+    'interdiff_correction_prepare_info': (C.c_int, [C.POINTER(CorrectionCtx), i32, i32, vp, C.POINTER(i64)]),
     'interdiff_metrics_workspace_bytes': (sz, [C.POINTER(CorrectionCtx), i32, i32]),
     'interdiff_metrics': (C.c_int, [C.POINTER(CorrectionCtx), vp, vp, vp, vp, vp, vp, vp, vp, i32, i32, i32,
                                     vp, vp, sz, vp]),
diff --git a/interdiff_amd/correction.py b/interdiff_amd/correction.py
--- a/interdiff_amd/correction.py
+++ b/interdiff_amd/correction.py
@@ -47,7 +47,33 @@
     graph_capturable = True
 
     def workspace_for(self, B, T):
-        return torch.empty(self.lib.interdiff_correction_workspace_bytes(C.byref(self.ctx), B, T), dtype=torch.uint8, device=self.device)
+        return self._clear_header(torch.empty(self.lib.interdiff_correction_workspace_bytes(C.byref(self.ctx), B, T), dtype=torch.uint8, device=self.device))
+
+    def _clear_header(self, ws):
+        _lib.check(self.lib.interdiff_correction_prepare(C.byref(self.ctx), None, None, None, 0, 0, _lib.dptr(ws), ws.numel(), _lib.stream()), 'correction_prepare')
+        return ws
+
+    def prepare_sample(self, y, ws=None):
+        hp, beta, pts = y['hand_pose'].contiguous().float(), y['beta'].contiguous().float(), y['obj_points'].contiguous().float()
+        T, B = hp.shape[0], hp.shape[1]
+        if pts.shape[1] != self.ctx.n_points:
+            raise ValueError('obj_points must have %d points' % self.ctx.n_points)
+        if ws is None:
+            ws = self._workspace(B, T)
+        _lib.check(self.lib.interdiff_correction_prepare(C.byref(self.ctx), _lib.dptr(hp), _lib.dptr(beta), _lib.dptr(pts), B, T, _lib.dptr(ws), ws.numel(),
+                                                         _lib.stream()), 'correction_prepare')
+        return self.prepare_info(B, T, ws)['prepared']
+
+    def end_sample(self, ws=None):
+        for w in ([ws] if ws is not None else list(self._ws.values())):
+            self._clear_header(w)
+
+    def prepare_info(self, B, T, ws=None):
+        if ws is None:
+            ws = self._workspace(B, T)
+        info = (C.c_int64 * 4)()
+        _lib.check(self.lib.interdiff_correction_prepare_info(C.byref(self.ctx), B, T, _lib.dptr(ws), info), 'correction_prepare_info')
+        return dict(prepared=bool(info[0]), U=int(info[1]), base_id=ws[info[2]:info[2] + 4 * T * B].view(torch.int32), cap=int(info[3]))
 
     def apply_dev(self, x, table, state, y, ws):
         B, _, Cc, T = x.shape
@@ -64,7 +90,7 @@
         key = torch.cuda.current_stream(self.device).cuda_stream
         ws = self._ws.pop(key, None)
         if ws is None or ws.numel() < need:
-            ws = torch.empty(need, dtype=torch.uint8, device=self.device)
+            ws = self._clear_header(torch.empty(need, dtype=torch.uint8, device=self.device))
         self._ws[key] = ws
         if len(self._ws) > self.MAX_STREAM_WORKSPACES:
             torch.cuda.synchronize(self.device)
diff --git a/interdiff_amd/csrc/contact_scan.h b/interdiff_amd/csrc/contact_scan.h
--- a/interdiff_amd/csrc/contact_scan.h
+++ b/interdiff_amd/csrc/contact_scan.h
@@ -518,6 +518,7 @@
     int64_t nn_from;
     const float *pts_frame; int frames_per_clip;
     PredArgs pred;
+    bool porder_ready;
 };
 
 template <bool OPT, bool WITH_PRED>
@@ -533,7 +534,7 @@
     const int32_t *adj_ptr = OPT ? nullptr : c->adj_ptr, *adj_face = OPT ? nullptr : c->adj_face, *adj_corner = OPT ? nullptr : c->adj_corner;
     const int32_t *adj_pair = OPT ? nullptr : c->adj_pair_scan;
     const int M = OPT ? 0 : c->n_markers;
-    if (!OPT && a.porder) hipLaunchKernelGGL(corr_point_order_kernel, dim3((unsigned)a.B), dim3(1024), 0, s, a.obj_points, a.P, a.porder);
+    if (!OPT && a.porder && !a.porder_ready) hipLaunchKernelGGL(corr_point_order_kernel, dim3((unsigned)a.B), dim3(1024), 0, s, a.obj_points, a.P, a.porder);
     const int nclips = WITH_PRED ? a.pred.nclips : 0;
     const size_t lds_launch = (nclips > 0 && lds < idf_objproj_dev::OBJPROJ_LDS) ? idf_objproj_dev::OBJPROJ_LDS : lds;
     if (lds_launch > (size_t)LDS_LIMIT) return IDF_E_INVAL;
diff --git a/interdiff_amd/csrc/correction.hip b/interdiff_amd/csrc/correction.hip
--- a/interdiff_amd/csrc/correction.hip
+++ b/interdiff_amd/csrc/correction.hip
@@ -2,6 +2,7 @@
 #include "objproj.h"
 #include "rot_math.h"
 #include <float.h>
+#include <unordered_map>
 
 namespace {
 
@@ -96,12 +97,62 @@
     x0[i] = a * x + (1.0f - a) * other;
 }
 
+__global__ __launch_bounds__(256) void corr_share_rows_kernel(const float *__restrict__ hand_pose, const float *__restrict__ beta, int B, int T,
+                                                              int32_t *__restrict__ base_id, int32_t *__restrict__ rep_frame, int32_t *__restrict__ rep_cnt) {
+    extern __shared__ int32_t first[];
+    const int b = blockIdx.x, tid = threadIdx.x;
+    const uint32_t *hp = reinterpret_cast<const uint32_t *>(hand_pose), *bt = reinterpret_cast<const uint32_t *>(beta);
+    for (int t = tid; t < T; t += 256) {
+        const size_t n = (size_t)t * B + b;
+        int f = t;
+        for (int tp = 0; tp < t; ++tp) {
+            const size_t np = (size_t)tp * B + b;
+            bool eq = true;
+            for (int k = 0; k < 90 && eq; ++k) eq = hp[n * 90 + k] == hp[np * 90 + k];
+            for (int k = 0; k < 10 && eq; ++k) eq = bt[n * 10 + k] == bt[np * 10 + k];
+            if (eq) { f = tp; break; }
+        }
+        first[t] = f;
+    }
+    __syncthreads();
+    if (tid == 0) {
+        int r = 0;
+        for (int t = 0; t < T; ++t)
+            if (first[t] == t) { first[T + t] = r; rep_frame[(size_t)b * T + r] = t; ++r; }
+        rep_cnt[b] = r;
+    }
+    __syncthreads();
+    for (int t = tid; t < T; t += 256) base_id[(size_t)t * B + b] = first[T + first[t]];
+}
+
+__global__ __launch_bounds__(256) void corr_gather_rows_kernel(const float *__restrict__ hand_pose, const float *__restrict__ beta, int B, int T,
+                                                               int32_t *__restrict__ base_id, const int32_t *__restrict__ rep_frame, int32_t *__restrict__ rep_cnt,
+                                                               float *__restrict__ pose, float *__restrict__ betas, float *__restrict__ trans) {
+    const int b = blockIdx.x, tid = threadIdx.x;
+    int off = 0;
+    for (int i = 0; i < b; ++i) off += rep_cnt[i];
+    const int cnt = rep_cnt[b];
+    for (int t = tid; t < T; t += 256) base_id[(size_t)t * B + b] += off;
+    for (int i = tid; i < cnt * 169; i += 256) {
+        const int r = i / 169, k = i - r * 169;
+        const size_t u = (size_t)off + r, n = (size_t)rep_frame[(size_t)b * T + r] * B + b;
+        if (k < 156) pose[u * 156 + k] = k < 66 ? 0.f : hand_pose[n * 90 + (k - 66)];
+        else if (k < 166) betas[u * 10 + (k - 156)] = beta[n * 10 + (k - 156)];
+        else trans[u * 3 + (k - 166)] = 0.f;
+    }
+    if (b == B - 1 && tid == 0) rep_cnt[B] = off + cnt;
+}
+
 struct CorrWs {
     float *pose, *trans, *objR, *objT, *gt_angles, *gt_trans, *verts, *jtr, *markers, *loss_sum, *min_dist, *proj, *proj_keep;
     int32_t *label, *contact, *porder;
     uint8_t *condition;
     void *smpl_ws;
     size_t smpl_ws_bytes, total;
+    int32_t *base_id, *rep_cnt, *rep_frame;
+    float *rep_beta, *base;
+    int64_t base_cap;
+    size_t base_id_off;
 };
 
 CorrWs carve(const idf_correction_ctx *c, int B, int T, void *ws) {
@@ -130,6 +181,13 @@
     w.proj_keep = (float *)take((size_t)B * idf_objproj_keep_floats() * 4);
     w.smpl_ws_bytes = interdiff_smpl_workspace_bytes(c->smpl, N);
     w.smpl_ws = take(w.smpl_ws_bytes);
+    w.base_id_off = off;
+    w.base_id = (int32_t *)take(N * 4);
+    w.rep_cnt = (int32_t *)take(((size_t)B + 1) * 4);
+    w.rep_frame = (int32_t *)take(N * 4);
+    w.rep_beta = (float *)take(N * 10 * 4);
+    w.base_cap = N / 4;
+    w.base = (float *)take((size_t)w.base_cap * interdiff_smpl_base_floats(c->smpl) * 4);
     w.total = off;
     return w;
 }
@@ -141,6 +199,74 @@
 extern "C" size_t interdiff_correction_workspace_bytes(const idf_correction_ctx *c, int32_t B, int32_t T) {
     if (!c || !c->smpl || B <= 0 || T <= 0) return 0;
     return carve(c, B, T, nullptr).total;
+}
+
+struct CorrHeader {
+    bool prepared;
+    const idf_correction_ctx *ctx;
+    const float *hand_pose, *beta, *obj_points;
+    int32_t B, T, U;
+};
+static std::mutex g_corr_hdr_mu;
+static std::unordered_map<const void *, CorrHeader> g_corr_hdr;
+
+static bool corr_header(const void *ws, CorrHeader *h) {
+    std::lock_guard<std::mutex> lk(g_corr_hdr_mu);
+    const auto it = g_corr_hdr.find(ws);
+    if (it == g_corr_hdr.end()) return false;
+    *h = it->second;
+    return true;
+}
+
+static bool corr_shape_ok(const idf_correction_ctx *c, int32_t B, int32_t T) {
+    return c->smpl->J == 52 && c->smpl->n_betas == 10 && c->n_markers <= MAXM && c->n_markers == c->objproj->P && c->n_points <= MAXP && T == c->objproj->T &&
+           c->past_len == c->objproj->past_len && c->past_len < T;
+}
+
+extern "C" int interdiff_correction_prepare(const idf_correction_ctx *c, const float *hand_pose, const float *beta, const float *obj_points, int32_t B,
+                                            int32_t T, void *ws, size_t ws_bytes, void *stream) {
+    if (!ws) return IDF_E_INVAL;
+    {
+        std::lock_guard<std::mutex> lk(g_corr_hdr_mu);
+        g_corr_hdr.erase(ws);
+    }
+    if (!hand_pose && !beta && !obj_points) return IDF_OK;
+    if (!c || !c->smpl || !c->objproj || !hand_pose || !beta || !obj_points || B <= 0 || T <= 0 || !corr_shape_ok(c, B, T)) return IDF_E_INVAL;
+    CorrWs w = carve(c, B, T, ws);
+    if (ws_bytes < w.total) return IDF_E_NOMEM;
+    hipStream_t s = idf_stream(stream);
+    idf_prof_mark(IDF_K_CORR_PREPARE, s);
+    hipLaunchKernelGGL(corr_share_rows_kernel, dim3((unsigned)B), dim3(256), 2 * (size_t)T * sizeof(int32_t), s, hand_pose, beta, B, T, w.base_id, w.rep_frame,
+                       w.rep_cnt);
+    hipLaunchKernelGGL(corr_gather_rows_kernel, dim3((unsigned)B), dim3(256), 0, s, hand_pose, beta, B, T, w.base_id, w.rep_frame, w.rep_cnt, w.pose,
+                       w.rep_beta, w.trans);
+    idf_prof_mark(-1, s);
+    int32_t U = 0;
+    if (hipMemcpyAsync(&U, w.rep_cnt + B, sizeof(U), hipMemcpyDeviceToHost, s) != hipSuccess || hipStreamSynchronize(s) != hipSuccess) return IDF_E_LAUNCH;
+    CorrHeader h{false, c, hand_pose, beta, obj_points, B, T, U};
+    if (U >= 1 && U <= w.base_cap) {
+        int rc = interdiff_smpl_blend_base(c->smpl, w.pose, w.rep_beta, w.trans, U, w.base, w.jtr, w.smpl_ws, w.smpl_ws_bytes, stream);
+        if (rc) return rc;
+        rc = idf_point_order(s, obj_points, B, c->n_points, w.porder);
+        if (rc) return rc;
+        IDF_CHECK_LAUNCH();
+        h.prepared = true;
+    }
+    std::lock_guard<std::mutex> lk(g_corr_hdr_mu);
+    g_corr_hdr[ws] = h;
+    return IDF_OK;
+}
+
+extern "C" int interdiff_correction_prepare_info(const idf_correction_ctx *c, int32_t B, int32_t T, const void *ws, int64_t *info4) {
+    if (!c || !c->smpl || !ws || !info4 || B <= 0 || T <= 0) return IDF_E_INVAL;
+    const CorrWs w = carve(c, B, T, nullptr);
+    CorrHeader h{};
+    const bool have = corr_header(ws, &h) && h.B == B && h.T == T;
+    info4[0] = have && h.prepared;
+    info4[1] = have ? h.U : 0;
+    info4[2] = (int64_t)w.base_id_off;
+    info4[3] = w.base_cap;
+    return IDF_OK;
 }
 
 static int correction_impl(const idf_correction_ctx *c, float *x0, const float *gt, const float *hand_pose,
@@ -149,24 +275,26 @@
                            size_t ws_bytes, void *stream) {
     if (!c || !c->smpl || !c->objproj || !x0 || !gt || !hand_pose || !beta || !obj_points || !ws || B <= 0 || T <= 0) return IDF_E_INVAL;
     const int V = c->smpl->V, M = c->n_markers, P = c->n_points;
-    if (c->smpl->J != 52 || c->smpl->n_betas != 10 || M > MAXM || M != c->objproj->P || P > MAXP || T != c->objproj->T ||
-        c->past_len != c->objproj->past_len || c->past_len >= T)
-        return IDF_E_INVAL;
+    if (!corr_shape_ok(c, B, T)) return IDF_E_INVAL;
     CorrWs w = carve(c, B, T, ws);
     if (ws_bytes < w.total) return IDF_E_NOMEM;
     hipStream_t s = idf_stream(stream);
     const int64_t N = (int64_t)B * T;
+    CorrHeader hdr{};
+    const bool prepared = corr_header(ws, &hdr) && hdr.prepared && hdr.ctx == c && hdr.hand_pose == hand_pose && hdr.beta == beta &&
+                          hdr.obj_points == obj_points && hdr.B == B && hdr.T == T && hdr.U >= 1 && hdr.U <= w.base_cap;
     const bool fused = (c->tune & 2) == 0 && idf_objproj_check(c->objproj) == IDF_OK;
     idf_prof_mark(IDF_K_CORR_PREPARE, s);
     hipLaunchKernelGGL(corr_prepare_kernel, dim3((unsigned)idf_cdiv(N * 24, 256)), dim3(256), 0, s, x0, gt, hand_pose, B, T, w.pose,
                        w.trans, w.objR, w.objT, w.gt_angles, w.gt_trans);
-    int rc = interdiff_smpl_forward(c->smpl, w.pose, beta, w.trans, N, w.verts, w.jtr, nullptr, w.smpl_ws, w.smpl_ws_bytes, stream);
+    int rc = prepared ? interdiff_smpl_forward_from_base(c->smpl, w.pose, beta, w.trans, N, w.base, w.base_id, w.verts, w.jtr, nullptr, w.smpl_ws, w.smpl_ws_bytes, stream)
+                      : interdiff_smpl_forward(c->smpl, w.pose, beta, w.trans, N, w.verts, w.jtr, nullptr, w.smpl_ws, w.smpl_ws_bytes, stream);
     if (rc) return rc;
     idf_prof_mark(IDF_K_CORR_CONTACT, s);
     ContactArgs a{};
     a.verts = w.verts; a.V = V;
     a.obj_points = obj_points; a.P = P;
-    a.porder = w.porder;
+    a.porder = w.porder; a.porder_ready = prepared;
     a.objR = w.objR; a.objT = w.objT;
     a.ctx = c;
     a.B = B;
diff --git a/interdiff_amd/csrc/smpl.hip b/interdiff_amd/csrc/smpl.hip
--- a/interdiff_amd/csrc/smpl.hip
+++ b/interdiff_amd/csrc/smpl.hip
@@ -78,13 +78,18 @@
 constexpr int SF = 16;
 constexpr int TBF = 10, TBV = 4;
 
-template <int NG>
+enum { SMPL_FULL = 0, SMPL_PREFIX = 1, SMPL_SUFFIX = 2 };
+constexpr int GV = 12;
+
+template <int NG, int ROLE>
 __global__ __launch_bounds__(BT) void smpl_blend_skin_kernel(const idf_smpl_model m, const float *__restrict__ feat,
                                                               const float *__restrict__ A, const float *__restrict__ trans,
                                                               int64_t N, float *__restrict__ verts,
-                                                              float *__restrict__ v_posed) {
+                                                              float *__restrict__ v_posed, float *base ,
+                                                              const int32_t *__restrict__ base_id , int ldb) {
     extern __shared__ __attribute__((aligned(16))) float sm[];
-    idf_args_now(m.V, m.J, m.S, m.blend, m.skin_idx, m.skin_w, feat, A, trans, N, verts, v_posed, gridDim.x);
+    static_assert(NG > GV, "the constant k-groups come first");
+    idf_args_now(m.V, m.J, m.S, m.blend, m.skin_idx, m.skin_w, feat, A, trans, N, verts, v_posed, base, base_id, ldb, gridDim.x);
     constexpr int KB = 16 * NG, nq = KB / 4;
     const int V = m.V, J = m.J, S = m.S;
     float *As = sm, *stage = sm;
@@ -110,19 +115,38 @@
         }
     }
     const int vl = tid & 63, vme = v0 + vl;
-    float sw[4];
-    int so[4];
-#pragma unroll
-    for (int k = 0; k < 4; ++k) {
-        const size_t e = (size_t)min(vme, V - 1) * S + min(k, S - 1);
-        sw[k] = m.skin_w[e];
-        so[k] = m.skin_idx[e] * 12;
-    }
-#pragma unroll
-    for (int k = 0; k < 4; ++k) {
-        const bool ok = k < S && vme < V;
-        sw[k] = ok ? sw[k] : 0.f;
-        so[k] = ok ? so[k] : 0;
+    float sw[4] = {0.f, 0.f, 0.f, 0.f};
+    int so[4] = {0, 0, 0, 0};
+    if constexpr (ROLE != SMPL_PREFIX) {
+#pragma unroll
+        for (int k = 0; k < 4; ++k) {
+            const size_t e = (size_t)min(vme, V - 1) * S + min(k, S - 1);
+            sw[k] = m.skin_w[e];
+            so[k] = m.skin_idx[e] * 12;
+        }
+#pragma unroll
+        for (int k = 0; k < 4; ++k) {
+            const bool ok = k < S && vme < V;
+            sw[k] = ok ? sw[k] : 0.f;
+            so[k] = ok ? so[k] : 0;
+        }
+    }
+    f32x4 acc[FM][3];
+    if constexpr (ROLE == SMPL_SUFFIX) {
+        const float *bcol = base + (size_t)vtile * NTC + wave * 48 + li;
+#pragma unroll
+        for (int i = 0; i < FM; ++i)
+#pragma unroll
+            for (int r = 0; r < 4; ++r) {
+                const float *bp = bcol + (size_t)base_id[min(f0 + (fh * FM + i) * 16 + kq * 4 + r, N - 1)] * ldb;
+#pragma unroll
+                for (int t = 0; t < 3; ++t) acc[i][t][r] = bp[t * 16];
+            }
+    } else {
+#pragma unroll
+        for (int i = 0; i < FM; ++i)
+#pragma unroll
+            for (int t = 0; t < 3; ++t) acc[i][t] = f32x4{0.f, 0.f, 0.f, 0.f};
     }
     asm volatile("s_waitcnt vmcnt(0)" ::: "memory");
     __syncthreads();
@@ -131,11 +155,6 @@
     const float *brow[3];
 #pragma unroll
     for (int t = 0; t < 3; ++t) brow[t] = m.blend + ((size_t)((vtile * 4 + wave) * 3 + t) * NG * 64 + lane) * 4;
-    f32x4 acc[FM][3];
-#pragma unroll
-    for (int i = 0; i < FM; ++i)
-#pragma unroll
-        for (int t = 0; t < 3; ++t) acc[i][t] = f32x4{0.f, 0.f, 0.f, 0.f};
     constexpr int PD = 3;
     float4 bq[PD + 1][3];
     auto ldg = [&](float4 (&dst)[3], int gi) {
@@ -157,14 +176,30 @@
             for (int t = 0; t < 3; ++t) acc[i][t] = __builtin_amdgcn_mfma_f32_16x16x4f32(a.w, bc[t].w, acc[i][t], 0, 0, 0);
         }
     };
-#pragma unroll
-    for (int g = 0; g < PD && g < NG; ++g) ldg(bq[g], g);
-#pragma unroll
-    for (int g = 0; g < NG; ++g) {
-        if (g + PD < NG) ldg(bq[(g + PD) % (PD + 1)], g + PD);
+    constexpr int P0 = ROLE == SMPL_SUFFIX ? NG - GV : 0, NS = ROLE == SMPL_PREFIX ? NG - GV : NG - P0;
+    auto grp = [](int p) { return p < NG - GV ? GV + p : p - (NG - GV); };
+#pragma unroll
+    for (int g = 0; g < PD && g < NS; ++g) ldg(bq[g], grp(P0 + g));
+#pragma unroll
+    for (int g = 0; g < NS; ++g) {
+        if (g + PD < NS) ldg(bq[(g + PD) % (PD + 1)], grp(P0 + g + PD));
         __builtin_amdgcn_sched_barrier(0);
-        mac(bq[g % (PD + 1)], g);
+        mac(bq[g % (PD + 1)], grp(P0 + g));
         __builtin_amdgcn_sched_barrier(0);
+    }
+    if constexpr (ROLE == SMPL_PREFIX) {
+        IDF_SMPL_STAMP(2);
+        float *bcol = base + (size_t)vtile * NTC + wave * 48 + li;
+#pragma unroll
+        for (int i = 0; i < FM; ++i)
+#pragma unroll
+            for (int r = 0; r < 4; ++r) {
+                const int64_t fr = f0 + (fh * FM + i) * 16 + kq * 4 + r;
+                if (fr >= N) continue;
+#pragma unroll
+                for (int t = 0; t < 3; ++t) bcol[(size_t)fr * ldb + t * 16] = acc[i][t][r];
+            }
+        return;
     }
     __syncthreads();
     IDF_SMPL_STAMP(2);
@@ -235,10 +270,15 @@
     return idf_align((size_t)N * m->KB * sizeof(float)) + idf_align(((size_t)N + SF) * m->J * 12 * sizeof(float));
 }
 
-extern "C" int interdiff_smpl_forward(const idf_smpl_model *m, const float *pose, const float *betas, const float *trans,
-                                      int64_t N, float *verts, float *jtr, float *v_posed, void *ws, size_t ws_bytes,
-                                      void *stream) {
-    if (!m || !pose || !betas || !trans || !verts || !jtr || !ws || N < 0) return IDF_E_INVAL;
+extern "C" size_t interdiff_smpl_base_floats(const idf_smpl_model *m) {
+    return m ? (size_t)idf_cdiv(m->V, VT) * NTC : 0;
+}
+
+template <int ROLE>
+static int smpl_run(const idf_smpl_model *m, const float *pose, const float *betas, const float *trans, int64_t N, float *verts, float *jtr,
+                    float *v_posed, float *base, const int32_t *base_id, void *ws, size_t ws_bytes, void *stream) {
+    if (!m || !pose || !betas || !trans || (ROLE != SMPL_PREFIX && !verts) || !jtr || !ws || N < 0) return IDF_E_INVAL;
+    if (ROLE != SMPL_FULL && (!base || (ROLE == SMPL_SUFFIX && !base_id))) return IDF_E_INVAL;
     if (m->J < 1 || m->J > MAXJ || m->KB % 16 != 0 || m->KB < 9 * (m->J - 1) + m->n_betas + 1 || m->S < 1) return IDF_E_INVAL;
     if (ws_bytes < interdiff_smpl_workspace_bytes(m, N)) return IDF_E_NOMEM;
     if (N == 0) return IDF_OK;
@@ -251,12 +291,29 @@
     if (lds > 150 * 1024 || m->KB % 32 != 0 || (m->V * 3) % 2 != 0 || m->S > 4) return IDF_E_INVAL;
     if (m->KB != 480) return IDF_E_INVAL;
     static std::atomic<uint64_t> lds_ok{0};
-    if (lds > 64 * 1024 && idf_opt_in_lds(reinterpret_cast<const void *>(smpl_blend_skin_kernel<30>), 150 * 1024, lds_ok) != IDF_OK) return IDF_E_LAUNCH;
+    if (lds > 64 * 1024 && idf_opt_in_lds(reinterpret_cast<const void *>(smpl_blend_skin_kernel<30, ROLE>), 150 * 1024, lds_ok) != IDF_OK) return IDF_E_LAUNCH;
     idf_prof_mark(IDF_K_SMPL_BLEND_SKIN, s);
     const unsigned nwg_launch = (unsigned)(idf_cdiv(idf_cdiv(N, FT), TBF) * idf_cdiv(idf_cdiv(m->V, VT), TBV) * TBF * TBV);
-    hipLaunchKernelGGL(smpl_blend_skin_kernel<30>, dim3(nwg_launch), dim3(BT), lds, s, *m,
-                       feat, A, trans, N, verts, v_posed);
+    hipLaunchKernelGGL((smpl_blend_skin_kernel<30, ROLE>), dim3(nwg_launch), dim3(BT), lds, s, *m,
+                       feat, A, trans, N, verts, v_posed, base, base_id, (int)interdiff_smpl_base_floats(m));
     idf_prof_mark(-1, s);
     IDF_CHECK_LAUNCH();
     return IDF_OK;
 }
+
+extern "C" int interdiff_smpl_forward(const idf_smpl_model *m, const float *pose, const float *betas, const float *trans,
+                                      int64_t N, float *verts, float *jtr, float *v_posed, void *ws, size_t ws_bytes,
+                                      void *stream) {
+    return smpl_run<SMPL_FULL>(m, pose, betas, trans, N, verts, jtr, v_posed, nullptr, nullptr, ws, ws_bytes, stream);
+}
+
+extern "C" int interdiff_smpl_blend_base(const idf_smpl_model *m, const float *pose, const float *betas, const float *trans, int64_t U, float *base,
+                                         float *jtr, void *ws, size_t ws_bytes, void *stream) {
+    return smpl_run<SMPL_PREFIX>(m, pose, betas, trans, U, nullptr, jtr, nullptr, base, nullptr, ws, ws_bytes, stream);
+}
+
+extern "C" int interdiff_smpl_forward_from_base(const idf_smpl_model *m, const float *pose, const float *betas, const float *trans, int64_t N,
+                                                const float *base, const int32_t *base_id, float *verts, float *jtr, float *v_posed, void *ws,
+                                                size_t ws_bytes, void *stream) {
+    return smpl_run<SMPL_SUFFIX>(m, pose, betas, trans, N, verts, jtr, v_posed, const_cast<float *>(base), base_id, ws, ws_bytes, stream);
+}
diff --git a/interdiff_amd/diffusion.py b/interdiff_amd/diffusion.py
--- a/interdiff_amd/diffusion.py
+++ b/interdiff_amd/diffusion.py
@@ -38,6 +38,13 @@
 
 def inpaint(x, gt, mask_u8):
     _lib.check(_lib.load().interdiff_inpaint(_lib.dptr(x, torch.float32), _lib.dptr(gt, torch.float32), _lib.dptr(mask_u8), x.numel(), _lib.stream()), 'inpaint')
+
+
+def hook_wants_prepare(hook, y, t_first, todo):
+    if hook is None or not hasattr(hook, 'prepare_sample') or not isinstance(y, dict) or not all(k in y for k in ('hand_pose', 'beta', 'obj_points')):
+        return False
+    active = getattr(hook, 'is_active', None)
+    return active is None or any(active(i) for i in range(t_first, t_first - todo, -1))
 
 
 def seeded_state(t_start, seed, elem0):
@@ -224,18 +231,25 @@
         cond = model_kwargs.get('y', {}).get('cond') if isinstance(model_kwargs.get('y', None), dict) else None
         if cond is not None and hasattr(model, 'prepare_memory'):
             model.prepare_memory(cond)
-        for it, i in enumerate(range(t_first, t_first - todo, -1)):
-            t, th = ts[i], ts_hook[i]
-            t.host_value = th.host_value = i
-            if step_noise is None:
-                nz = None
-            elif callable(step_noise):
-                nz = step_noise(it, img).contiguous()
-            else:
-                nz = step_noise[it]
-            self._step(model, img, None, i, it, t, model_kwargs, denoised_fn, nz, seed, elem0, rows_kw, th, rows)
-            if dump_steps is not None and it in dump_steps:
-                dump.append(img.clone())
+        hook_prepared = hook_wants_prepare(denoised_fn, model_kwargs.get('y'), t_first, todo)
+        if hook_prepared:
+            denoised_fn.prepare_sample(model_kwargs['y'])
+        try:
+            for it, i in enumerate(range(t_first, t_first - todo, -1)):
+                t, th = ts[i], ts_hook[i]
+                t.host_value = th.host_value = i
+                if step_noise is None:
+                    nz = None
+                elif callable(step_noise):
+                    nz = step_noise(it, img).contiguous()
+                else:
+                    nz = step_noise[it]
+                self._step(model, img, None, i, it, t, model_kwargs, denoised_fn, nz, seed, elem0, rows_kw, th, rows)
+                if dump_steps is not None and it in dump_steps:
+                    dump.append(img.clone())
+        finally:
+            if hook_prepared:
+                denoised_fn.end_sample()
         return dump if dump_steps is not None else img
 
     def sample_timesteps(self, B, device, generator=None):
diff --git a/interdiff_amd/graph_sampler.py b/interdiff_amd/graph_sampler.py
--- a/interdiff_amd/graph_sampler.py
+++ b/interdiff_amd/graph_sampler.py
@@ -69,6 +69,7 @@
         self.y = {k: torch.empty(y[k].shape, dtype=torch.float32, device=entry.x.device) for k in HOOK_KEYS}
         self.y['inpainted_motion'] = entry.gt if entry.gt is not None else torch.empty_like(entry.x)
         self.fresh = True
+        self.prepared_run = False
 
 
 class Entry:
@@ -166,6 +167,7 @@
     def __init__(self, model, entry, table, rows, fused, split, hook, hk, tmap=None):
         self.model, self.entry, self.table, self.rows, self.tmap = model, entry, table, rows, tmap
         self.fused, self.split, self.hook, self.hk = fused, split, hook, hk
+        self.prepared = False
 
     def enqueue_forward(self):
         st = self.entry
@@ -218,7 +220,7 @@
         return self.graph((k, self.fused, self.split), self.enqueue_plain, k)
 
     def hook_block(self, k):
-        return self.graph(('hook', self.hook._uid, k, self.fused, self.split), self.enqueue_hook_block, k)
+        return self.graph(('hook', self.hook._uid, k, self.fused, self.split, self.prepared), self.enqueue_hook_block, k)
 
     def eager_hook_step(self, t, model_kwargs):
         st = self.entry
@@ -290,5 +292,17 @@
         for ch in st.chains[1:]:
             ch.state.copy_(diffusion.seeded_state(t_start, seed, elem0 + ch.sl.start * per_clip))
     st.ts.fill_(diff.timestep_map[t_start])
-    dump = run.play(plan_steps(t_start, todo, hook_gate(hook), dump_steps, fuse_hook), t_start, diff._timesteps(B, dev, loop_side=True), model_kwargs)
+    prepare = diffusion.hook_wants_prepare(hook, y, t_start, todo)
+    prep_ws = run.hk.ws if fuse_hook else None
+    try:
+        if prepare:
+            run.prepared = hook.prepare_sample(run.hk.y if fuse_hook else y, ws=prep_ws)
+            if run.prepared and fuse_hook and not run.hk.prepared_run:
+                hook.apply_dev(run.hk.y['inpainted_motion'].clone(), table, torch.zeros(8, dtype=torch.int64, device=dev), run.hk.y, run.hk.ws)
+                torch.cuda.synchronize(dev)
+                run.hk.prepared_run = True
+        dump = run.play(plan_steps(t_start, todo, hook_gate(hook), dump_steps, fuse_hook), t_start, diff._timesteps(B, dev, loop_side=True), model_kwargs)
+    finally:
+        if prepare:
+            hook.end_sample(prep_ws)
     return dump if dump_steps is not None else st.x.clone()
diff --git a/interdiff_amd/smpl.py b/interdiff_amd/smpl.py
--- a/interdiff_amd/smpl.py
+++ b/interdiff_amd/smpl.py
@@ -66,7 +66,19 @@
             self._ws = torch.empty(max(need, 256), dtype=torch.uint8, device=self.device)
         return self._ws
 
-    def forward(self, th_pose_axisang, th_betas=None, th_trans=None, th_offsets=None, scale=1., want_v_posed=True):
+    def blend_base(self, th_pose_axisang, th_betas=None):
+        U = th_pose_axisang.shape[0]
+        if th_betas is None:
+            th_betas = torch.zeros(U, self.cmodel.n_betas, device=self.device)
+        pose, betas = th_pose_axisang.contiguous().float(), th_betas.contiguous().float()
+        base = torch.empty(U, self.lib.interdiff_smpl_base_floats(C.byref(self.cmodel)), dtype=torch.float32, device=self.device)
+        jtr, trans = torch.empty(U, self.cmodel.J, 3, device=self.device), torch.zeros(U, 3, device=self.device)
+        ws = self._workspace(U)
+        _lib.check(self.lib.interdiff_smpl_blend_base(C.byref(self.cmodel), _lib.dptr(pose, torch.float32), _lib.dptr(betas, torch.float32), _lib.dptr(trans), U,
+                                                      _lib.dptr(base), _lib.dptr(jtr), _lib.dptr(ws), ws.numel(), _lib.stream()), 'smpl_blend_base')
+        return base
+
+    def forward(self, th_pose_axisang, th_betas=None, th_trans=None, th_offsets=None, scale=1., want_v_posed=True, base=None, base_id=None):
         if th_offsets is not None or scale != 1.:
             raise NotImplementedError('th_offsets / scale are not used on the eval_smpl_short path')
         N = th_pose_axisang.shape[0]
@@ -82,6 +94,14 @@
         jtr = torch.empty(N, J, 3, dtype=torch.float32, device=self.device)
         v_posed = torch.empty(N, V, 3, dtype=torch.float32, device=self.device) if want_v_posed else None
         ws = self._workspace(N)
+        if base is not None:
+            if base_id.dtype != torch.int32 or base_id.numel() != N or int(base_id.max()) >= base.shape[0] or int(base_id.min()) < 0:
+                raise ValueError('base_id must be int32 [N] with values below %d' % base.shape[0])
+            _lib.check(self.lib.interdiff_smpl_forward_from_base(C.byref(self.cmodel), _lib.dptr(pose, torch.float32), _lib.dptr(betas, torch.float32),
+                                                                 _lib.dptr(trans, torch.float32), N, _lib.dptr(base, torch.float32), _lib.dptr(base_id), _lib.dptr(verts),
+                                                                 _lib.dptr(jtr), _lib.dptr(v_posed, allow_none=True), _lib.dptr(ws), ws.numel(), _lib.stream()),
+                       'smpl_forward_from_base')
+            return verts, jtr, v_posed, v_posed
         _lib.check(self.lib.interdiff_smpl_forward(C.byref(self.cmodel), _lib.dptr(pose, torch.float32), _lib.dptr(betas, torch.float32),
                                                    _lib.dptr(trans, torch.float32), N, _lib.dptr(verts), _lib.dptr(jtr),
                                                    _lib.dptr(v_posed, allow_none=True), _lib.dptr(ws), ws.numel(), _lib.stream()),
```

Result: slower. 7.050 million (-1.5%).
